# hmetaxa/MVTopicModel

Hardware: AMD Instinct MI355X
Metric: gibbs_tokens_per_sec (higher is better)
Workload: dtype f64

## Files before the change

include/mvhdp.h:

```cpp
#ifndef MVHDP_H
#define MVHDP_H

#include <stddef.h>
#include <stdint.h>

#ifdef __cplusplus
extern "C" {
#endif

#define MVHDP_MAX_MODALITIES 8
#define MVHDP_MAX_TOPICS     2048
#define MVHDP_UNASSIGNED_TOPIC (-1)

typedef enum {
    MVHDP_OK = 0,
    MVHDP_ERR_INVALID_ARG   = -1,
    MVHDP_ERR_STATE         = -2,
    MVHDP_ERR_HIP           = -3,
    MVHDP_ERR_NO_DEVICE     = -4,
    MVHDP_ERR_NEGATIVE_COUNT= -5,
    MVHDP_ERR_UNSUPPORTED   = -6
} mvhdp_status;

typedef struct mvhdp_ctx* mvhdp_handle;

typedef struct {
    int32_t num_topics;
    int32_t num_modalities;
    int32_t num_types[MVHDP_MAX_MODALITIES];
    int32_t device;
    int64_t doc_id_base;
    uint32_t flags;
} mvhdp_config;

typedef struct {
    const double* alpha;
    double alpha_sum[MVHDP_MAX_MODALITIES];
    double beta[MVHDP_MAX_MODALITIES];
    double beta_sum[MVHDP_MAX_MODALITIES];
    double gamma[MVHDP_MAX_MODALITIES];
    double p_a[MVHDP_MAX_MODALITIES][MVHDP_MAX_MODALITIES];
    double p_b[MVHDP_MAX_MODALITIES][MVHDP_MAX_MODALITIES];
    const uint8_t* inactive;
} mvhdp_hyper;

typedef struct {
    int64_t tokens;
    int64_t changed;
    int64_t new_mass_cnt;
    int64_t topic_doc_mass_cnt;
    int64_t word_ftree_mass_cnt;
    int64_t oov_skipped;
    int64_t aborted_docs;
    int64_t exact_fallbacks;
    int32_t activated_topic;
    int32_t activated_modality;
    int64_t activation_key;
    double  sweep_kernel_ms;
    double  total_ms;
    int32_t activations;
    int32_t reserved;
} mvhdp_sweep_stats;

#define MVHDP_ACT_DOC_SHIFT   34
#define MVHDP_ACT_VIEW_SHIFT  31
#define MVHDP_ACT_POS_SHIFT   11
#define MVHDP_ACT_TOPIC_MASK  0x7ffLL
#define MVHDP_ACT_VIEW_MASK   0x7LL
#define MVHDP_ACT_KEY(doc, view, pos, topic) \
    (((int64_t)(doc) << MVHDP_ACT_DOC_SHIFT) | ((int64_t)(view) << MVHDP_ACT_VIEW_SHIFT) | ((int64_t)(pos) << MVHDP_ACT_POS_SHIFT) | (int64_t)(topic))
#define MVHDP_ACT_KEY_TOPIC(key) ((int32_t)((key) & MVHDP_ACT_TOPIC_MASK))
#define MVHDP_ACT_KEY_VIEW(key)  ((int32_t)(((key) >> MVHDP_ACT_VIEW_SHIFT) & MVHDP_ACT_VIEW_MASK))
#define MVHDP_ACT_KEY_NONE INT64_MAX

typedef struct {
    double* tok_dbg[MVHDP_MAX_MODALITIES];
    int32_t n_trace;
    const int64_t* trace_doc;
    const int32_t* trace_view;
    const int32_t* trace_pos;
    double* trace_out;
} mvhdp_debug;

#define MVHDP_SWEEP_REUSE_TREES 0x1u
#define MVHDP_SWEEP_NO_APPLY    0x2u
#define MVHDP_SWEEP_EXACT_CHAIN 0x4u
#define MVHDP_SWEEP_GENERIC_KERNEL 0x8u
#define MVHDP_SWEEP_FROZEN      0x10u

#define MVHDP_SWEEP_LIVE        0x20u
#define MVHDP_SWEEP_LIVE_SEGMENTS(n) (((uint32_t)(n) & 0xffu) << 16)

#define MVHDP_SWEEP_SEGMENT_APPLY 0x40u

#define MVHDP_SWEEP_SEGMENT_OVERLAP 0x80u

#define MVHDP_SWEEP_ONLY_SEGMENT(s) ((((uint32_t)(s) + 1u) & 0xffu) << 24)

#define MVHDP_SWEEP_SHARD_BIRTHS 0x200u

typedef enum {
    MVHDP_BUF_COUNTS = 0,
    MVHDP_BUF_DELTA  = 1,
    MVHDP_BUF_BIRTH_KEYS = 2,
    MVHDP_BUF_COUNTS12 = 3,
    MVHDP_BUF_ROW_CLASS = 4
} mvhdp_buffer;

int mvhdp_create(const mvhdp_config* cfg, mvhdp_handle* out);
int mvhdp_destroy(mvhdp_handle h);
const char* mvhdp_last_error(mvhdp_handle h);
const char* mvhdp_version(void);

int mvhdp_set_corpus(mvhdp_handle h, int32_t m, int64_t num_docs,
                     const int64_t* doc_off , const int32_t* tokens );
int mvhdp_set_assignments(mvhdp_handle h, int32_t m, const int32_t* z );
int mvhdp_set_view_presence(mvhdp_handle h, int32_t m, const uint8_t* present );
int mvhdp_get_assignments(mvhdp_handle h, int32_t m, int32_t* z );

int mvhdp_set_hyper(mvhdp_handle h, const mvhdp_hyper* hy);
int mvhdp_get_alpha(mvhdp_handle h, double* alpha , uint8_t* inactive );
int mvhdp_build_counts(mvhdp_handle h);
int mvhdp_build_trees(mvhdp_handle h);
int mvhdp_build_inference_trees(mvhdp_handle h);
int mvhdp_init_assignments_from_trees(mvhdp_handle h, uint64_t seed);
int mvhdp_get_counts(mvhdp_handle h, int32_t m, int32_t* n_wk , int32_t* n_k );
int mvhdp_set_counts(mvhdp_handle h, int32_t m, const int32_t* n_wk, const int32_t* n_k);
int mvhdp_get_tree(mvhdp_handle h, int32_t m, int32_t type, double* tree );
int mvhdp_get_doc_topic_hist(mvhdp_handle h, int32_t m, int32_t* hist , int32_t hist_len,
                             int32_t* doc_len_counts , int32_t len_len);

int mvhdp_get_count_histogram(mvhdp_handle h, int32_t m, int32_t* hist, int32_t len);
int mvhdp_view_overlap_sums(mvhdp_handle h, double* sums );
int mvhdp_model_log_likelihood(mvhdp_handle h, double* log_likelihood );
int mvhdp_gamma_doc_statistics(mvhdp_handle h, int32_t m, double gamma_m, uint64_t seed, uint32_t round, double* qs, double* qw);
int mvhdp_dp_table_statistics(mvhdp_handle h, int32_t m, const int32_t* hist , int32_t hist_len, const double* conc ,
                              uint64_t seed, uint32_t round, double* mk , uint8_t* active );
int mvhdp_antoniak_draws(mvhdp_handle h, int32_t n, const int32_t* items , const double* conc , uint64_t seed, uint32_t round, int32_t* tables );
int mvhdp_doc_topic_proportions(mvhdp_handle h, const double* view_weights , int64_t d0, int64_t d1, double* out );


int mvhdp_doc_topics_top(mvhdp_handle h, const double* view_weights , int64_t d0, int64_t d1, double threshold, int32_t max,
                         int64_t cap, int64_t* row_off , int32_t* topics, double* weights, int64_t* count);
int mvhdp_entity_topic_distributions(mvhdp_handle h, const double* view_weights, double threshold, int32_t max, int32_t round_digits ,
                                     int64_t n_groups, const int64_t* member_off , const int64_t* members ,
                                     double* out );

typedef enum { MVHDP_SIM_COS_FOLDED = 0,
               MVHDP_SIM_COS        = 1,
               MVHDP_SIM_JSD        = 2    } mvhdp_sim_metric;
typedef struct { int32_t metric; int32_t n, dim; const double* x ; double min_weight; double threshold;
                 int32_t stripe_rows ; int64_t candidate_capacity ; } mvhdp_sim_args;
typedef struct { int64_t pairs_screened ,
                 candidates, emitted; int32_t stripes, regrown; double margin; } mvhdp_sim_stats;
int mvhdp_similar_pairs(mvhdp_handle h, const mvhdp_sim_args* a, int64_t cap, int32_t* i, int32_t* j, double* sim,
                        int64_t* count, mvhdp_sim_stats* stats );
int mvhdp_sim_probe(int32_t n, int32_t dim, int32_t stripe_rows, mvhdp_sim_stats* out);

#define MVHDP_DIAG_MAX_TOP_WORDS 64
#define MVHDP_DIAG_PROPORTIONS   7
#define MVHDP_DIAG_TOKENS             0
#define MVHDP_DIAG_DOCUMENT_ENTROPY   1
#define MVHDP_DIAG_WORD_LENGTH        2
#define MVHDP_DIAG_COHERENCE          3
#define MVHDP_DIAG_NORM_DISCR_WEIGHT  4
#define MVHDP_DIAG_DISCR_WEIGHT       5
#define MVHDP_DIAG_UNIFORM_DIST       6
#define MVHDP_DIAG_CORPUS_DIST        7
#define MVHDP_DIAG_EFF_NUM_WORDS      8
#define MVHDP_DIAG_TOKEN_DOC_DIFF     9
#define MVHDP_DIAG_RANK_1_DOCS       10
#define MVHDP_DIAG_ALLOCATION_RATIO  11
#define MVHDP_DIAG_ALLOCATION_COUNT  12
#define MVHDP_DIAG_ROWS              13
typedef struct {
    int32_t num_top_words;
    const int32_t* word_length;
} mvhdp_diag_args;
typedef struct {
    double*  scores;
    double*  word_scores;
    int32_t* codoc;
    int32_t* top_types;
    int32_t* top_counts;
    int32_t* nonzero;
    int32_t* num_rank1_docs;
    int32_t* num_nonzero_docs;
    int32_t* num_docs_at_proportions;
    double*  sum_count_log_count;
    int32_t* word_type_counts;
    int64_t* num_tokens;
    double*  discr_weight_per_view;
} mvhdp_diag_out;
int mvhdp_top_words(mvhdp_handle h, int32_t m, int32_t n, int32_t* types , int32_t* counts , int32_t* nonzero );
int mvhdp_discr_weights(mvhdp_handle h, double* per_view , int32_t m, double* type_weight );
int mvhdp_diagnostics(mvhdp_handle h, const mvhdp_diag_args* args, mvhdp_diag_out* out);

typedef struct {
    int32_t num_columns;
    int32_t num_context_columns;
    int32_t with_topics;
    int32_t window;
    int32_t num_samples;
    int32_t min_doc_length;
    int64_t sampling_table_size;
    double  sampling_factor;
    double  min_exp, max_exp;
    int32_t sigmoid_cache_size;
    int32_t reserved;
} mvhdp_emb_config;
typedef struct {
    int64_t words_so_far;
    int64_t words_sampled;
    int64_t words_considered;
    int64_t docs_skipped;
    int64_t calls;
    int64_t negatives_skipped;
    double  residual;
    double  last_epoch_residual;
    int64_t last_epoch_calls;
    double  kernel_ms;
} mvhdp_emb_stats;
#define MVHDP_EMB_SERIAL 0x1u
int mvhdp_emb_init(mvhdp_handle h, const mvhdp_emb_config* cfg, const double* weights , uint64_t seed);
int mvhdp_emb_count_words(mvhdp_handle h);
int mvhdp_emb_train(mvhdp_handle h, int32_t epochs, uint64_t seed, uint32_t round, uint32_t flags, mvhdp_emb_stats* stats );
int mvhdp_emb_get_vectors(mvhdp_handle h, double* weights , double* negative_weights );
int mvhdp_emb_set_vectors(mvhdp_handle h, const double* weights , const double* negative_weights );
int mvhdp_emb_word_stats(mvhdp_handle h, int64_t* counts , double* retention , int64_t* total_words );
int mvhdp_emb_sampling_table(mvhdp_handle h, int64_t first, int64_t n, int32_t* types );
int mvhdp_emb_softmax(mvhdp_handle h, int32_t reset_sums, double* exp_dot , double* sum_exp );
int mvhdp_emb_nearest(mvhdp_handle h, const double* query , int32_t n, int32_t* words, double* word_sims, int32_t* topics, double* topic_sims);
int mvhdp_emb_release(mvhdp_handle h);

int mvhdp_set_vectors_mix(mvhdp_handle h, double lambda, const double* exp_dot , const double* sum_exp );
int mvhdp_get_vectors_mix(mvhdp_handle h, double* lambda, double* mix );

int mvhdp_sweep(mvhdp_handle h, uint32_t sweep_idx, uint64_t seed, uint32_t flags,
                const double* p_override, const mvhdp_debug* dbg, mvhdp_sweep_stats* stats);
int mvhdp_sweep_many(mvhdp_handle h, uint32_t first_idx, int32_t n, uint64_t seed, uint32_t flags, mvhdp_sweep_stats* stats );
int mvhdp_apply_delta(mvhdp_handle h, int32_t activated_topic, int32_t activated_modality);
int mvhdp_apply_delta_begin(mvhdp_handle h);
int mvhdp_apply_delta_rows(mvhdp_handle h, int64_t row_begin, int64_t row_end);
int mvhdp_apply_delta_end(mvhdp_handle h, int32_t activated_topic, int32_t activated_modality);
int mvhdp_get_birth_keys(mvhdp_handle h, int64_t* keys );
int mvhdp_activate_births(mvhdp_handle h, const int64_t* keys );
int mvhdp_trees_current(mvhdp_handle h);
int mvhdp_get_view_weights(mvhdp_handle h, double* p );

typedef struct {
    int32_t force_primary;
    int32_t narrow;
    int32_t walk_fixed;
    int32_t single_stream;
    int32_t live16;
    int32_t single_wave;
    double  walk_theta[MVHDP_MAX_MODALITIES];
    double  primary_min_share;
    int32_t learnt_walk_step[4];
// ... 80 lines not shown
```

mvtopicmodel_amd/csrc/mvhdp_api.hip:

```cpp
#include "mvhdp_ctx.h"

static thread_local std::string g_create_error;

static std::mutex g_reg_mutex;
static std::set<mvhdp_ctx*>* g_live = nullptr;
static bool g_exiting = false, g_atexit_registered = false;
static void release_device_resources(mvhdp_ctx* h);

static void mvhdp_at_exit()
{
    std::lock_guard<std::mutex> lk(g_reg_mutex);
    g_exiting = true;
    if (g_live) for (mvhdp_ctx* h : *g_live) release_device_resources(h);
}

static void register_handle(mvhdp_ctx* h)
{
    std::lock_guard<std::mutex> lk(g_reg_mutex);
    if (!g_live) g_live = new std::set<mvhdp_ctx*>();
    g_live->insert(h);
    if (!g_atexit_registered) { atexit(mvhdp_at_exit); g_atexit_registered = true; }
}

bool mvhdp_is_live(mvhdp_ctx* h)
{
    std::lock_guard<std::mutex> lk(g_reg_mutex);
    return g_live && g_live->count(h) != 0;
}

static void read_environment(mvhdp_ctx* h)
{
    if (const char* f = getenv("MVHDP_FORCE_RMAX")) { const int v = atoi(f); if (v == 1 || v == 2 || v == 4 || v == 8 || v == 16 || v == 32) h->tu.force_primary = v; }
    if (const char* f = getenv("MVHDP_NARROW")) h->tu.narrow = atoi(f) != 0 ? -1 : 0;
    if (const char* f = getenv("MVHDP_SINGLE_STREAM")) h->tu.single_stream = atoi(f) != 0;
    if (const char* f = getenv("MVHDP_SIDE_PRIORITY")) h->side_priority = atoi(f);
    if (const char* f = getenv("MVHDP_LIVE16")) h->tu.live16 = atoi(f);
    if (const char* f = getenv("MVHDP_LIVE_OVERLAP")) h->tu.live_overlap = atoi(f);
    if (const char* f = getenv("MVHDP_LIVE_ROWS")) h->tu.live_rows = atoi(f);
    if (const char* f = getenv("MVHDP_LIVE_ROWS_THETA")) h->tu.live_rows_theta = atof(f);
    if (const char* f = getenv("MVHDP_COEF_LDS_KB")) h->tu.coef_lds_max_bytes = std::max(0, std::min(64, atoi(f))) * 1024;
    if (const char* f = getenv("MVHDP_LIVE_ROWS_SEGMENTS")) h->tu.live_rows_segments = std::max(1, std::min(255, atoi(f)));
    if (const char* f = getenv("MVHDP_WIDEST_ON_MAIN")) h->tu.widest_on_main = atoi(f) != 0;
    if (const char* f = getenv("MVHDP_NARROW_WIDE")) h->tu.narrow_wide = atoi(f) != 0;
    if (const char* f = getenv("MVHDP_SLIM")) h->tu.slim = std::max(0, std::min(2, atoi(f)));
    if (const char* f = getenv("MVHDP_LIVE_TREE_EVERY")) h->live_tree_every = std::max(1, atoi(f));
    if (const char* f = getenv("MVHDP_GATE_PCT")) { const int v = atoi(f); if (v >= 5 && v <= 95) h->gate_pct = v; }
    if (const char* f = getenv("MVHDP_FOUR_ROUND_ON_C")) h->tu.four_round_on_c = atoi(f);
    if (const char* f = getenv("MVHDP_DELTA16")) h->tu.delta16 = atoi(f) != 0;
    if (const char* f = getenv("MVHDP_FORK_DELAY_US")) h->tu.fork_delay_us = std::max(0, std::min(1000, atoi(f)));
    if (const char* f = getenv("MVHDP_FORCE_MODE")) { if (!strcmp(f, "serial")) h->tu.single_stream = 1; }
    if (const char* f = getenv("MVHDP_PRIMARY_MIN_SHARE")) { const double v = atof(f); if (v > 0.0 && v <= 1.0) h->tu.primary_min_share = v; }
    if (const char* t = getenv("MVHDP_WALK_THETA")) {
        int m = 0;
        for (const char* q = t; *q && m < MVHDP_MAXM; m++) {
            h->tu.walk_theta[m] = atof(q);
            while (*q && *q != ',') q++;
            if (*q == ',') q++;
        }
        for (; m < MVHDP_MAXM; m++) h->tu.walk_theta[m] = 0.0;
        h->tu.walk_fixed = 1;
    }
    h->dbg_env = getenv("MVHDP_DEBUG") != nullptr;
    h->diag.overlap_serial = getenv("MVHDP_OVERLAP_SERIAL") != nullptr;
    h->diag.no_row_sample = getenv("MVHDP_NO_ROW_SAMPLE") != nullptr;
    h->diag.no_heavy_refresh = getenv("MVHDP_NO_HEAVY_REFRESH") != nullptr;
}

hipError_t make_stream(hipStream_t* out, bool high_priority)
{
    int least = 0, greatest = 0;
    if (high_priority && hipDeviceGetStreamPriorityRange(&least, &greatest) == hipSuccess && greatest < least &&
        hipStreamCreateWithPriority(out, hipStreamNonBlocking, greatest) == hipSuccess) return hipSuccess;
    if (high_priority) { (void)hipGetLastError(); *out = nullptr; }
    return hipStreamCreateWithFlags(out, hipStreamNonBlocking);
}

extern "C" const char* mvhdp_version(void) { return "mvhdp 0.1 (gfx950)"; }

extern "C" const char* mvhdp_last_error(mvhdp_handle h) { return (h && mvhdp_is_live(h)) ? h->err.c_str() : g_create_error.c_str(); }

extern "C" int mvhdp_create(const mvhdp_config* cfg, mvhdp_handle* out)
{
    if (!cfg || !out) { g_create_error = "null argument"; return MVHDP_ERR_INVALID_ARG; }
    *out = nullptr;
    const int K = cfg->num_topics, M = cfg->num_modalities;
    if (K < 1 || K > MVHDP_MAX_TOPICS || M < 1 || M > MVHDP_MAX_MODALITIES) {
        g_create_error = "num_topics must be in [1,2048] and num_modalities in [1,8]";
        return MVHDP_ERR_INVALID_ARG;
    }
    for (int m = 0; m < M; m++) if (cfg->num_types[m] < 1) { g_create_error = "num_types[m] must be >= 1"; return MVHDP_ERR_INVALID_ARG; }
    for (int m = 0; m < M; m++) if (cfg->num_types[m] >= (1 << 29)) { g_create_error = "num_types[m] must be below 2^29"; return MVHDP_ERR_INVALID_ARG; }
    if (cfg->doc_id_base < 0 || cfg->doc_id_base >= (1LL << 29)) { g_create_error = "doc_id_base out of range"; return MVHDP_ERR_INVALID_ARG; }
    int ndev = 0;
    if (hipGetDeviceCount(&ndev) != hipSuccess || ndev <= 0 || cfg->device < 0 || cfg->device >= ndev) {
        g_create_error = "no usable HIP device (the sweep has no CPU fallback)";
        return MVHDP_ERR_NO_DEVICE;
    }
    hipDeviceProp_t prop;
    if (hipGetDeviceProperties(&prop, cfg->device) != hipSuccess) { g_create_error = "hipGetDeviceProperties failed"; return MVHDP_ERR_HIP; }
    if (strncmp(prop.gcnArchName, "gfx950", 6) != 0) {
        g_create_error = std::string("device is ") + prop.gcnArchName + ", this library is built for gfx950 only";
        return MVHDP_ERR_NO_DEVICE;
    }
    mvhdp_ctx* h = new mvhdp_ctx();
    register_handle(h);
    h->cfg = *cfg;
    h->device = cfg->device;
    h->num_cus = prop.multiProcessorCount;
    h->max_lds = 160 * 1024;
    MvModel& mm = h->mm;
    mm.K = K; mm.M = M;
    mm.rowbase[0] = 0;
    for (int m = 0; m < M; m++) { mm.V[m] = cfg->num_types[m]; mm.rowbase[m + 1] = mm.rowbase[m] + cfg->num_types[m]; }
    mm.doc_id_base = cfg->doc_id_base;
    mm.first_inactive = -1;
    mm.D = -1;
#define CREATE_HIP(call) do { hipError_t e_ = (call); if (e_ != hipSuccess) { \
    g_create_error = std::string(#call) + ": " + hipGetErrorString(e_); mvhdp_destroy(h); return MVHDP_ERR_HIP; } } while (0)
    CREATE_HIP(hipSetDevice(h->device));
    CREATE_HIP(hipStreamCreateWithFlags(&h->stream, hipStreamNonBlocking));
    h->own_stream = true;
    for (auto& e : h->ev) CREATE_HIP(hipEventCreate(&e));
    const int64_t nrows = mm.rowbase[M];
    const size_t cbytes = (size_t)(nrows * K + (int64_t)M * K + MVHDP_TAIL_WORDS) * sizeof(int32_t);
    CREATE_HIP(hipMalloc(&mm.counts, cbytes));
    CREATE_HIP(hipMalloc(&mm.delta, cbytes));
    CREATE_HIP(hipMemset(mm.counts, 0, cbytes));
    CREATE_HIP(hipMalloc(&mm.counts16, (size_t)nrows * K * sizeof(uint16_t) + 64));
    CREATE_HIP(hipMemset(mm.counts16, 0, (size_t)nrows * K * sizeof(uint16_t)));
    CREATE_HIP(hipMalloc(&mm.delta16, (size_t)(nrows * K + 2) * sizeof(uint16_t)));
    CREATE_HIP(hipMemsetD16(mm.delta16, (unsigned short)0x8000, (size_t)(nrows * K + 2)));
    CREATE_HIP(hipMalloc(&mm.heavy, (size_t)nrows));
    CREATE_HIP(hipMemset(mm.heavy, 1, (size_t)nrows));
    CREATE_HIP(hipMemset(mm.delta, 0, cbytes));
    CREATE_HIP(hipMalloc(&mm.trees, (size_t)nrows * 2 * K * sizeof(double)));
    CREATE_HIP(hipMalloc(&mm.root, (size_t)nrows * sizeof(double)));
    CREATE_HIP(hipMalloc(&mm.mass0, (size_t)nrows * sizeof(float)));
    CREATE_HIP(hipMemset(mm.mass0, 0, (size_t)nrows * sizeof(float)));
    CREATE_HIP(hipMalloc(&mm.coef, (size_t)M * (((K + 7) & ~7) + K + 8) * sizeof(float)));
    {
        const int nlev = (K > 1) ? (32 - __builtin_clz((unsigned)(K - 1))) : 0;
        mm.dt_f = nlev ? ((nlev - 1) % 3) + 1 : 0;
        mm.dt_nbd = 1; mm.dt_base[0] = 0; mm.dt_depth[0] = 0;
        int nblk = 1;
        for (int dep = mm.dt_f; nlev && dep < nlev; dep += 3) {
            mm.dt_base[mm.dt_nbd] = nblk; mm.dt_depth[mm.dt_nbd] = dep; mm.dt_nbd++;
            nblk += 1 << dep;
        }
        mm.dt_nblk = nblk;
        CREATE_HIP(hipMalloc(&mm.dtab, (size_t)nrows * nblk * 8 * sizeof(double)));
    }
    CREATE_HIP(hipMalloc(&h->d_alpha, (size_t)M * (K + 1) * sizeof(double)));
    CREATE_HIP(hipMalloc(&h->d_inactive, (size_t)K));
    CREATE_HIP(hipMemset(h->d_inactive, 0, (size_t)K));
    CREATE_HIP(hipMalloc(&h->d_births, (size_t)(2 + 2 * K) * sizeof(int32_t)));
    CREATE_HIP(hipMemset(h->d_births, 0, (size_t)(2 + 2 * K) * sizeof(int32_t)));
    CREATE_HIP(hipMalloc(&h->d_birth_keys, (size_t)K * sizeof(long long)));
    CREATE_HIP(hipMalloc(&h->d_birth_table, (size_t)K * sizeof(long long)));
    {
        const std::vector<long long> none((size_t)K, LLONG_MAX);
        CREATE_HIP(hipMemcpy(h->d_birth_table, none.data(), (size_t)K * sizeof(long long), hipMemcpyHostToDevice));
    }
    CREATE_HIP(hipMalloc(&h->d_ctl, CTL_WORDS * sizeof(unsigned long long)));
    CREATE_HIP(hipMemset(h->d_ctl, 0, CTL_WORDS * sizeof(unsigned long long)));
    h->d_stats = h->d_ctl;
    h->d_act_key = (long long*)(h->d_ctl + ST_COUNT);
    h->d_ovf_meta = (unsigned int*)(h->d_ctl + ST_COUNT + 1);
    h->d_doc_counter = h->d_ctl + ST_COUNT + 1 + META_WORDS64;
    CREATE_HIP(hipHostMalloc((void**)&h->h_ctl, CTL_WORDS * sizeof(unsigned long long), hipHostMallocDefault));
    for (int c = 0; c < MVHDP_N_CLASSES; c++)
        for (int f = 0; f < MVHDP_N_FLAVOURS; f++) { h->regs.regs[c][f] = mvhdp_sweep_kernel_regs(c, f); h->regs.regs_mix[c][f] = mvhdp_sweep_kernel_regs(c, f == MVHDP_FLAVOUR_PLAIN ? MVHDP_FLAVOUR_WALK : f, true); }
    read_environment(h);
    {
        int vmax = 0;
        for (int m = 0; m < M; m++) vmax = std::max(vmax, (int)cfg->num_types[m]);
        if (plan_slim_table(K, vmax, h->tu.slim)) {
            CREATE_HIP(hipMalloc(&mm.counts12, (size_t)nrows * mvhdp_slim_row_bytes(K)));
            CREATE_HIP(hipMemset(mm.counts12, 0, (size_t)nrows * mvhdp_slim_row_bytes(K)));
        }
    }
    mm.alpha = h->d_alpha;
    mm.inactive = h->d_inactive;
    h->h_alpha.assign((size_t)M * (K + 1), 0.0);
    h->h_inactive.assign((size_t)K, 0);
    h->wt.init_defaults(K);
    h->wt_mix.init_defaults(K);
    *out = h;
    return MVHDP_OK;
}

static void release_device_resources(mvhdp_ctx* h)
{
    if (h->device_released) return;
    h->device_released = true;
    hipSetDevice(h->device);
    if (h->stream) hipStreamSynchronize(h->stream);
    auto fr = [](auto*& p) { if (p) { hipFree((void*)p); p = nullptr; } };
    for (int m = 0; m < MVHDP_MAXM; m++) { fr(h->d_doc_off[m]); fr(h->d_tok[m]); fr(h->d_z[m]); fr(h->d_carry[m]); fr(h->d_present[m]); }
    fr(h->mm.counts); fr(h->mm.delta16); fr(h->mm.counts16); fr(h->mm.counts12); fr(h->mm.heavy); fr(h->mm.delta); fr(h->mm.trees); fr(h->mm.root); fr(h->mm.coef); fr(h->mm.mass0); fr(h->d_births); fr(h->d_birth_keys); fr(h->d_birth_table); fr(h->mm.dtab); fr(h->mm.p);
    fr(h->d_alpha); fr(h->d_inactive); fr(h->d_ctl);
    fr(h->d_mix); fr(h->d_mix32); h->mm.mix = nullptr; h->mm.mix32 = nullptr; h->mix_lambda = 0.0;
    mvhdp_emb_free(h);
    if (h->h_ctl) { hipHostFree(h->h_ctl); h->h_ctl = nullptr; }
    h->d_stats = nullptr; h->d_act_key = nullptr; h->d_doc_counter = nullptr; h->d_ovf_meta = nullptr;
    fr(h->d_doc_order); fr(h->d_lists); fr(h->d_nslots); fr(h->d_stats_many); fr(h->d_heavy_list); fr(h->d_heavy_ctl);
    if (h->ev_rf_go) { hipEventDestroy(h->ev_rf_go); h->ev_rf_go = nullptr; }
    if (h->ev_rf_done) { hipEventDestroy(h->ev_rf_done); h->ev_rf_done = nullptr; }
    if (h->rf_stream) { hipStreamDestroy(h->rf_stream); h->rf_stream = nullptr; }
    fr(h->ov.counts2); fr(h->ov.counts16_2); fr(h->ov.dtab2); fr(h->ov.root2); fr(h->ov.trees2); fr(h->ov.delta2); fr(h->ov.delta3); fr(h->ov.ctl2); fr(h->ov.lists2);
    for (auto& e : h->ov.ev_seg) if (e) { hipEventDestroy(e); e = nullptr; }
    if (h->ov.ev_start) { hipEventDestroy(h->ov.ev_start); h->ov.ev_start = nullptr; }
    if (h->ov.x1) { hipStreamDestroy(h->ov.x1); h->ov.x1 = nullptr; }
    if (h->ov.xa) { hipStreamDestroy(h->ov.xa); h->ov.xa = nullptr; }
    for (auto& e : h->ev_many) if (e) { hipEventDestroy(e); e = nullptr; }
    for (auto& e : h->ev) if (e) { hipEventDestroy(e); e = nullptr; }
    if (h->ev_fork) { hipEventDestroy(h->ev_fork); h->ev_fork = nullptr; }
    for (auto& e : h->ev_join) if (e) { hipEventDestroy(e); e = nullptr; }
    for (auto& st : h->side) if (st) { hipStreamDestroy(st); st = nullptr; }
    if (h->own_stream && h->stream) hipStreamDestroy(h->stream);
    h->stream = nullptr;
}

extern "C" int mvhdp_destroy(mvhdp_handle h)
{
    if (!h) return MVHDP_OK;
    bool exiting;
    {
        std::lock_guard<std::mutex> lk(g_reg_mutex);
        if (!g_live || g_live->erase(h) == 0) return MVHDP_ERR_INVALID_ARG;
        exiting = g_exiting;
    }
    if (!exiting) release_device_resources(h);
    delete h;
    return MVHDP_OK;
}

extern "C" int mvhdp_set_stream(mvhdp_handle h, void* hip_stream)
{
    CHECK_H(h);
    HIPC(h, hipSetDevice(h->device));
    HIPC(h, hipStreamSynchronize(h->stream));
    if (h->own_stream) { hipStreamDestroy(h->stream); h->own_stream = false; }
    if (hip_stream) h->stream = (hipStream_t)hip_stream;
    else { HIPC(h, hipStreamCreateWithFlags(&h->stream, hipStreamNonBlocking)); h->own_stream = true; }
    return MVHDP_OK;
}

extern "C" int mvhdp_synchronize(mvhdp_handle h)
{
    CHECK_H(h);
    HIPC(h, hipSetDevice(h->device));
    HIPC(h, hipStreamSynchronize(h->stream));
    return MVHDP_OK;
}

extern "C" int mvhdp_set_corpus(mvhdp_handle h, int32_t m, int64_t D, const int64_t* doc_off, const int32_t* tokens)
{
    CHECK_H(h);
    MvModel& mm = h->mm;
    if (m < 0 || m >= mm.M || D < 0 || !doc_off) FAIL(h, MVHDP_ERR_INVALID_ARG, "set_corpus: bad view, num_docs or doc_off");
    if (mm.D >= 0 && D != mm.D) {
        bool any_other = false;
        for (int j = 0; j < mm.M; j++) if (j != m && h->have_corpus[j]) any_other = true;
        if (any_other) FAIL(h, MVHDP_ERR_INVALID_ARG, "set_corpus: every view must list the same entities (empty span = view absent)");
    }
    if (mm.doc_id_base + D >= (1LL << 29)) FAIL(h, MVHDP_ERR_INVALID_ARG, "set_corpus: too many entities");
    if (doc_off[0] != 0) FAIL(h, MVHDP_ERR_INVALID_ARG, "set_corpus: doc_off[0] must be 0");
    for (int64_t d = 0; d < D; d++) {
        int64_t len = doc_off[d + 1] - doc_off[d];
        if (len < 0) FAIL(h, MVHDP_ERR_INVALID_ARG, "set_corpus: doc_off must be non-decreasing");
        if (len >= (1 << 20)) FAIL(h, MVHDP_ERR_INVALID_ARG, "set_corpus: a view of one entity is limited to 2^20-1 tokens");
    }
    const int64_t N = doc_off[D];
    if (N > 0 && !tokens) FAIL(h, MVHDP_ERR_INVALID_ARG, "set_corpus: tokens is null");
    HIPC(h, hipSetDevice(h->device));
    HIPC(h, hipStreamSynchronize(h->stream));
    if (h->d_doc_off[m]) { hipFree(h->d_doc_off[m]); h->d_doc_off[m] = nullptr; }
    if (h->d_tok[m]) { hipFree(h->d_tok[m]); h->d_tok[m] = nullptr; }
    if (h->d_z[m]) { hipFree(h->d_z[m]); h->d_z[m] = nullptr; }
    if (h->d_present[m]) { hipFree(h->d_present[m]); h->d_present[m] = nullptr; }
    h->h_present[m].clear(); mm.present[m] = nullptr;
    HIPC(h, hipMalloc(&h->d_doc_off[m], (size_t)(D + 1) * sizeof(int64_t)));
    HIPC(h, hipMemcpy(h->d_doc_off[m], doc_off, (size_t)(D + 1) * sizeof(int64_t), hipMemcpyHostToDevice));
    const size_t nb = (size_t)std::max<int64_t>(N, 1) * sizeof(int32_t);
    HIPC(h, hipMalloc(&h->d_tok[m], nb));
    HIPC(h, hipMalloc(&h->d_z[m], nb));
    if (N > 0) HIPC(h, hipMemcpy(h->d_tok[m], tokens, (size_t)N * sizeof(int32_t), hipMemcpyHostToDevice));
    HIPC(h, hipMemset(h->d_z[m], 0xff, nb));
    h->unassigned[m] = N > 0;
    h->h_doc_off[m].assign(doc_off, doc_off + D + 1);
    h->N[m] = N;
    h->have_corpus[m] = true;
    h->max_doc_tokens = -1;
    if (h->d_doc_order) { hipFree(h->d_doc_order); h->d_doc_order = nullptr; }
    if (h->d_lists) { hipFree(h->d_lists); h->d_lists = nullptr; }
    if (h->ov.lists2) { hipFree(h->ov.lists2); h->ov.lists2 = nullptr; }
    if (h->d_nslots) { hipFree(h->d_nslots); h->d_nslots = nullptr; }
    mm.nslots = nullptr;
    for (auto& c : h->d_carry) if (c) { hipFree(c); c = nullptr; }
    h->nslots_valid = false;
    mm.D = D;
    mm.doc_off[m] = (const int64_t*)h->d_doc_off[m];
    mm.tok[m] = (const int32_t*)h->d_tok[m];
    mm.z[m] = (int32_t*)h->d_z[m];
    if (mm.p) { hipFree(mm.p); mm.p = nullptr; }
    h->have_counts = false; h->have_trees = false;
    return MVHDP_OK;
}

int require_corpus(mvhdp_ctx* h)
{
    for (int m = 0; m < h->mm.M; m++)
        if (!h->have_corpus[m]) FAIL(h, MVHDP_ERR_STATE, "set_corpus has not been called for every view");
    return MVHDP_OK;
}

extern "C" int mvhdp_set_assignments(mvhdp_handle h, int32_t m, const int32_t* z)
{
    CHECK_H(h);
    if (m < 0 || m >= h->mm.M) FAIL(h, MVHDP_ERR_INVALID_ARG, "set_assignments: bad view");
    if (!h->have_corpus[m]) FAIL(h, MVHDP_ERR_STATE, "set_assignments before set_corpus");
    if (h->N[m] > 0 && !z) FAIL(h, MVHDP_ERR_INVALID_ARG, "set_assignments: null z");
    bool any_unassigned = false;
    for (int64_t i = 0; i < h->N[m]; i++) {
        if (z[i] < -1 || z[i] >= h->mm.K) FAIL(h, MVHDP_ERR_INVALID_ARG, "set_assignments: topic out of range");
        any_unassigned = any_unassigned || z[i] < 0;
    }
    HIPC(h, hipSetDevice(h->device));
    HIPC(h, hipStreamSynchronize(h->stream));
    if (h->N[m] > 0) HIPC(h, hipMemcpy(h->d_z[m], z, (size_t)h->N[m] * sizeof(int32_t), hipMemcpyHostToDevice));
    h->unassigned[m] = any_unassigned;
    h->nslots_valid = false;
    if (h->have_counts) h->counts_stale = true;
    return MVHDP_OK;
}

extern "C" int mvhdp_set_view_presence(mvhdp_handle h, int32_t m, const uint8_t* present)
{
    CHECK_H(h);
    MvModel& mm = h->mm;
    if (m < 0 || m >= mm.M) FAIL(h, MVHDP_ERR_INVALID_ARG, "set_view_presence: bad view");
    if (!h->have_corpus[m]) FAIL(h, MVHDP_ERR_STATE, "set_view_presence before set_corpus");
    HIPC(h, hipSetDevice(h->device));
    HIPC(h, hipStreamSynchronize(h->stream));
    if (h->d_present[m]) { hipFree(h->d_present[m]); h->d_present[m] = nullptr; }
    h->h_present[m].clear(); mm.present[m] = nullptr;
    if (h->d_carry[m]) { hipFree(h->d_carry[m]); h->d_carry[m] = nullptr; }
    if (!present || mm.D == 0) return MVHDP_OK;
    for (int64_t d = 0; d < mm.D; d++)
        if (!present[d] && h->h_doc_off[m][d + 1] > h->h_doc_off[m][d]) FAIL(h, MVHDP_ERR_INVALID_ARG, "set_view_presence: an entity with tokens in the view is marked absent");
    h->h_present[m].assign(present, present + mm.D);
    HIPC(h, hipMalloc(&h->d_present[m], (size_t)mm.D));
    HIPC(h, hipMemcpy(h->d_present[m], present, (size_t)mm.D, hipMemcpyHostToDevice));
    mm.present[m] = h->d_present[m];
    return MVHDP_OK;
}

extern "C" int mvhdp_get_assignments(mvhdp_handle h, int32_t m, int32_t* z)
{
    CHECK_H(h);
    if (m < 0 || m >= h->mm.M) FAIL(h, MVHDP_ERR_INVALID_ARG, "get_assignments: bad view");
    if (!h->have_corpus[m]) FAIL(h, MVHDP_ERR_STATE, "get_assignments before set_corpus");
    HIPC(h, hipSetDevice(h->device));
    HIPC(h, hipStreamSynchronize(h->stream));
    if (h->N[m] > 0) HIPC(h, hipMemcpy(z, h->d_z[m], (size_t)h->N[m] * sizeof(int32_t), hipMemcpyDeviceToHost));
    return MVHDP_OK;
}

extern "C" int mvhdp_set_hyper(mvhdp_handle h, const mvhdp_hyper* hy)
{
    CHECK_H(h);
    if (!hy || !hy->alpha) FAIL(h, MVHDP_ERR_INVALID_ARG, "set_hyper: null");
    MvModel& mm = h->mm;
    const int K = mm.K, M = mm.M;
    for (int m = 0; m < M; m++) {
        if (!(hy->beta_sum[m] >= 1e-30 && hy->beta_sum[m] <= 1e30) || !(hy->beta[m] >= 1e-30 && hy->beta[m] <= 1e30))
            FAIL(h, MVHDP_ERR_INVALID_ARG, "set_hyper: beta and beta_sum must be in [1e-30, 1e30]");
        mm.alpha_sum[m] = hy->alpha_sum[m]; mm.beta[m] = hy->beta[m];
        mm.beta_sum[m] = hy->beta_sum[m];   mm.gamma[m] = hy->gamma[m];
        for (int j = 0; j < M; j++) { mm.p_a[m][j] = hy->p_a[m][j]; mm.p_b[m][j] = hy->p_b[m][j]; }
    }
    h->h_alpha.assign(hy->alpha, hy->alpha + (size_t)M * (K + 1));
    if (hy->inactive) h->h_inactive.assign(hy->inactive, hy->inactive + K);
    else h->h_inactive.assign((size_t)K, 0);
    mm.first_inactive = -1;
    for (int k = 0; k < K; k++) if (h->h_inactive[k]) { mm.first_inactive = k; break; }
    HIPC(h, hipSetDevice(h->device));
    HIPC(h, hipStreamSynchronize(h->stream));
    HIPC(h, hipMemcpy(h->d_alpha, h->h_alpha.data(), (size_t)M * (K + 1) * sizeof(double), hipMemcpyHostToDevice));
    HIPC(h, hipMemcpy(h->d_inactive, h->h_inactive.data(), (size_t)K, hipMemcpyHostToDevice));
    h->have_hyper = true;
    h->have_trees = false;
    return MVHDP_OK;
}

extern "C" int mvhdp_get_alpha(mvhdp_handle h, double* alpha, uint8_t* inactive)
{
    CHECK_H(h);
    if (!h->have_hyper) FAIL(h, MVHDP_ERR_STATE, "get_alpha before set_hyper");
    if (alpha) memcpy(alpha, h->h_alpha.data(), h->h_alpha.size() * sizeof(double));
    if (inactive) memcpy(inactive, h->h_inactive.data(), h->h_inactive.size());
    return MVHDP_OK;
}

extern "C" int mvhdp_build_counts(mvhdp_handle h)
{
    CHECK_H(h);
    int rc = require_corpus(h); if (rc) return rc;
    HIPC(h, hipSetDevice(h->device));
    HIPC(h, mvhdp_launch_build_counts(h->mm, h->N, h->stream));
    if (h->delta_pending) {
        HIPC(h, hipMemsetAsync(h->mm.delta, 0, (size_t)counts_len(h) * sizeof(int32_t), h->stream));
        h->delta_pending = false; h->delta_clean = true;
    }
    if (h->delta16_used) {
        HIPC(h, hipMemsetD16Async(h->mm.delta16, (unsigned short)0x8000, (size_t)(h->mm.rowbase[h->mm.M] * h->mm.K), h->stream));
        h->delta16_used = false;
    }
    HIPC(h, hipStreamSynchronize(h->stream));
    h->have_counts = true; h->have_trees = false; h->counts_stale = false;
    return MVHDP_OK;
}

static int ensure_full_trees(mvhdp_ctx* h)
{
    if (!h->have_trees || h->full_trees) return MVHDP_OK;
    HIPC(h, mvhdp_launch_build_trees(h->mm, h->trees_inference, true, h->stream));
    HIPC(h, hipStreamSynchronize(h->stream));
    h->full_trees = true;
    return MVHDP_OK;
}

extern "C" int mvhdp_build_trees(mvhdp_handle h)
{
    CHECK_H(h);
    if (!h->have_hyper) FAIL(h, MVHDP_ERR_STATE, "build_trees before set_hyper");
    if (!h->have_counts) FAIL(h, MVHDP_ERR_STATE, "build_trees before build_counts/set_counts");
    HIPC(h, hipSetDevice(h->device));
    HIPC(h, mvhdp_launch_build_trees(h->mm, false, true, h->stream));
    HIPC(h, hipStreamSynchronize(h->stream));
    h->have_trees = true; h->full_trees = true; h->trees_inference = false;
    return MVHDP_OK;
}

extern "C" int mvhdp_build_inference_trees(mvhdp_handle h)
{
    CHECK_H(h);
    if (!h->have_hyper) FAIL(h, MVHDP_ERR_STATE, "build_inference_trees before set_hyper");
    if (!h->have_counts) FAIL(h, MVHDP_ERR_STATE, "build_inference_trees before build_counts/set_counts");
    HIPC(h, hipSetDevice(h->device));
    HIPC(h, mvhdp_launch_build_trees(h->mm, true, true, h->stream));
    HIPC(h, hipStreamSynchronize(h->stream));
    h->have_trees = true; h->full_trees = true; h->trees_inference = true;
    return MVHDP_OK;
}

extern "C" int mvhdp_init_assignments_from_trees(mvhdp_handle h, uint64_t seed)
{
    CHECK_H(h);
    int rc = require_corpus(h); if (rc) return rc;
    if (!h->have_trees) FAIL(h, MVHDP_ERR_STATE, "init_assignments_from_trees before build_trees/build_inference_trees");
    HIPC(h, hipSetDevice(h->device));
    HIPC(h, mvhdp_launch_init_from_trees(h->mm, (uint32_t)seed, (uint32_t)(seed >> 32), h->stream));
    HIPC(h, hipStreamSynchronize(h->stream));
    for (int m = 0; m < h->mm.M; m++) h->unassigned[m] = false;
    h->nslots_valid = false;
    if (h->have_counts) h->counts_stale = true;
    return MVHDP_OK;
}

extern "C" int mvhdp_get_counts(mvhdp_handle h, int32_t m, int32_t* n_wk, int32_t* n_k)
{
    CHECK_H(h);
    MvModel& mm = h->mm;
    if (m < 0 || m >= mm.M) FAIL(h, MVHDP_ERR_INVALID_ARG, "get_counts: bad view");
    HIPC(h, hipSetDevice(h->device));
    HIPC(h, hipStreamSynchronize(h->stream));
    const int K = mm.K;
    if (n_wk) HIPC(h, hipMemcpy(n_wk, mm.counts + mm.rowbase[m] * K, (size_t)mm.V[m] * K * sizeof(int32_t), hipMemcpyDeviceToHost));
    if (n_k) HIPC(h, hipMemcpy(n_k, mm.counts + mm.rowbase[mm.M] * K + (int64_t)m * K, (size_t)K * sizeof(int32_t), hipMemcpyDeviceToHost));
    return MVHDP_OK;
}

extern "C" int mvhdp_set_counts(mvhdp_handle h, int32_t m, const int32_t* n_wk, const int32_t* n_k)
{
    CHECK_H(h);
    MvModel& mm = h->mm;
    if (m < 0 || m >= mm.M) FAIL(h, MVHDP_ERR_INVALID_ARG, "set_counts: bad view");
    HIPC(h, hipSetDevice(h->device));
    HIPC(h, hipStreamSynchronize(h->stream));
    const int K = mm.K;
    if (n_wk) HIPC(h, hipMemcpy(mm.counts + mm.rowbase[m] * K, n_wk, (size_t)mm.V[m] * K * sizeof(int32_t), hipMemcpyHostToDevice));
    if (n_k) HIPC(h, hipMemcpy(mm.counts + mm.rowbase[mm.M] * K + (int64_t)m * K, n_k, (size_t)K * sizeof(int32_t), hipMemcpyHostToDevice));
    h->have_counts = true; h->have_trees = false; h->counts_stale = false;
    return MVHDP_OK;
}

extern "C" int mvhdp_get_tree(mvhdp_handle h, int32_t m, int32_t type, double* tree)
{
    CHECK_H(h);
    MvModel& mm = h->mm;
    if (m < 0 || m >= mm.M || type < 0 || type >= mm.V[m] || !tree) FAIL(h, MVHDP_ERR_INVALID_ARG, "get_tree: bad argument");
    if (!h->have_trees) FAIL(h, MVHDP_ERR_STATE, "get_tree before build_trees");
    HIPC(h, hipSetDevice(h->device));
    { int rc2 = ensure_full_trees(h); if (rc2) return rc2; }
    HIPC(h, hipStreamSynchronize(h->stream));
    HIPC(h, hipMemcpy(tree, mm.trees + (mm.rowbase[m] + type) * 2 * mm.K, (size_t)2 * mm.K * sizeof(double), hipMemcpyDeviceToHost));
    return MVHDP_OK;
}

extern "C" int mvhdp_get_doc_topic_hist(mvhdp_handle h, int32_t m, int32_t* hist, int32_t hist_len,
                                        int32_t* doc_len_counts, int32_t len_len)
{
    CHECK_H(h);
    MvModel& mm = h->mm;
    if (m < 0 || m >= mm.M || (hist && hist_len < 1) || (doc_len_counts && len_len < 1))
        FAIL(h, MVHDP_ERR_INVALID_ARG, "get_doc_topic_hist: bad argument");
    int rc = require_corpus(h); if (rc) return rc;
    HIPC(h, hipSetDevice(h->device));
    int32_t *d_hist = nullptr, *d_len = nullptr;
    hipError_t e = hipSuccess;
    if (hist) e = hipMalloc(&d_hist, (size_t)mm.K * hist_len * sizeof(int32_t));
    if (e == hipSuccess && doc_len_counts) e = hipMalloc(&d_len, (size_t)len_len * sizeof(int32_t));
    if (e == hipSuccess) e = mvhdp_launch_doc_topic_hist(mm, m, d_hist, hist_len, d_len, len_len, h->stream);
    if (e == hipSuccess && hist) e = hipMemcpy(hist, d_hist, (size_t)mm.K * hist_len * sizeof(int32_t), hipMemcpyDeviceToHost);
    if (e == hipSuccess && doc_len_counts) e = hipMemcpy(doc_len_counts, d_len, (size_t)len_len * sizeof(int32_t), hipMemcpyDeviceToHost);
    if (d_hist) hipFree(d_hist);
    if (d_len) hipFree(d_len);
    HIPC(h, e);
    return MVHDP_OK;
}

int64_t compute_max_doc_tokens(mvhdp_ctx* h)
{
    if (h->max_doc_tokens >= 0) return h->max_doc_tokens;
    int64_t mx = 0, mn = INT64_MAX;
    const MvModel& mm = h->mm;
    std::vector<int64_t> tot((size_t)mm.D);
    for (int64_t d = 0; d < mm.D; d++) {
        int64_t t = 0;
        for (int m = 0; m < mm.M; m++) t += h->h_doc_off[m][d + 1] - h->h_doc_off[m][d];
        tot[d] = t;
        mx = std::max(mx, t); mn = std::min(mn, t);
    }
    if (h->d_doc_order) { hipFree(h->d_doc_order); h->d_doc_order = nullptr; }
// ... 125 lines not shown
    if (row_begin < 0 || row_end > nrows || row_begin > row_end) FAIL(h, MVHDP_ERR_INVALID_ARG, "apply_delta_rows: bad row range");
    HIPC(h, hipSetDevice(h->device));
    HIPC(h, mvhdp_launch_build_trees_rows(h->mm, false, h->last_need_full, row_begin, row_end, true, h->d_stats + ST_NEGATIVE, h->stream));
    h->rows_applied += row_end - row_begin;
    return MVHDP_OK;
}

extern "C" int mvhdp_apply_delta_end(mvhdp_handle h, int32_t activated_topic, int32_t activated_modality)
{
    CHECK_H(h);
    const int64_t nrows = h->mm.rowbase[h->mm.M];
    if (h->rows_applied != nrows) { h->rows_applied = -1; FAIL(h, MVHDP_ERR_STATE, "apply_delta_end: the row ranges applied do not cover every row exactly once"); }
    h->rows_applied = -1;
    HIPC(h, hipSetDevice(h->device));
    unsigned long long neg = 0;
    HIPC(h, hipMemcpyAsync(&neg, h->d_stats + ST_NEGATIVE, sizeof neg, hipMemcpyDeviceToHost, h->stream));
    HIPC(h, hipStreamSynchronize(h->stream));
    h->delta_clean = true; h->delta_pending = false;
    h->have_trees = true; h->full_trees = h->last_need_full; h->trees_inference = false;
    if (activated_topic >= 0) {
        h->have_trees = false;
        int rc = apply_activation(h, activated_topic, activated_modality);
        if (rc) return rc;
    }
    if (neg) FAIL(h, MVHDP_ERR_NEGATIVE_COUNT, "a topic count went below zero (UPD:202-215)");
    return MVHDP_OK;
}

extern "C" int mvhdp_trees_current(mvhdp_handle h)
{
    CHECK_H(h);
    return h->have_trees ? 1 : 0;
}

extern "C" int mvhdp_get_tuning(mvhdp_handle h, mvhdp_tuning* t)
{
    CHECK_H(h);
    if (!t) FAIL(h, MVHDP_ERR_INVALID_ARG, "get_tuning: null");
    memset(t, 0, sizeof *t);
    t->force_primary = h->tu.force_primary; t->narrow = h->tu.narrow; t->walk_fixed = h->tu.walk_fixed;
    t->single_stream = h->tu.single_stream; t->primary_min_share = h->tu.primary_min_share; t->live16 = h->tu.live16;
    t->single_wave = h->tu.single_wave; t->live_overlap = h->tu.live_overlap; t->live_rows = h->tu.live_rows;
    for (int m = 0; m < MVHDP_MAX_MODALITIES; m++) { t->walk_theta[m] = h->tu.walk_theta[m]; t->tree_branch_share[m] = h->wt.walk_f[m]; }
    for (int g = 0; g < WALK_GROUPS; g++) t->learnt_walk_step[g] = g == h->wt.walk_cls ? h->wt.walk_i : h->wt.walk_i_by[g];
    t->learnt_walk_step[3] = -1;
    return MVHDP_OK;
}

extern "C" int mvhdp_set_tuning(mvhdp_handle h, const mvhdp_tuning* t)
{
    CHECK_H(h);
    if (!t) FAIL(h, MVHDP_ERR_INVALID_ARG, "set_tuning: null");
    const int fp = t->force_primary;
    if (!(fp == 0 || fp == 1 || fp == 2 || fp == 4 || fp == 8 || fp == 16 || fp == 32)) FAIL(h, MVHDP_ERR_INVALID_ARG, "set_tuning: force_primary must be 0, 1, 2, 4, 8, 16 or 32");
    if (t->primary_min_share < 0.0 || t->primary_min_share > 1.0) FAIL(h, MVHDP_ERR_INVALID_ARG, "set_tuning: primary_min_share outside [0, 1]");
    for (int g = 0; g < WALK_GROUPS; g++) if (t->learnt_walk_step[g] < -1 || t->learnt_walk_step[g] > MVHDP_WALK_BINS) FAIL(h, MVHDP_ERR_INVALID_ARG, "set_tuning: learnt_walk_step outside [-1, 20]");
    h->tu.force_primary = fp; h->tu.narrow = t->narrow; h->tu.walk_fixed = t->walk_fixed ? 1 : 0;
    h->tu.single_stream = t->single_stream ? 1 : 0;
    h->tu.live16 = t->live16 < 0 ? -1 : (t->live16 ? 1 : 0);
    h->tu.single_wave = t->single_wave ? 1 : 0;
    h->tu.live_overlap = t->live_overlap < 0 ? -1 : (t->live_overlap ? 1 : 0);
    h->tu.live_rows = t->live_rows < 0 ? -1 : (t->live_rows ? 1 : 0);
    h->tu.primary_min_share = t->primary_min_share > 0.0 ? t->primary_min_share : 0.10;
    for (int m = 0; m < MVHDP_MAX_MODALITIES; m++) h->tu.walk_theta[m] = t->walk_theta[m];
    if (t->learnt_walk_step[0] >= 0 || t->learnt_walk_step[1] >= 0 || t->learnt_walk_step[2] >= 0) h->wt.restore(t->learnt_walk_step, t->tree_branch_share, h->mm.M);
    return MVHDP_OK;
}

extern "C" int mvhdp_plan_probe(const mvhdp_plan_input* pi, const mvhdp_tuning* t, mvhdp_plan_output* po)
{
    if (!pi || !po) return MVHDP_ERR_INVALID_ARG;
    PlanIn in;
    in.K = pi->num_topics; in.M = pi->num_modalities; in.D = pi->num_entities; in.mdt = pi->max_entity_tokens;
    if (in.K < 1 || in.K > MVHDP_MAX_TOPICS || in.M < 1 || in.M > MVHDP_MAX_MODALITIES || in.D < 0) return MVHDP_ERR_INVALID_ARG;
    in.have_order = true;
    for (int c = 0; c < 5; c++) in.n_longer[c] = pi->entities_longer_than[c];
    for (int b = 0; b < MVHDP_HIST_BINS; b++) in.tok_hist[b] = pi->tokens_by_list_rounds[b];
    for (int b = 0; b < MVHDP_ENT_BINS; b++) in.ent_hist[b] = pi->entities_by_class[b];
    in.flags = pi->flags; in.debug = pi->debug != 0; in.batch = pi->batch != 0; in.trees_current = pi->trees_current != 0;
    in.first_inactive = pi->inactive_topics ? 0 : -1;
    in.num_cus = pi->num_cus > 0 ? pi->num_cus : 256;
    for (int c = 0; c < MVHDP_N_CLASSES; c++) for (int f = 0; f < 3; f++) in.regs.regs[c][f] = pi->kernel_registers[c][f];
    for (int c = 0; c < MVHDP_N_CLASSES; c++) for (int f = 0; f < 3; f++) in.regs.regs_mix[c][f] = pi->kernel_registers_mix[c][f] > 0 ? pi->kernel_registers_mix[c][f] : pi->kernel_registers[c][f];
    in.vectors_mix = pi->vectors_mix != 0 && !(pi->flags & MVHDP_SWEEP_FROZEN);
    in.slim_table = t && t->narrow == 2;
    PlanTuning tu;
    WalkTuner wt;
    wt.init_defaults(in.K);
    if (t) {
        tu.force_primary = t->force_primary; tu.narrow = t->narrow; tu.walk_fixed = t->walk_fixed; tu.single_stream = t->single_stream;
        tu.live16 = t->live16; tu.single_wave = t->single_wave ? 1 : 0; tu.live_overlap = t->live_overlap; tu.live_rows = t->live_rows;
        if (t->primary_min_share > 0) tu.primary_min_share = t->primary_min_share;
        for (int m = 0; m < MVHDP_MAX_MODALITIES; m++) tu.walk_theta[m] = t->walk_theta[m];
        if (t->learnt_walk_step[0] >= 0 || t->learnt_walk_step[1] >= 0 || t->learnt_walk_step[2] >= 0) wt.restore(t->learnt_walk_step, t->tree_branch_share, in.M);
    }
    SweepPlan p;
    plan_sweep(in, tu, wt, p);
    memset(po, 0, sizeof *po);
    po->status = p.err;
    if (p.err) return MVHDP_OK;
    po->segments = p.nseg; po->primary_class = p.pc; po->routed_prefix = p.H; po->register_resident = p.fast ? 1 : 0;
    po->need_full_trees = p.need_full ? 1 : 0; po->dominant_class = p.dominant;
    for (int c = 0; c < MVHDP_N_CLASSES; c++) {
        po->class_used[c] = p.cls[c].used ? 1 : 0; po->class_map[c] = p.class_map[c];
        po->class_stream[c] = p.cls[c].stream; po->class_grid[c] = p.cls[c].grid; po->class_lds_bytes[c] = (int64_t)p.cls[c].lds;
        po->class_walk[c] = p.cls[c].walk; po->class_narrow[c] = p.cls[c].narrow; po->class_register_resident[c] = p.cls[c].fast ? 1 : 0;
        po->class_theta0[c] = p.cls[c].theta[0];
    }
    po->delta16 = p.delta16 ? 1 : 0;
    po->live_rows = p.live_rows ? 1 : 0;
    return MVHDP_OK;
}

extern "C" int mvhdp_tuner_probe(int32_t num_modalities, const double* tree_branch_share, const double* u1_hist, const double* ns_by_step ,
                                 int32_t n_sweeps, int32_t group, int32_t* steps_out )
{
    if (!tree_branch_share || !ns_by_step || !steps_out || num_modalities < 1 || num_modalities > MVHDP_MAX_MODALITIES || n_sweeps < 0) return MVHDP_ERR_INVALID_ARG;
    WalkTuner wt;
    if (group < 0 || group >= WALK_GROUPS) return MVHDP_ERR_INVALID_ARG;
    for (int m = 0; m < num_modalities; m++) wt.walk_f[m] = tree_branch_share[m];
    for (int b = 0; b < MVHDP_WALK_BINS; b++) wt.walk_hist[b] = u1_hist ? u1_hist[b] : 0.0;
    for (int i = 0; i < n_sweeps; i++) {
        double theta[WALK_GROUPS][MVHDP_MAXM]; bool measure;
        wt.propose(group, num_modalities, theta, &measure);
        steps_out[i] = wt.walk_probe_i;
        wt.observe(true, 1, num_modalities, ns_by_step[std::max(0, std::min(MVHDP_WALK_BINS, wt.walk_probe_i))]);
    }
    return MVHDP_OK;
}

extern "C" int mvhdp_get_view_weights(mvhdp_handle h, double* p)
{
    CHECK_H(h);
    MvModel& mm = h->mm;
    if (!p) FAIL(h, MVHDP_ERR_INVALID_ARG, "get_view_weights: null");
    if (mm.M == 1) { for (int64_t d = 0; d < mm.D; d++) p[d] = 1.0; return MVHDP_OK; }
    if (!mm.p) FAIL(h, MVHDP_ERR_STATE, "get_view_weights before the first sweep");
    HIPC(h, hipSetDevice(h->device));
    HIPC(h, hipStreamSynchronize(h->stream));
    HIPC(h, hipMemcpy(p, mm.p, (size_t)mm.D * mm.M * mm.M * sizeof(double), hipMemcpyDeviceToHost));
    return MVHDP_OK;
}

extern "C" int mvhdp_device_buffer(mvhdp_handle h, mvhdp_buffer which, void** dev_ptr, size_t* bytes)
{
    CHECK_H(h);
    if (!dev_ptr || !bytes) FAIL(h, MVHDP_ERR_INVALID_ARG, "device_buffer: null");
    size_t b = (size_t)counts_len(h) * sizeof(int32_t);
    if (which == MVHDP_BUF_COUNTS) { *dev_ptr = h->mm.counts; *bytes = b; return MVHDP_OK; }
    if (which == MVHDP_BUF_DELTA) { *dev_ptr = h->mm.delta; *bytes = b; return MVHDP_OK; }
    if (which == MVHDP_BUF_BIRTH_KEYS) { *dev_ptr = h->d_birth_table; *bytes = (size_t)h->mm.K * sizeof(long long); return MVHDP_OK; }
    if (which == MVHDP_BUF_COUNTS12 && h->mm.counts12) { *dev_ptr = h->mm.counts12; *bytes = (size_t)h->mm.rowbase[h->mm.M] * mvhdp_slim_row_bytes(h->mm.K); return MVHDP_OK; }
    if (which == MVHDP_BUF_ROW_CLASS) { *dev_ptr = h->mm.heavy; *bytes = (size_t)h->mm.rowbase[h->mm.M]; return MVHDP_OK; }
    FAIL(h, MVHDP_ERR_INVALID_ARG, "device_buffer: unknown buffer (or a handle without that table)");
}

extern "C" int mvhdp_counts_written(mvhdp_handle h)
{
    CHECK_H(h);
    h->have_counts = true; h->have_trees = false; h->counts_stale = false;
    return MVHDP_OK;
}

static double log_gamma_stirling_host(double z)
{
    const double HALF_LOG_TWO_PI = std::log(6.283185307179586) / 2.0;
    int shift = 0;
    while (z < 2.0) { z = z + 1; shift++; }
    double result = HALF_LOG_TWO_PI + (z - 0.5) * std::log(z) - z + 1 / (12.0 * z) - 1 / (360.0 * z * z * z)
                    + 1 / (1260.0 * z * z * z * z * z);
    while (shift > 0) { shift--; z = z - 1; result = result - std::log(z); }
    return result;
}

extern "C" int mvhdp_get_count_histogram(mvhdp_handle h, int32_t m, int32_t* hist, int32_t len)
{
    CHECK_H(h);
    MvModel& mm = h->mm;
    if (m < 0 || m >= mm.M || !hist || len < 1) FAIL(h, MVHDP_ERR_INVALID_ARG, "get_count_histogram: bad argument");
    if (!h->have_counts) FAIL(h, MVHDP_ERR_STATE, "get_count_histogram before build_counts/set_counts");
    HIPC(h, hipSetDevice(h->device));
    int32_t* d = nullptr;
    HIPC(h, hipMalloc(&d, (size_t)len * sizeof(int32_t)));
    hipError_t e = mvhdp_launch_count_hist(mm, m, d, len, h->stream);
    if (e == hipSuccess) e = hipMemcpyAsync(hist, d, (size_t)len * sizeof(int32_t), hipMemcpyDeviceToHost, h->stream);
    if (e == hipSuccess) e = hipStreamSynchronize(h->stream);
    hipFree(d);
    HIPC(h, e);
    return MVHDP_OK;
}

int mvhdp_view_overlap_accumulate(mvhdp_ctx* h, double* acc)
{
    MvModel& mm = h->mm;
    int rc = require_corpus(h); if (rc) return rc;
    const int M = mm.M;
    if (mm.D == 0) return MVHDP_OK;
    HIPC(h, hipSetDevice(h->device));
    double* d = nullptr;
    const size_t n = (size_t)M * M * mm.D;
    HIPC(h, hipMalloc(&d, n * sizeof(double)));
    std::vector<double> host(n);
    hipError_t e = mvhdp_launch_view_overlap(mm, d, h->stream);
    if (e == hipSuccess) e = hipMemcpyAsync(host.data(), d, n * sizeof(double), hipMemcpyDeviceToHost, h->stream);
    if (e == hipSuccess) e = hipStreamSynchronize(h->stream);
    hipFree(d);
    HIPC(h, e);
    for (int i = 0; i < M * M; i++) {
        double a = acc[i];
        const double* col = host.data() + (size_t)i * mm.D;
        for (int64_t doc = 0; doc < mm.D; doc++) a += col[doc];
        acc[i] = a;
    }
    return MVHDP_OK;
}

extern "C" int mvhdp_view_overlap_sums(mvhdp_handle h, double* sums)
{
    CHECK_H(h);
    if (!sums) FAIL(h, MVHDP_ERR_INVALID_ARG, "view_overlap_sums: null");
    for (int i = 0; i < h->mm.M * h->mm.M; i++) sums[i] = 0.0;
    return mvhdp_view_overlap_accumulate(h, sums);
}

int mvhdp_doc_topic_prepare(mvhdp_ctx* h, DocTopicCarry& carry)
{
    MvModel& mm = h->mm;
    int rc = require_corpus(h); if (rc) return rc;
    if (!h->have_hyper) FAIL(h, MVHDP_ERR_STATE, "doc_topic_proportions before set_hyper");
    HIPC(h, hipSetDevice(h->device));
    for (int m = 0; m < mm.M; m++) {
        if (!h->d_carry[m] && mm.D > 0) {
            std::vector<int64_t> src((size_t)mm.D);
            int64_t last = -1;
            for (int64_t d = 0; d < mm.D; d++) {
                const bool has = h->h_present[m].empty() ? h->h_doc_off[m][d + 1] > h->h_doc_off[m][d] : h->h_present[m][(size_t)d] != 0;
                if (has) last = d;
                src[(size_t)d] = last;
            }
            HIPC(h, hipMalloc(&h->d_carry[m], (size_t)mm.D * sizeof(int64_t)));
            HIPC(h, hipMemcpy(h->d_carry[m], src.data(), (size_t)mm.D * sizeof(int64_t), hipMemcpyHostToDevice));
        }
        carry.src[m] = h->d_carry[m];
    }
    return MVHDP_OK;
}

extern "C" int mvhdp_doc_topic_proportions(mvhdp_handle h, const double* view_weights, int64_t d0, int64_t d1, double* out)
{
    CHECK_H(h);
    MvModel& mm = h->mm;
    int rc = require_corpus(h); if (rc) return rc;
    if (!h->have_hyper) FAIL(h, MVHDP_ERR_STATE, "doc_topic_proportions before set_hyper");
    if (!view_weights || !out || d0 < 0 || d1 > mm.D || d0 > d1) FAIL(h, MVHDP_ERR_INVALID_ARG, "doc_topic_proportions: bad range or null buffer");
    if (d1 == d0) return MVHDP_OK;
    DocTopicCarry carry{};
    rc = mvhdp_doc_topic_prepare(h, carry); if (rc) return rc;
    double *d_w = nullptr, *d_out = nullptr;
    const size_t n = (size_t)(d1 - d0) * mm.K;
    hipError_t e = hipMalloc(&d_w, (size_t)mm.M * sizeof(double));
    if (e == hipSuccess) e = hipMalloc(&d_out, n * sizeof(double));
    if (e == hipSuccess) e = hipMemcpyAsync(d_w, view_weights, (size_t)mm.M * sizeof(double), hipMemcpyHostToDevice, h->stream);
    if (e == hipSuccess) e = mvhdp_launch_doc_topic_prop(mm, carry, d_w, d0, d1, d_out, h->stream);
    if (e == hipSuccess) e = hipMemcpyAsync(out, d_out, n * sizeof(double), hipMemcpyDeviceToHost, h->stream);
    if (e == hipSuccess) e = hipStreamSynchronize(h->stream);
    if (d_w) hipFree(d_w);
    if (d_out) hipFree(d_out);
    HIPC(h, e);
    return MVHDP_OK;
}

extern "C" int mvhdp_gamma_doc_statistics(mvhdp_handle h, int32_t m, double gamma_m, uint64_t seed, uint32_t round, double* qs, double* qw)
{
    CHECK_H(h);
    MvModel& mm = h->mm;
    if (m < 0 || m >= mm.M || !qs || !qw || !(gamma_m > 0.0)) FAIL(h, MVHDP_ERR_INVALID_ARG, "gamma_doc_statistics: bad argument");
    int rc = require_corpus(h); if (rc) return rc;
    *qs = 0; *qw = 0;
    if (mm.D == 0) return MVHDP_OK;
    HIPC(h, hipSetDevice(h->device));
    const int NB = 1024;
    double* d_part = nullptr;
    std::vector<double> part(2 * NB);
    hipError_t e = hipMalloc(&d_part, 2 * NB * sizeof(double));
    if (e == hipSuccess) e = mvhdp_launch_gamma_doc_stats(mm, m, gamma_m, (uint32_t)seed, (uint32_t)(seed >> 32), round, d_part, NB, h->stream);
    if (e == hipSuccess) e = hipMemcpyAsync(part.data(), d_part, 2 * NB * sizeof(double), hipMemcpyDeviceToHost, h->stream);
    if (e == hipSuccess) e = hipStreamSynchronize(h->stream);
    if (d_part) hipFree(d_part);
    HIPC(h, e);
    double a = 0, b = 0;
    for (int i = 0; i < NB; i++) { a += part[2 * i]; b += part[2 * i + 1]; }
    *qs = a; *qw = b;
    return MVHDP_OK;
}

extern "C" int mvhdp_dp_table_statistics(mvhdp_handle h, int32_t m, const int32_t* hist, int32_t hist_len, const double* conc, uint64_t seed, uint32_t round,
                                         double* mk, uint8_t* active)
{
    CHECK_H(h);
    MvModel& mm = h->mm;
    const int K = mm.K;
    if (m < 0 || m >= mm.M || !hist || hist_len < 1 || !conc || !mk || !active) FAIL(h, MVHDP_ERR_INVALID_ARG, "dp_table_statistics: bad argument");
    HIPC(h, hipSetDevice(h->device));
    const size_t hb = (size_t)K * hist_len * sizeof(int32_t);
    void* d = nullptr;
    hipError_t e = hipMalloc(&d, hb + (size_t)K * (2 * sizeof(double) + 8));
// ... 116 lines not shown
```

mvtopicmodel_amd/csrc/mvhdp_ctx.h:

```cpp
#pragma once
#include "mvhdp_device.h"
#include "../../include/mvhdp.h"
#include "mvhdp_plan.h"

#include <algorithm>
#include <functional>
#include <limits>
#include <climits>
#include <mutex>
#include <set>
#include <cmath>
#include <cstdio>
#include <cstdlib>
#include <cstring>
#include <string>
#include <vector>


struct EmbState;

struct mvhdp_ctx {
    mvhdp_config cfg{};
    MvModel mm{};
    int device = 0;
    int num_cus = 256;
    size_t max_lds = 65536;
    hipStream_t stream = nullptr;
    bool own_stream = false;
    hipEvent_t ev[4]{};
    std::string err;

    int64_t N[MVHDP_MAXM]{};
    bool have_corpus[MVHDP_MAXM]{};
    std::vector<int64_t> h_doc_off[MVHDP_MAXM];
    void* d_doc_off[MVHDP_MAXM]{};
    void* d_tok[MVHDP_MAXM]{};
    void* d_z[MVHDP_MAXM]{};
    uint8_t* d_present[MVHDP_MAXM]{};
    std::vector<uint8_t> h_present[MVHDP_MAXM];
    int64_t max_doc_tokens = -1;

    double* d_alpha = nullptr;
    uint8_t* d_inactive = nullptr;
    std::vector<double> h_alpha;
    std::vector<uint8_t> h_inactive;
    bool have_hyper = false, have_counts = false, have_trees = false;
    bool full_trees = false;
    bool trees_inference = false;
    bool delta_clean = false;
    bool delta_pending = false;
    bool last_need_full = true;
    int64_t rows_applied = -1;
    bool device_released = false;

    unsigned long long* d_ctl = nullptr;
    unsigned long long* h_ctl = nullptr;
    unsigned long long* d_stats = nullptr;
    long long* d_act_key = nullptr;
    int32_t* d_births = nullptr;
    long long* d_birth_keys = nullptr;
    long long* d_birth_table = nullptr;
    std::vector<int32_t> h_births;
    std::vector<long long> h_birth_keys;
    unsigned long long* d_doc_counter = nullptr;
    int32_t* d_doc_order = nullptr;
    unsigned int* d_ovf_meta = nullptr;
    int32_t* d_lists = nullptr;
    uint16_t* d_nslots = nullptr;
    int32_t* d_heavy_list = nullptr; unsigned int* d_heavy_ctl = nullptr;
    hipStream_t rf_stream = nullptr; hipEvent_t ev_rf_go = nullptr, ev_rf_done = nullptr;
    int live_tree_every = 1;
    int gate_pct = 60;
    struct Diag {
        bool overlap_serial = false;
        bool no_row_sample = false;
        bool no_heavy_refresh = false;
    } diag;
    bool delta16_used = false;
    int side_priority = 2;
    hipStream_t side[PLAN_N_STREAMS]{};
    hipEvent_t ev_fork = nullptr, ev_join[PLAN_N_STREAMS]{};
    std::vector<hipEvent_t> ev_many;
    unsigned long long* d_stats_many = nullptr;
    int stats_many_cap = 0;
    std::vector<int64_t> tokens_desc;
    int64_t* d_carry[MVHDP_MAXM]{};
    unsigned long long last_hist[MVHDP_HIST_BINS]{};
    unsigned long long last_ent[MVHDP_ENT_BINS]{};
    bool nslots_valid = false;
    bool unassigned[MVHDP_MAXM]{};
    bool counts_stale = false;
    struct Overlap {
        int32_t* counts2 = nullptr; uint16_t* counts16_2 = nullptr; double* dtab2 = nullptr; double* root2 = nullptr; double* trees2 = nullptr;
        int32_t* delta2 = nullptr; int32_t* delta3 = nullptr;
        unsigned long long* ctl2 = nullptr;
        int32_t* lists2 = nullptr;
        hipStream_t x1 = nullptr, xa = nullptr;
        hipEvent_t ev_start = nullptr;
        bool deltas_dirty = false;
        std::vector<hipEvent_t> ev_seg;
    } ov;
    PlanRegs regs{};
    PlanTuning tu;
    WalkTuner wt;
    bool dbg_env = false;
    size_t lds_attr_set = 0;
    EmbState* emb = nullptr;
    double* d_mix = nullptr;
    float* d_mix32 = nullptr;
    double mix_lambda = 0.0;
    WalkTuner wt_mix;
};


bool mvhdp_is_live(mvhdp_ctx* h);
#define CHECK_H(h) do { if (!(h) || !mvhdp_is_live(h)) return MVHDP_ERR_INVALID_ARG; \
                        if ((h)->device_released) return MVHDP_ERR_STATE;  } while (0)
#define HIPC(h, call) do { hipError_t e_ = (call); if (e_ != hipSuccess) { \
    (h)->err = std::string(#call) + ": " + hipGetErrorString(e_); return MVHDP_ERR_HIP; } } while (0)
#define FAIL(h, code, msg) do { (h)->err = (msg); return (code); } while (0)

enum { MVHDP_HEAVY_CAP = 8192 };
enum { MVHDP_REFRESH_BLOCKS = 16 };
enum { MVHDP_TAIL_WORDS = 4 };
static int64_t counts_len(const mvhdp_ctx* h) { return h->mm.rowbase[h->mm.M] * h->mm.K + (int64_t)h->mm.M * h->mm.K; }

enum { META_HIST = 0, META_MISROUTED = 40, META_WORDS64 = 48, META_BYTES = META_WORDS64 * 8, META_CLASS_COUNTS = 64  };
static_assert(MVHDP_HIST_BINS + MVHDP_ENT_BINS <= 32, "histograms overlap the class counts");
enum { CTL_WORDS = ST_COUNT + 1 + META_WORDS64 + 8 };


struct DebugBufs {
    std::vector<void*> to_free;
    double* tok_dbg[MVHDP_MAXM] = {};
    int n_trace = 0;
    const int64_t* trace_doc = nullptr; const int32_t* trace_view = nullptr; const int32_t* trace_pos = nullptr;
    double* trace_out = nullptr;
    void release() { for (void* p : to_free) hipFree(p); to_free.clear(); }
};

struct SweepOutcome {
    int n_activations = 0;
    long long first_act = LLONG_MAX;
};

struct PendingSweep {
    SweepPlan p;
    SweepOutcome oc;
    uint32_t flags = 0;
    bool debug = false;
    const mvhdp_debug* dbg = nullptr;
    DebugBufs db;
    bool open = false;
    bool births = false;
};
int mvhdp_sweep_begin(mvhdp_ctx* h, uint32_t sweep_idx, uint64_t seed, uint32_t flags, const double* p_override, const mvhdp_debug* dbg, PendingSweep& ps);
int mvhdp_sweep_finish(mvhdp_ctx* h, PendingSweep& ps, mvhdp_sweep_stats* stats);
int require_corpus(mvhdp_ctx* h);
int64_t compute_max_doc_tokens(mvhdp_ctx* h);
int apply_activation(mvhdp_ctx* h, int32_t activated_topic, int32_t activated_modality);
int activate_born(mvhdp_ctx* h, const std::vector<std::pair<int32_t, long long>>& born, SweepOutcome& oc);
hipError_t make_stream(hipStream_t* out, bool high_priority);
int mvhdp_activate_births_ex(mvhdp_ctx* h, const int64_t* keys, int* n_born, long long* first_key);
int mvhdp_view_overlap_accumulate(mvhdp_ctx* h, double* acc );
int mvhdp_ll_doc_accumulate(mvhdp_ctx* h, int m, double* ll, int64_t* cnt);
int mvhdp_ll_model_finish(mvhdp_ctx* h, int m, double ll_doc, int64_t modalityCnt, double* out);

struct DiagModel {
    int N = 0;
    std::vector<int32_t> types, counts, nonzero, nk;
    std::vector<int64_t> word_type_counts;
    std::vector<double> type_weight, per_view;
};
struct DiagAcc {
    std::vector<int32_t> codoc, rank1_docs, nonzero_docs, at_proportions;
    std::vector<double> sum_count_log_count;
    int64_t num_tokens = 0;
    void reset(int K, int N)
    {
        codoc.assign((size_t)K * N * N, 0); rank1_docs.assign((size_t)K, 0); nonzero_docs.assign((size_t)K, 0);
        at_proportions.assign((size_t)K * MVHDP_DIAG_PROPORTIONS, 0); sum_count_log_count.assign((size_t)K, 0.0); num_tokens = 0;
    }
};
int mvhdp_diag_check_args(mvhdp_ctx* h, const mvhdp_diag_args* args, const mvhdp_diag_out* out);
int mvhdp_diag_model(mvhdp_ctx* h, int N, DiagModel& dm);
int mvhdp_diag_docs(mvhdp_ctx* h, const DiagModel& dm, DiagAcc& acc);
int mvhdp_diag_finish(mvhdp_ctx* h, const DiagModel& dm, const DiagAcc& acc, const mvhdp_diag_args* args, const mvhdp_diag_out* out);

int mvhdp_doc_topic_prepare(mvhdp_ctx* h, DocTopicCarry& carry);

void mvhdp_emb_free(mvhdp_ctx* h);
static inline WalkTuner& walk_tuner_of(mvhdp_ctx* h, uint32_t flags) { return (h->mm.mix && !(flags & MVHDP_SWEEP_FROZEN)) ? h->wt_mix : h->wt; }
```

mvtopicmodel_amd/csrc/mvhdp_device.h:

```cpp
#pragma once
#include <hip/hip_runtime.h>
#include <stdint.h>
#include "mvhdp_flavour.h"

#define MVHDP_MAXM 8
#define MVHDP_WALK_BINS 20
#define MVHDP_VIEW_STATS (2 + MVHDP_WALK_BINS)

struct MvModel {
    int32_t K, M;
    int32_t V[MVHDP_MAXM];
    int64_t rowbase[MVHDP_MAXM + 1];
    int64_t D;
    int64_t doc_id_base;
    const int64_t* doc_off[MVHDP_MAXM];
    const int32_t* tok[MVHDP_MAXM];
    int32_t* z[MVHDP_MAXM];
    const uint8_t* present[MVHDP_MAXM];
    uint16_t* nslots;
    int32_t* counts;
    uint16_t* delta16;
    uint16_t* counts16;
    uint8_t* heavy;
    int32_t* delta;
    double* trees;
    double* root;
    float* coef;
    float* mass0;
    double* dtab;
    int32_t dt_nblk, dt_nbd, dt_f;
    int32_t dt_base[6], dt_depth[6];
    const double* alpha;
    const uint8_t* inactive;
    double alpha_sum[MVHDP_MAXM], beta[MVHDP_MAXM], beta_sum[MVHDP_MAXM], gamma[MVHDP_MAXM];
    double p_a[MVHDP_MAXM][MVHDP_MAXM], p_b[MVHDP_MAXM][MVHDP_MAXM];
    double* p;
    int32_t first_inactive;
    const double* mix;
    const float* mix32;
    double oml;
    uint8_t* counts12;
};

#define MVHDP_SL_STRICT_LIVE 0x8000u
#define MVHDP_SL_NO_ROW_SAMPLE 0x2000u
#define MVHDP_ROW_HEAVY 1
#define MVHDP_ROW_BIG 2
#define MVHDP_ROW_SLIM 4
#define MVHDP_ROW_CLASS(h) ((h) & 3)

struct SweepLaunch {
    uint32_t sweep_idx;
    uint32_t seed_lo, seed_hi;
    uint32_t flags;
    int32_t  S_cap;
    int32_t  waves_per_block;
    uint32_t block_shared_bytes;
    int32_t  nk_global;
    uint32_t wave_bytes;
    unsigned long long* stats;
    long long* act_key;
    int32_t* births;
    long long* birth_keys;
    unsigned long long* doc_counter;
    const int32_t* q_list;
    const unsigned int* q_list_count;
    const int32_t* q_order;
    int64_t q_order_start, q_order_count, q_order_stride;
    double walk_theta[MVHDP_MAXM];
    int32_t walk;
    int32_t narrow;
    int32_t delta16;
    int32_t live16;
    int32_t live_rows;
    int32_t coef_lds;
    unsigned long long* slot_hist;
    double* tok_dbg[MVHDP_MAXM];
    int32_t n_trace;
    const int64_t* trace_doc; const int32_t* trace_view; const int32_t* trace_pos;
    double* trace_out;
};

enum {
    ST_TOKENS = 0, ST_CHANGED, ST_NEW, ST_DOC, ST_TREE, ST_OOV, ST_ABORT, ST_FALLBACK, ST_NEGATIVE, ST_MISCLASS, ST_ONDEMAND,
    ST_VIEW_BASE, ST_VIEW_LAST = ST_VIEW_BASE + MVHDP_VIEW_STATS * MVHDP_MAXM - 1,
    ST_T_QUEUE, ST_T_PROLOGUE, ST_T_VIEW, ST_T_CHUNK_HEAD, ST_T_TOKENS, ST_T_CHUNK_END, ST_T_TOTAL,
    ST_T_ENT0, ST_T_ENT1, ST_T_ENT2, ST_N_ENT0, ST_N_ENT1, ST_N_ENT2, ST_T_INIT, ST_T_FLUSH, ST_N_WAVES, ST_T_ROWS, ST_T_ROWS_WAIT,
    ST_COUNT
};

size_t mvhdp_sweep_wave_bytes(int M, int S_cap);

hipError_t mvhdp_launch_build_counts(const MvModel& mm, const int64_t* n_tokens_per_view, hipStream_t s);
hipError_t mvhdp_launch_build_trees(const MvModel& mm, bool inference_leaves, bool write_full, hipStream_t s, bool beside_samplers = false);
hipError_t mvhdp_launch_build_trees_rows(const MvModel& mm, bool inference_leaves, bool write_full, int64_t row_begin, int64_t row_end,
                                         bool apply_first, unsigned long long* negatives, hipStream_t s);
hipError_t mvhdp_launch_build_trees_from_mirror(const MvModel& mm, bool write_full, hipStream_t s, bool beside_samplers = false);
hipError_t mvhdp_launch_widen_mirror(const MvModel& mm, hipStream_t s);
hipError_t mvhdp_launch_live_rows_prepare(const MvModel& mm, bool from_mirror, bool with_heavy_trees, int32_t* heavy_list, unsigned int* heavy_ctl, int heavy_cap, int batch_cells, hipStream_t s);
hipError_t mvhdp_launch_heavy_refresh(const MvModel& mm, const int32_t* heavy_list, const unsigned int* ctl, int heavy_cap, int blocks, hipStream_t s);
hipError_t mvhdp_launch_set_u32(unsigned int* p, unsigned int v, hipStream_t s);
hipError_t mvhdp_launch_apply_nk(const MvModel& mm, unsigned long long* negatives, hipStream_t s);
hipError_t mvhdp_launch_apply2_counts(const MvModel& dst, const int32_t* dA, int32_t* dB, bool use_mirror, unsigned long long* negatives, hipStream_t s);
hipError_t mvhdp_launch_apply_sparse(const MvModel& dst, int32_t* d, bool use_mirror, hipStream_t s);
hipError_t mvhdp_launch_gate(const unsigned long long* qhead, unsigned long long threshold, hipStream_t s);
hipError_t mvhdp_launch_init_from_trees(const MvModel& mm, uint32_t seed_lo, uint32_t seed_hi, hipStream_t s);
hipError_t mvhdp_launch_draw_p(const MvModel& mm, uint32_t sweep_idx, uint32_t seed_lo, uint32_t seed_hi, hipStream_t s);
hipError_t mvhdp_launch_sweep(const MvModel& mm, const SweepLaunch& sl, int grid_blocks, bool debug, hipStream_t s);
hipError_t mvhdp_launch_apply_delta(const MvModel& mm, unsigned long long* stats, hipStream_t s, bool with_delta16 = false);
hipError_t mvhdp_launch_delay(int microseconds, hipStream_t s);
hipError_t mvhdp_launch_ctl_reset(unsigned long long* stats, int n_stats, long long* act_key, unsigned long long* meta, int n_meta,
                                  unsigned int* class_counts, unsigned long long* qheads, hipStream_t s);
hipError_t mvhdp_launch_birth_table(const int32_t* births, const long long* birth_keys, const long long* act_key, int K, long long* keys, hipStream_t s);
hipError_t mvhdp_launch_live_helper(const MvModel& mm, int which, unsigned long long* stats, hipStream_t s);
hipError_t mvhdp_launch_doc_topic_hist(const MvModel& mm, int m, int32_t* hist, int32_t hist_len,
                                       int32_t* doc_len_counts, int32_t len_len, hipStream_t s);
hipError_t mvhdp_sweep_set_max_lds(size_t bytes);
hipError_t mvhdp_launch_count_hist(const MvModel& mm, int m, int32_t* hist, int32_t len, hipStream_t s);
hipError_t mvhdp_launch_view_overlap(const MvModel& mm, double* out, hipStream_t s);
hipError_t mvhdp_launch_loglik_doc(const MvModel& mm, int m, double* doc_out, hipStream_t s);
hipError_t mvhdp_launch_loglik_topic(const MvModel& mm, int m, double* partial, int n_partial, unsigned long long* nonzero, hipStream_t s);
hipError_t mvhdp_launch_gamma_doc_stats(const MvModel& mm, int m, double gamma_m, uint32_t seed_lo, uint32_t seed_hi, uint32_t round,
                                        double* partial, int n_blocks, hipStream_t s);
hipError_t mvhdp_launch_dp_tables(const int32_t* hist, int hist_len, int K, int m, const double* conc, uint32_t seed_lo, uint32_t seed_hi, uint32_t round,
                                  double* mk, uint8_t* active, hipStream_t s);
hipError_t mvhdp_launch_antoniak_draws(int n, const int32_t* items, const double* conc, uint32_t seed_lo, uint32_t seed_hi, uint32_t round, int32_t* tables, hipStream_t s);
hipError_t mvhdp_launch_slot_hist(const MvModel& mm, unsigned long long* hist, hipStream_t s);
struct DocTopicCarry { const int64_t* src[MVHDP_MAXM]; };
hipError_t mvhdp_launch_doc_topic_prop(const MvModel& mm, const DocTopicCarry& carry, const double* w_dev, int64_t d0, int64_t d1, double* out_dev, hipStream_t s);
#define MVHDP_N_CLASSES 6
struct ClassifyArgs {
    const int32_t* order;
    int64_t n, start, stride;
    int32_t class_map[MVHDP_N_CLASSES];
    int32_t check_views;
    int32_t* lists[MVHDP_N_CLASSES];
    unsigned int* counts;
    unsigned long long* misrouted;
};
hipError_t mvhdp_launch_classify(const MvModel& mm, const ClassifyArgs& ca, hipStream_t s);
size_t mvhdp_sweep_fast_wave_bytes(int M, int S_cap, int rmax);
hipError_t mvhdp_launch_sweep_fast(const MvModel& mm, const SweepLaunch& sl, int rmax, int grid_blocks, bool debug, hipStream_t s);
int mvhdp_sweep_kernel_regs(int cls, int flavour, bool mix = false);
int mvhdp_sweep_generic_regs(bool debug, bool mix = false);

#define MVHDP_DOC_BATCH 2
#define MVHDP_HIST_BINS 17
#define MVHDP_ENT_BINS 8
#define MVHDP_NSLOTS_UNKNOWN 0xFFFFu

__host__ __device__ __forceinline__ int mvhdp_class_of(int n, bool view_beyond_16_bits)
{
    int c = (n <= 64) ? 0 : (n <= 128) ? 1 : (n <= 256) ? 2 : (n <= 512) ? 3 : (n <= 1024) ? 4 : 5;
    if (c >= 3 && view_beyond_16_bits) c = 5;
    return c;
}

__device__ __forceinline__ int dtab_sample(const MvModel& mm, int64_t row, double u01)
{
    const int K = mm.K;
    const double* __restrict__ dt = mm.dtab + row * (int64_t)mm.dt_nblk * 8;
    double u = 0.0;
    int i = 1;
    for (int bd = 0; bd < mm.dt_nbd; bd++) {
        if (bd == 0 || i < K) {
            const double2* __restrict__ blk = (const double2*)(dt + (int64_t)(mm.dt_base[bd] + (i - (1 << mm.dt_depth[bd]))) * 8);
            const double2 q0 = blk[0], q1 = blk[1], q2 = blk[2], q3 = blk[3];
            const int levels = (bd == 0) ? mm.dt_f : 3;
            if (bd == 0) u = u01 * q3.y;
            int path = 0;
            if (i < K && levels > 0) {
                const double l = q0.x;
                if (u < l) { i = 2 * i; } else { u = u - l; i = 2 * i + 1; path = 1; }
            }
            if (i < K && levels > 1) {
                const double l = path ? q1.x : q0.y;
                if (u < l) { i = 2 * i; path = 2 * path; } else { u = u - l; i = 2 * i + 1; path = 2 * path + 1; }
                if (i < K && levels > 2) {
                    const double l3 = (path == 0) ? q1.y : (path == 1) ? q2.x : (path == 2) ? q2.y : q3.x;
                    if (u < l3) { i = 2 * i; } else { u = u - l3; i = 2 * i + 1; }
                }
            }
        }
    }
    return i - K;
}

__device__ __forceinline__ int dtab_sample_uniform(const MvModel& mm, int64_t row, double u01)
{
    typedef const __attribute__((address_space(4))) double* cdptr;
    const int K = mm.K;
    const cdptr dt = (cdptr)(mm.dtab + row * (int64_t)mm.dt_nblk * 8);
    double u = 0.0;
    int i = 1;
    for (int bd = 0; bd < mm.dt_nbd; bd++) {
        if (bd == 0 || i < K) {
            const cdptr blk = dt + (int64_t)(mm.dt_base[bd] + (i - (1 << mm.dt_depth[bd]))) * 8;
            const double q0x = blk[0], q0y = blk[1], q1x = blk[2], q1y = blk[3], q2x = blk[4], q2y = blk[5], q3x = blk[6], q3y = blk[7];
            const int levels = (bd == 0) ? mm.dt_f : 3;
            if (bd == 0) u = u01 * q3y;
            int path = 0;
            if (i < K && levels > 0) {
                const double l = q0x;
                if (u < l) { i = 2 * i; } else { u = u - l; i = 2 * i + 1; path = 1; }
            }
            if (i < K && levels > 1) {
                const double l = path ? q1x : q0y;
                if (u < l) { i = 2 * i; path = 2 * path; } else { u = u - l; i = 2 * i + 1; path = 2 * path + 1; }
                if (i < K && levels > 2) {
                    const double l3 = (path == 0) ? q1y : (path == 1) ? q2x : (path == 2) ? q2y : q3x;
                    if (u < l3) { i = 2 * i; } else { u = u - l3; i = 2 * i + 1; }
                }
            }
            i = __builtin_amdgcn_readfirstlane(i);
        }
    }
    return i - K;
}
```

mvtopicmodel_amd/csrc/mvhdp_enqueue.hip:

```cpp
#include "mvhdp_ctx.h"

static hipError_t births_begin(mvhdp_ctx* h, hipStream_t s)
{
    const int K = h->mm.K;
    h->h_births.assign((size_t)2 + 2 * K, -1);
    int n = 0;
    for (int k = 0; k < K; k++) if (h->h_inactive[k]) { h->h_births[(size_t)2 + K + k] = n; h->h_births[(size_t)2 + n++] = k; }
    h->h_births[0] = 0; h->h_births[1] = n;
    h->h_birth_keys.assign((size_t)K, LLONG_MAX);
    hipError_t e = hipMemcpyAsync(h->d_births, h->h_births.data(), h->h_births.size() * sizeof(int32_t), hipMemcpyHostToDevice, s);
    if (e == hipSuccess) e = hipMemcpyAsync(h->d_birth_keys, h->h_birth_keys.data(), (size_t)K * sizeof(long long), hipMemcpyHostToDevice, s);
    return e;
}
int activate_born(mvhdp_ctx* h, const std::vector<std::pair<int32_t, long long>>& born, SweepOutcome& oc)
{
    if (born.empty()) return MVHDP_OK;
    MvModel& mm = h->mm;
    const int K = mm.K;
    for (const auto& b : born) {
        const int t = b.first, mv = MVHDP_ACT_KEY_VIEW(b.second);
        h->h_inactive[t] = 0;
        h->h_alpha[(size_t)mv * (K + 1) + t] = h->h_alpha[(size_t)mv * (K + 1) + K];
        if (oc.n_activations++ == 0) oc.first_act = b.second;
    }
// ... 79 lines not shown
static int alloc_debug(mvhdp_ctx* h, const mvhdp_debug* dbg, DebugBufs& db)
{
    const int K = h->mm.K, M = h->mm.M;
    hipStream_t s = h->stream;
    for (int m = 0; m < M; m++) {
        if (dbg->tok_dbg[m] && h->N[m] > 0) {
            void* p = nullptr;
            hipError_t e = hipMalloc(&p, (size_t)h->N[m] * 4 * sizeof(double));
            if (e != hipSuccess) { db.release(); HIPC(h, e); }
            db.to_free.push_back(p);
            hipMemsetAsync(p, 0, (size_t)h->N[m] * 4 * sizeof(double), s);
            db.tok_dbg[m] = (double*)p;
        }
    }
    if (dbg->n_trace > 0) {
        void *a = nullptr, *b = nullptr, *c = nullptr, *o = nullptr;
        const size_t n = (size_t)dbg->n_trace;
        if (hipMalloc(&a, n * 8) != hipSuccess || hipMalloc(&b, n * 4) != hipSuccess ||
            hipMalloc(&c, n * 4) != hipSuccess || hipMalloc(&o, n * (K + 1) * 8) != hipSuccess) {
            for (void* q : {a, b, c, o}) if (q) hipFree(q);
            db.release(); FAIL(h, MVHDP_ERR_HIP, "debug trace allocation failed");
        }
        db.to_free.push_back(a); db.to_free.push_back(b); db.to_free.push_back(c); db.to_free.push_back(o);
        hipMemcpyAsync(a, dbg->trace_doc, n * 8, hipMemcpyHostToDevice, s);
        hipMemcpyAsync(b, dbg->trace_view, n * 4, hipMemcpyHostToDevice, s);
        hipMemcpyAsync(c, dbg->trace_pos, n * 4, hipMemcpyHostToDevice, s);
        hipMemsetAsync(o, 0, n * (K + 1) * 8, s);
        db.n_trace = dbg->n_trace;
        db.trace_doc = (const int64_t*)a; db.trace_view = (const int32_t*)b; db.trace_pos = (const int32_t*)c;
        db.trace_out = (double*)o;
    }
    return MVHDP_OK;
}

static int64_t segment_share(int64_t P, int seg, int nseg) { return P > seg ? (P - seg + nseg - 1) / nseg : 0; }

struct SegCtl {
    unsigned int* class_counts;
    unsigned long long* qheads;
    int32_t* lists;
};

static hipError_t launch_segment_kernels(mvhdp_ctx* h, const SweepPlan& p, const MvModel& mk_in, const SweepLaunch& sl, int seg, hipStream_t s,
                                         const SegCtl& ctl, unsigned long long* d_stats)
{
    const MvModel& mm = h->mm;
    MvModel mk = mk_in;
    if (p.frozen) { mk.mix = nullptr; mk.mix32 = nullptr; }
    const int nseg = p.nseg;
    hipError_t e = hipSuccess;
    auto step = [&](hipError_t r) { if (e == hipSuccess) e = r; };
    auto share = [&](int64_t P) { return segment_share(P, seg, nseg); };
    const int64_t n_seg = share(mm.D);
    unsigned int* class_counts = ctl.class_counts;
    double tok_tot = 0;
    for (int b = 0; b < MVHDP_HIST_BINS; b++) tok_tot += (double)h->last_hist[b];
    const bool sizes_known = h->last_ent[MVHDP_N_CLASSES] == 0 && tok_tot > 0;
    auto blocks_for = [&](int64_t n, const ClassLaunch& g) {
        const int64_t need = (n + (int64_t)g.wpb * MVHDP_DOC_BATCH - 1) / ((int64_t)g.wpb * MVHDP_DOC_BATCH);
        return (int)std::max<int64_t>(1, std::min<int64_t>(need, g.grid));
    };
    {
        const int64_t H_seg = p.route ? share(p.H) : 0;
        ClassifyArgs ca{};
        int32_t* lists = ctl.lists ? ctl.lists : h->d_lists;
        bool used_stream[PLAN_N_STREAMS] = {};
        if (p.route && H_seg > 0) {
            if (!ctl.lists && !h->d_lists) step(hipMalloc(&h->d_lists, (size_t)MVHDP_N_CLASSES * mm.D * sizeof(int32_t)));
            lists = ctl.lists ? ctl.lists : h->d_lists;
            if (!h->ev_fork) step(hipEventCreateWithFlags(&h->ev_fork, hipEventDisableTiming));
            if (e != hipSuccess) return e;
            ca.order = h->d_doc_order; ca.n = H_seg; ca.start = seg; ca.stride = nseg;
            for (int c = 0; c < MVHDP_N_CLASSES; c++) { ca.class_map[c] = p.class_map[c]; ca.lists[c] = lists + (size_t)c * mm.D; }
            ca.check_views = compute_max_doc_tokens(h) > 65535 ? 1 : 0;
            ca.counts = class_counts;
            ca.misrouted = d_stats + ST_MISCLASS;
            step(mvhdp_launch_classify(mm, ca, s));
            step(hipEventRecord(h->ev_fork, s));
        }
        for (int c = MVHDP_N_CLASSES - 1; c >= p.pc && e == hipSuccess; c--) {
            const ClassLaunch& g = p.cls[c];
            if (!g.used) continue;
            if (c != p.pc && !(p.route && H_seg > 0)) continue;
            hipStream_t st = s;
            if (g.stream != PLAN_STREAM_MAIN && p.route && H_seg > 0) {
                const int si = g.stream;
                if (!h->side[si]) step(make_stream(&h->side[si], si != PLAN_STREAM_C && h->side_priority && !(h->side_priority == 2 && si == PLAN_STREAM_D)));
                if (!h->ev_join[si]) step(hipEventCreateWithFlags(&h->ev_join[si], hipEventDisableTiming));
                if (e != hipSuccess) return e;
                if (!used_stream[si]) step(hipStreamWaitEvent(h->side[si], h->ev_fork, 0));
                used_stream[si] = true;
                st = h->side[si];
            }
            if (c == p.pc && st == s) {
                bool side = false;
                for (int si = 1; si < PLAN_N_STREAMS; si++) side = side || used_stream[si];
                if (side) step(mvhdp_launch_delay(h->tu.fork_delay_us, s));
            }
            SweepLaunch sc = sl;
            sc.doc_counter = ctl.qheads + c;
            sc.wave_bytes = g.wave_bytes; sc.waves_per_block = g.wpb; sc.S_cap = g.S_cap;
            sc.walk = g.walk; sc.narrow = g.narrow;
            for (int m = 0; m < MVHDP_MAXM; m++) sc.walk_theta[m] = g.theta[m];
            int64_t n_c;
            if (c == p.pc) {
                if (p.route && H_seg > 0) { sc.q_list = ca.lists[c]; sc.q_list_count = class_counts + c; }
                sc.q_order = h->d_doc_order; sc.q_order_start = seg + H_seg * nseg; sc.q_order_stride = nseg; sc.q_order_count = n_seg - H_seg;
                n_c = n_seg;
            } else {
                sc.q_list = ca.lists[c]; sc.q_list_count = class_counts + c;
                sc.q_order = nullptr; sc.q_order_start = 0; sc.q_order_count = 0;
                n_c = H_seg;
                if (sizes_known) {
                    unsigned long long cnt = 0;
                    for (int q = 0; q < MVHDP_N_CLASSES; q++) if (p.class_map[q] == c) cnt += h->last_ent[q];
                    n_c = std::min<int64_t>(H_seg, (int64_t)(2 * cnt / (unsigned)nseg) + 64);
                }
            }
            if (g.fast) step(mvhdp_launch_sweep_fast(mk, sc, g.r, blocks_for(n_c, g), p.debug, st));
            else step(mvhdp_launch_sweep(mk, sc, blocks_for(n_c, g), p.debug, st));
        }
        for (int si = 1; si < PLAN_N_STREAMS; si++) if (used_stream[si]) step(hipEventRecord(h->ev_join[si], h->side[si]));
        for (int si = 1; si < PLAN_N_STREAMS; si++) if (used_stream[si]) step(hipStreamWaitEvent(s, h->ev_join[si], 0));
    }
    return e;
}


static SweepLaunch fill_launch(mvhdp_ctx* h, const SweepPlan& p, uint32_t sweep_idx, uint64_t seed, const DebugBufs* db, unsigned long long* d_stats)
{
    SweepLaunch sl{};
    sl.sweep_idx = sweep_idx; sl.seed_lo = (uint32_t)seed; sl.seed_hi = (uint32_t)(seed >> 32);
    sl.flags = p.flags & 0x7fffu; sl.S_cap = p.S_cap;
    if (h->tu.single_wave && p.live) sl.flags |= MVHDP_SL_STRICT_LIVE;
    if (p.live_rows && h->diag.no_row_sample) sl.flags |= MVHDP_SL_NO_ROW_SAMPLE;
#ifdef MVHDP_PROBE
    if (!p.overlap)
        if (const char* f = getenv("MVHDP_ATOMIC_PROBE")) sl.flags |= ((unsigned)atoi(f) & 7u) << 16;
#endif
    sl.q_order_stride = 1;
    sl.nk_global = p.nk_global; sl.block_shared_bytes = p.block_shared_bytes;
    sl.live16 = p.live16 ? 1 : 0; sl.delta16 = p.delta16 ? 1 : 0;
    sl.live_rows = p.live_rows ? 1 : 0; sl.coef_lds = p.coef_lds ? 1 : 0;
    sl.stats = d_stats; sl.act_key = h->d_act_key;
    if (sweep_births(p, p.flags, h->mm)) { sl.births = h->d_births; sl.birth_keys = h->d_birth_keys; }
    sl.slot_hist = (unsigned long long*)h->d_ovf_meta + META_HIST;
    if (db) {
        for (int m = 0; m < h->mm.M; m++) sl.tok_dbg[m] = db->tok_dbg[m];
        sl.n_trace = db->n_trace; sl.trace_doc = db->trace_doc; sl.trace_view = db->trace_view; sl.trace_pos = db->trace_pos; sl.trace_out = db->trace_out;
    }
    return sl;
}

static hipError_t view_weights(mvhdp_ctx* h, uint32_t sweep_idx, uint64_t seed, const double* p_override, hipStream_t s)
{
    MvModel& mm = h->mm;
    if (mm.M <= 1) return hipSuccess;
    const size_t bytes = (size_t)mm.D * mm.M * mm.M * sizeof(double);
    if (!mm.p && mm.D > 0) { hipError_t e = hipMalloc(&mm.p, bytes); if (e != hipSuccess) return e; }
    if (p_override) return hipMemcpyAsync(mm.p, p_override, bytes, hipMemcpyHostToDevice, s);
    return mvhdp_launch_draw_p(mm, sweep_idx, (uint32_t)seed, (uint32_t)(seed >> 32), s);
}

static bool uses_refresher(const mvhdp_ctx* h, const SweepPlan& p) { return p.live_rows && p.live16 && !h->tu.single_wave && !h->diag.no_heavy_refresh; }

static hipError_t ensure_heavy_list(mvhdp_ctx* h)
{
    if (h->d_heavy_list) return hipSuccess;
    const hipError_t e = hipMalloc(&h->d_heavy_list, (size_t)MVHDP_HEAVY_CAP * sizeof(int32_t));
    return e != hipSuccess ? e : hipMalloc(&h->d_heavy_ctl, 2 * sizeof(unsigned int));
}
static hipError_t ensure_refresher(mvhdp_ctx* h)
{
    if (h->rf_stream) return hipSuccess;
    hipError_t e = make_stream(&h->rf_stream, true);
    if (e == hipSuccess) e = hipEventCreateWithFlags(&h->ev_rf_go, hipEventDisableTiming);
    return e != hipSuccess ? e : hipEventCreateWithFlags(&h->ev_rf_done, hipEventDisableTiming);
}

static hipError_t live_rows_prepare(mvhdp_ctx* h, const SweepPlan& p, bool from_mirror, hipStream_t s)
{
    hipError_t e = p.live16 ? ensure_heavy_list(h) : hipSuccess;
    if (e == hipSuccess && uses_refresher(h, p)) e = ensure_refresher(h);
    if (e != hipSuccess) return e;
    return mvhdp_launch_live_rows_prepare(h->mm, from_mirror, p.live16, p.live16 ? h->d_heavy_list : nullptr, p.live16 ? h->d_heavy_ctl : nullptr, MVHDP_HEAVY_CAP,
                                          p.live16 ? 512 : 256 , s);
}

static hipError_t rebuild_trees(mvhdp_ctx* h, const SweepPlan& p, hipStream_t s)
{
    const hipError_t e = mvhdp_launch_build_trees(h->mm, false, p.need_full, s);
    h->have_trees = true; h->full_trees = p.need_full; h->trees_inference = false;
    return e;
}

static hipError_t trees_at_sweep_start(mvhdp_ctx* h, const SweepPlan& p, hipStream_t s)
{
    hipError_t e = hipSuccess, e2 = hipSuccess;
    h->last_need_full = p.need_full;
    if (p.live_rows) { e = live_rows_prepare(h, p, false, s); h->have_trees = false; h->full_trees = false; }
    else if (!(p.flags & MVHDP_SWEEP_REUSE_TREES)) e = rebuild_trees(h, p, s);
    if (p.need_full && !h->full_trees) { e2 = mvhdp_launch_build_trees(h->mm, h->trees_inference, true, s); h->full_trees = true; }
    return e != hipSuccess ? e : e2;
}

static hipError_t live_epilogue(mvhdp_ctx* h, const SweepPlan& p, unsigned long long* d_stats, hipStream_t s)
{
    MvModel& mm = h->mm;
    const bool no_apply = (p.flags & MVHDP_SWEEP_NO_APPLY) != 0;
    hipError_t e = hipSuccess;
    if (p.live16 && mm.D > 0) { e = mvhdp_launch_widen_mirror(mm, s); h->have_trees = false; }
    const hipError_t e2 = mvhdp_launch_live_helper(mm, no_apply ? 1 : 2, d_stats, s);
    if (p.nseg > 1 && !(p.flags & MVHDP_SWEEP_REUSE_TREES) && (no_apply || p.overlap)) h->have_trees = false;
    return e != hipSuccess ? e : e2;
}

static int ensure_overlap_buffers(mvhdp_ctx* h, const SweepPlan& p)
{
    MvModel& mm = h->mm;
    const int64_t nrows = mm.rowbase[mm.M];
    const size_t cbytes = (size_t)(counts_len(h) + MVHDP_TAIL_WORDS) * sizeof(int32_t);
    auto& ov = h->ov;
    if (!ov.x1) HIPC(h, hipStreamCreateWithFlags(&ov.x1, hipStreamNonBlocking));
    if (!ov.ev_start) HIPC(h, hipEventCreateWithFlags(&ov.ev_start, hipEventDisableTiming));
    while (ov.ev_seg.size() < (size_t)3 * p.nseg) { hipEvent_t ev; HIPC(h, hipEventCreateWithFlags(&ev, hipEventDisableTiming)); ov.ev_seg.push_back(ev); }
    if (p.live) {
        if (!ov.dtab2) HIPC(h, hipMalloc(&ov.dtab2, (size_t)nrows * mm.dt_nblk * 8 * sizeof(double)));
        if (!ov.root2) HIPC(h, hipMalloc(&ov.root2, (size_t)nrows * sizeof(double)));
        if (p.need_full && !ov.trees2) HIPC(h, hipMalloc(&ov.trees2, (size_t)nrows * 2 * mm.K * sizeof(double)));
    }
    if (!ov.ctl2) { HIPC(h, hipMalloc(&ov.ctl2, 16 * sizeof(unsigned long long))); HIPC(h, hipMemset(ov.ctl2, 0, 16 * sizeof(unsigned long long))); }
    if (p.route && !ov.lists2 && mm.D > 0) HIPC(h, hipMalloc(&ov.lists2, (size_t)MVHDP_N_CLASSES * mm.D * sizeof(int32_t)));
    if (p.seg_apply) {
        if (!ov.counts2) HIPC(h, hipMalloc(&ov.counts2, cbytes));
        if (!ov.counts16_2) HIPC(h, hipMalloc(&ov.counts16_2, (size_t)nrows * mm.K * sizeof(uint16_t)));
        if (!ov.delta2) { HIPC(h, hipMalloc(&ov.delta2, cbytes)); HIPC(h, hipMemset(ov.delta2, 0, cbytes)); }
        if (!ov.delta3) { HIPC(h, hipMalloc(&ov.delta3, cbytes)); HIPC(h, hipMemset(ov.delta3, 0, cbytes)); }
    }
    return MVHDP_OK;
}

static int enqueue_overlapped(mvhdp_ctx* h, const SweepPlan& p, uint32_t sweep_idx, uint64_t seed, const double* p_override,
                              unsigned long long* d_stats, hipEvent_t ev_k0, hipEvent_t ev_k1)
{
    MvModel& mm = h->mm;
    const int M = mm.M, nseg = p.nseg;
    const uint32_t flags = p.flags;
    if (p.live_rows || p.coef_lds || p.debug || sweep_births(p, flags, mm) || p.only_seg >= 0)
        FAIL(h, MVHDP_ERR_HIP, "internal: overlapped segments planned together with live rows, debug outputs, births or a single segment");
    int rc = ensure_overlap_buffers(h, p); if (rc) return rc;
    auto& ov = h->ov;
    hipStream_t X[2] = {h->stream, h->diag.overlap_serial ? h->stream : ov.x1};
    hipError_t e = hipSuccess;
    auto step = [&](hipError_t r) { if (e == hipSuccess) e = r; };
    const int64_t clen = counts_len(h), nrows = mm.rowbase[M];
    const size_t cbytes = (size_t)clen * sizeof(int32_t);

    const SweepLaunch sl = fill_launch(h, p, sweep_idx, seed, nullptr, d_stats);
    step(view_weights(h, sweep_idx, seed, p_override, X[0]));
    bool use_mirror = false;
    for (int c = 0; c < MVHDP_N_CLASSES; c++) use_mirror = use_mirror || (p.cls[c].used && p.cls[c].narrow);
    step(trees_at_sweep_start(h, p, X[0]));
    MvModel B[2] = {mm, mm};
    if (p.live) { B[1].dtab = ov.dtab2; B[1].root = ov.root2; if (ov.trees2) B[1].trees = ov.trees2; }
    int32_t* D3[3] = {mm.delta, ov.delta2, ov.delta3};
    if (p.seg_apply) {
        B[1].counts = ov.counts2; B[1].counts16 = ov.counts16_2;
        step(hipMemcpyAsync(ov.counts2, mm.counts, cbytes, hipMemcpyDeviceToDevice, X[0]));
        step(hipMemcpyAsync(ov.counts16_2, mm.counts16, (size_t)nrows * mm.K * sizeof(uint16_t), hipMemcpyDeviceToDevice, X[0]));
        if (!h->delta_clean) step(hipMemsetAsync(mm.delta, 0, cbytes, X[0]));
        h->delta_clean = false;
        if (ov.deltas_dirty) { step(hipMemsetAsync(ov.delta2, 0, cbytes, X[0])); step(hipMemsetAsync(ov.delta3, 0, cbytes, X[0])); }
        ov.deltas_dirty = true;
    } else if (flags & MVHDP_SWEEP_NO_APPLY) {
        step(mvhdp_launch_live_helper(mm, 0, d_stats, X[0])); h->delta_clean = false;
    }
    SegCtl ctl[2] = {{h->d_ovf_meta + META_CLASS_COUNTS, h->d_doc_counter, nullptr}, {(unsigned int*)(ov.ctl2 + 8), ov.ctl2, ov.lists2}};
    step(mvhdp_launch_ctl_reset(d_stats, ST_COUNT, h->d_act_key, (unsigned long long*)h->d_ovf_meta, META_WORDS64, nullptr, nullptr, X[0]));
    step(hipEventRecord(ev_k0, X[0]));
    step(hipEventRecord(ov.ev_start, X[0]));
    step(hipStreamWaitEvent(X[1], ov.ev_start, 0));
    auto ev_done = [&](int s) { return ov.ev_seg[(size_t)3 * s]; };
    auto ev_applied = [&](int s) { return ov.ev_seg[(size_t)3 * s + 1]; };
    auto ev_reset = [&](int s) { return ov.ev_seg[(size_t)3 * s + 2]; };

    for (int seg = 0; seg < nseg && e == hipSuccess && mm.D > 0; seg++) {
        hipStream_t xs = X[seg & 1];
        const SegCtl& cs = ctl[seg & 1];
        MvModel mk;
        if (p.seg_apply) {
            mk = B[seg == 0 ? 0 : (seg - 1) & 1];
            mk.delta = D3[seg % 3];
        } else {
            mk = mm;
            mk.delta = mm.counts;
            mk.dtab = B[seg & 1].dtab; mk.root = B[seg & 1].root; mk.trees = B[seg & 1].trees;
            if (seg >= 1 && !(flags & MVHDP_SWEEP_REUSE_TREES)) {
                step(hipStreamWaitEvent(xs, ev_reset(seg - 1), 0));
                const int64_t n_prev = segment_share(mm.D, seg - 1, nseg), H_prev = p.route ? segment_share(p.H, seg - 1, nseg) : 0;
                const unsigned long long thr = (unsigned long long)((n_prev - H_prev) * h->gate_pct / 100);
                step(mvhdp_launch_gate(ctl[(seg - 1) & 1].qheads + p.pc, thr, xs));
                MvModel tm = mm;
                tm.dtab = mk.dtab; tm.root = mk.root; tm.trees = mk.trees;
                if (p.live16) step(mvhdp_launch_build_trees_from_mirror(tm, p.need_full, xs, true));
                else step(mvhdp_launch_build_trees(tm, false, p.need_full, xs, true));
            } else if (seg >= 1) {
                mk.dtab = mm.dtab; mk.root = mm.root; mk.trees = mm.trees;
            }
        }
        step(mvhdp_launch_ctl_reset(nullptr, 0, nullptr, nullptr, 0, cs.class_counts, cs.qheads, xs));
        step(hipEventRecord(ev_reset(seg), xs));
        step(launch_segment_kernels(h, p, mk, sl, seg, xs, cs, d_stats));
        step(hipEventRecord(ev_done(seg), xs));
        if (p.seg_apply) {
            if (seg >= 1) step(hipStreamWaitEvent(xs, ev_applied(seg - 1), 0));
            const MvModel& dst = B[(seg + 1) & 1];
            step(mvhdp_launch_apply2_counts(dst, D3[seg % 3], seg >= 1 ? D3[(seg - 1) % 3] : nullptr, use_mirror, d_stats + ST_NEGATIVE, xs));
            step(hipEventRecord(ev_applied(seg), xs));
        }
    }
    if (mm.D > 0 && e == hipSuccess) {
        step(hipStreamWaitEvent(X[0], p.seg_apply ? ev_applied(nseg - 1) : ev_done(nseg - 1), 0));
        if (nseg >= 2) step(hipStreamWaitEvent(X[0], ev_done(nseg - 2), 0));
        if (p.seg_apply) {
            step(mvhdp_launch_apply_sparse(B[(nseg + 1) & 1], D3[(nseg - 1) % 3], use_mirror, X[0]));
            h->have_trees = false;
        }
    }
    if (p.live) step(live_epilogue(h, p, d_stats, X[0]));
    step(hipEventRecord(ev_k1, X[0]));
    if (e != hipSuccess) HIPC(h, e);
    return MVHDP_OK;
}

static int enqueue_sweep(mvhdp_ctx* h, const SweepPlan& p, uint32_t sweep_idx, uint64_t seed, const double* p_override,
                         const DebugBufs* db, unsigned long long* d_stats, hipEvent_t ev_k0, hipEvent_t ev_k1, SweepOutcome& oc)
{
    if (p.overlap) return enqueue_overlapped(h, p, sweep_idx, seed, p_override, d_stats, ev_k0, ev_k1);
    MvModel& mm = h->mm;
    const int M = mm.M, nseg = p.nseg;
    const uint32_t flags = p.flags;
    hipStream_t s = h->stream;
    hipError_t e = hipSuccess;
    auto step = [&](hipError_t r) { if (e == hipSuccess) e = r; };

    const SweepLaunch sl = fill_launch(h, p, sweep_idx, seed, db, d_stats);
    const bool births = sl.births != nullptr;
    unsigned int* class_counts = h->d_ovf_meta + META_CLASS_COUNTS;
    step(view_weights(h, sweep_idx, seed, p_override, s));
    const bool refresher = uses_refresher(h, p);
    step(trees_at_sweep_start(h, p, s));
    MvModel mk = mm;
    if (p.live) {
        mk.delta = mm.counts;
        if (flags & MVHDP_SWEEP_NO_APPLY) { step(mvhdp_launch_live_helper(mm, 0, d_stats, s)); h->delta_clean = false; }
    } else if (!p.frozen) {
        if (!h->delta_clean) {
            step(hipMemsetAsync(mm.delta, 0, (size_t)counts_len(h) * sizeof(int32_t), s));
            if (h->delta16_used) step(hipMemsetD16Async(mm.delta16, (unsigned short)0x8000, (size_t)(mm.rowbase[M] * mm.K), s));
            h->delta16_used = false;
        }
        h->delta_clean = false;
        if (p.delta16) h->delta16_used = true;
    }
    step(mvhdp_launch_ctl_reset(d_stats, ST_COUNT, h->d_act_key, (unsigned long long*)h->d_ovf_meta, META_WORDS64, nullptr, h->d_doc_counter, s));
    if (births) step(births_begin(h, s));
    step(hipEventRecord(ev_k0, s));

    const int seg_lo = p.only_seg >= 0 ? p.only_seg : 0, seg_hi = p.only_seg >= 0 ? p.only_seg + 1 : nseg;
    for (int seg = seg_lo; seg < seg_hi && e == hipSuccess && mm.D > 0; seg++) {
        if (seg > seg_lo) {
            if (births && !(flags & MVHDP_SWEEP_NO_APPLY) && e == hipSuccess) {
                const int rc = births_end(h, s, oc);
                if (rc != MVHDP_OK) return rc;
                mk.first_inactive = mm.first_inactive;
                step(births_begin(h, s));
                step(mvhdp_launch_ctl_reset(nullptr, 0, h->d_act_key, nullptr, 0, nullptr, nullptr, s));
            } else
            if ((p.live || p.seg_apply) && !(flags & MVHDP_SWEEP_NO_APPLY) && mm.first_inactive >= 0 && e == hipSuccess) {
                long long key = LLONG_MAX;
                step(hipMemcpyAsync(&key, h->d_act_key, sizeof key, hipMemcpyDeviceToHost, s));
                step(hipStreamSynchronize(s));
                if (e == hipSuccess && key != LLONG_MAX) {
                    const int rc = apply_activation(h, MVHDP_ACT_KEY_TOPIC(key), MVHDP_ACT_KEY_VIEW(key));
                    if (rc != MVHDP_OK) return rc;
                    if (oc.n_activations++ == 0) oc.first_act = key;
                    mk.first_inactive = mm.first_inactive;
                    step(mvhdp_launch_ctl_reset(nullptr, 0, h->d_act_key, nullptr, 0, nullptr, nullptr, s));
                }
            }
            if (p.seg_apply) {
                step(mvhdp_launch_apply_nk(mm, d_stats + ST_NEGATIVE, s));
                step(mvhdp_launch_build_trees_rows(mm, false, p.need_full, 0, mm.rowbase[M], true, d_stats + ST_NEGATIVE, s));
                h->have_trees = true; h->full_trees = p.need_full; h->trees_inference = false;
            } else if (p.live_rows) {
                step(live_rows_prepare(h, p, p.live16, s));
            } else if (p.live && !(flags & MVHDP_SWEEP_REUSE_TREES) && (h->live_tree_every <= 1 || seg % h->live_tree_every == 0)) {
                if (p.live16) {
                    step(mvhdp_launch_build_trees_from_mirror(mm, p.need_full, s));
                    h->have_trees = true; h->full_trees = p.need_full; h->trees_inference = false;
                } else step(rebuild_trees(h, p, s));
            }
            step(mvhdp_launch_ctl_reset(nullptr, 0, nullptr, nullptr, 0, class_counts, h->d_doc_counter, s));
        }
        if (e != hipSuccess) break;
        if (refresher) {
            step(hipEventRecord(h->ev_rf_go, s));
            step(hipStreamWaitEvent(h->rf_stream, h->ev_rf_go, 0));
            step(mvhdp_launch_heavy_refresh(mm, h->d_heavy_list, h->d_heavy_ctl, MVHDP_HEAVY_CAP, MVHDP_REFRESH_BLOCKS, h->rf_stream));
            step(hipEventRecord(h->ev_rf_done, h->rf_stream));
        }
        step(launch_segment_kernels(h, p, mk, sl, seg, s, SegCtl{class_counts, h->d_doc_counter, nullptr}, d_stats));
        if (refresher) {
            hipError_t e2 = mvhdp_launch_set_u32(h->d_heavy_ctl + 1, 1u, s);
            if (e2 == hipSuccess) e2 = hipStreamWaitEvent(s, h->ev_rf_done, 0);
            step(e2);
        }
    }
    if (p.seg_apply && mm.D > 0) {
        step(mvhdp_launch_apply_delta(mm, d_stats, s));
        h->have_trees = false;
    }
    if (p.live) step(live_epilogue(h, p, d_stats, s));
    step(hipEventRecord(ev_k1, s));
    if (e != hipSuccess) HIPC(h, e);
    return MVHDP_OK;
}

static void stats_from_counters(const unsigned long long* hs, long long act, mvhdp_sweep_stats& st)
{
    st = mvhdp_sweep_stats{};
    st.tokens = (int64_t)hs[ST_TOKENS]; st.changed = (int64_t)hs[ST_CHANGED];
    st.new_mass_cnt = (int64_t)hs[ST_NEW]; st.topic_doc_mass_cnt = (int64_t)hs[ST_DOC];
    st.word_ftree_mass_cnt = (int64_t)hs[ST_TREE]; st.oov_skipped = (int64_t)hs[ST_OOV];
    st.aborted_docs = (int64_t)hs[ST_ABORT]; st.exact_fallbacks = (int64_t)hs[ST_FALLBACK];
    st.activation_key = act;
    st.activated_topic = -1; st.activated_modality = -1;
    if (act != LLONG_MAX) { st.activated_topic = MVHDP_ACT_KEY_TOPIC(act); st.activated_modality = MVHDP_ACT_KEY_VIEW(act); }
}

static void learn_from_sweep(mvhdp_ctx* h, const SweepPlan& p, const unsigned long long* hs, const unsigned long long* meta_hist, double kernel_ms, bool comparable)
{
    const MvModel& mm = h->mm;
    bool any_walk = false;
    for (int c = 0; c < MVHDP_N_CLASSES; c++) any_walk = any_walk || (p.cls[c].used && p.cls[c].walk);
    WalkTuner& wt = walk_tuner_of(h, p.flags);
    if (any_walk) wt.measured(mm.M, p.nseg, hs + ST_VIEW_BASE);
    if (mm.D > 0 && p.only_seg >= 0) {
        if (meta_hist[MVHDP_HIST_BINS + MVHDP_N_CLASSES] != 0) h->nslots_valid = false;
    } else if (mm.D > 0) {
        std::copy(meta_hist, meta_hist + MVHDP_HIST_BINS, h->last_hist);
        std::copy(meta_hist + MVHDP_HIST_BINS, meta_hist + MVHDP_HIST_BINS + MVHDP_ENT_BINS, h->last_ent);
        h->nslots_valid = h->last_ent[MVHDP_N_CLASSES] == 0;
    }
    if (h->dbg_env) {
        fprintf(stderr, "[mvhdp] walk threshold %.2f (base %.2f, phase %d, dir %+d, group %d); tree branch %.4f of tokens, walked on demand %.4f; per view tree share:",
                (double)wt.walk_probe_i / MVHDP_WALK_BINS, (double)wt.walk_i / MVHDP_WALK_BINS, wt.walk_phase, wt.walk_dir, wt.walk_cls,
                (double)hs[ST_TREE] / std::max<double>(1.0, (double)hs[ST_TOKENS]), (double)hs[ST_ONDEMAND] / std::max<double>(1.0, (double)hs[ST_TOKENS]));
        for (int m = 0; m < mm.M; m++) {
            const double n = std::max<double>(1.0, (double)hs[ST_VIEW_BASE + m * MVHDP_VIEW_STATS]);
            fprintf(stderr, " %.3f", hs[ST_VIEW_BASE + m * MVHDP_VIEW_STATS + 1] / n);
        }
        fprintf(stderr, "\n");
        if (hs[ST_T_TOTAL])
            fprintf(stderr, "[mvhdp] wave cycles: queue %.1f%% prologue %.1f%% view setup %.1f%% chunk head %.1f%% tokens %.1f%% chunk end %.1f%% | %.0f cycles per token per wave\n",
                    100.0 * hs[ST_T_QUEUE] / hs[ST_T_TOTAL], 100.0 * hs[ST_T_PROLOGUE] / hs[ST_T_TOTAL], 100.0 * hs[ST_T_VIEW] / hs[ST_T_TOTAL],
                    100.0 * hs[ST_T_CHUNK_HEAD] / hs[ST_T_TOTAL], 100.0 * hs[ST_T_TOKENS] / hs[ST_T_TOTAL], 100.0 * hs[ST_T_CHUNK_END] / hs[ST_T_TOTAL],
                    (double)hs[ST_T_TOTAL] / std::max<double>(1.0, (double)hs[ST_TOKENS]));
        if (hs[ST_T_ROWS])
            fprintf(stderr, "[mvhdp] live rows: %.0f cycles per tree-branch token, %.0f of them until the row is there (%.1f%% of the waves' time; %llu such tokens)\n",
                    (double)hs[ST_T_ROWS] / std::max<double>(1.0, (double)hs[ST_ONDEMAND]), (double)hs[ST_T_ROWS_WAIT] / std::max<double>(1.0, (double)hs[ST_ONDEMAND]),
                    100.0 * hs[ST_T_ROWS] / hs[ST_T_TOTAL], hs[ST_ONDEMAND]);
        if (hs[ST_N_WAVES])
            fprintf(stderr, "[mvhdp] cycles per token in a wave's first / second / later entities: %.0f / %.0f / %.0f (tokens %llu / %llu / %llu); per wave: block init %.0f cycles, wait + flush at the end %.0f, whole wave %.0f\n",
                    (double)hs[ST_T_ENT0] / std::max<double>(1.0, (double)hs[ST_N_ENT0]), (double)hs[ST_T_ENT1] / std::max<double>(1.0, (double)hs[ST_N_ENT1]),
                    (double)hs[ST_T_ENT2] / std::max<double>(1.0, (double)hs[ST_N_ENT2]), hs[ST_N_ENT0], hs[ST_N_ENT1], hs[ST_N_ENT2],
                    (double)hs[ST_T_INIT] / hs[ST_N_WAVES], (double)hs[ST_T_FLUSH] / hs[ST_N_WAVES], (double)hs[ST_T_TOTAL] / hs[ST_N_WAVES]);
    }
    const double tokens = (double)hs[ST_TOKENS];
    wt.observe(comparable && tokens > 0, p.walk_cfg, mm.M, tokens > 0 ? kernel_ms * 1e6 / tokens : 0.0);
}

static void debug_print_plan(const mvhdp_ctx* h, const SweepPlan& p, uint32_t sweep_idx)
{
    double tot = 0, b1 = 0, b2 = 0;
    for (int b = 0; b < MVHDP_HIST_BINS; b++) { tot += (double)h->last_hist[b]; if (b < 1) b1 += (double)h->last_hist[b]; if (b < 2) b2 += (double)h->last_hist[b]; }
    fprintf(stderr, "[mvhdp] sweep %u: %s primary class %d, routed prefix %lld, S_cap %d, %d segment(s); tokens in lists <=64: %.4f <=128: %.4f; kernels:",
            sweep_idx, p.fast ? "register-resident" : "generic", p.pc, (long long)p.H, p.S_cap, p.nseg, b1 / std::max(1.0, tot), b2 / std::max(1.0, tot));
    for (int c = 0; c < MVHDP_N_CLASSES; c++)
        if (p.cls[c].used)
            fprintf(stderr, " [class %d %s grid %d wpb %d lds %zu stream %d%s%s theta0 %.2f ents %llu]", c, p.cls[c].fast ? "fast" : "generic", p.cls[c].grid, p.cls[c].wpb, p.cls[c].lds,
                    p.cls[c].stream, p.cls[c].walk ? " walk" : "", p.cls[c].narrow == 2 ? " slim" : p.cls[c].narrow ? " narrow" : "", p.cls[c].theta[0], (unsigned long long)h->last_ent[c]);
    fprintf(stderr, "\n");
}

static int sweep_preconditions(mvhdp_ctx* h, uint32_t flags)
{
    if ((flags & MVHDP_SWEEP_SHARD_BIRTHS) && (!(flags & MVHDP_SWEEP_LIVE) || (flags & MVHDP_SWEEP_FROZEN) || (flags >> 24) != 0))
        FAIL(h, MVHDP_ERR_INVALID_ARG, "sweep: SHARD_BIRTHS goes with LIVE, not with FROZEN or ONLY_SEGMENT");
    int rc = require_corpus(h); if (rc) return rc;
    if (!h->have_hyper) FAIL(h, MVHDP_ERR_STATE, "sweep before set_hyper");
    if (!h->have_counts) FAIL(h, MVHDP_ERR_STATE, "sweep before build_counts/set_counts");
    if ((flags & (MVHDP_SWEEP_REUSE_TREES | MVHDP_SWEEP_FROZEN)) && !h->have_trees) FAIL(h, MVHDP_ERR_STATE, "REUSE_TREES / FROZEN without trees");
    if (h->rows_applied >= 0) FAIL(h, MVHDP_ERR_STATE, "sweep: an mvhdp_apply_delta_begin bracket is open (call mvhdp_apply_delta_end)");
    if (h->delta_pending && !(flags & MVHDP_SWEEP_FROZEN))
        FAIL(h, MVHDP_ERR_STATE, "sweep: the previous NO_APPLY sweep's deltas have not been applied (mvhdp_apply_delta)");
    if (h->counts_stale && !(flags & MVHDP_SWEEP_FROZEN))
        FAIL(h, MVHDP_ERR_STATE, "sweep: the assignments were replaced after the counts were built (call mvhdp_build_counts, mvhdp_set_counts or mvhdp_counts_written first)");
    return MVHDP_OK;
}

static int set_generic_lds(mvhdp_ctx* h, const SweepPlan& p)
{
    size_t lds = 0;
    for (int c = 0; c < MVHDP_N_CLASSES; c++) if (p.cls[c].used && !p.cls[c].fast) lds = std::max(lds, p.cls[c].lds);
    if (lds > 65536 && lds > h->lds_attr_set) { HIPC(h, mvhdp_sweep_set_max_lds(lds)); h->lds_attr_set = lds; }
    return MVHDP_OK;
}

static int plan_checked(mvhdp_ctx* h, uint32_t sweep_idx, uint32_t flags, bool debug, bool batch, SweepPlan& p)
{
    int rc = sweep_preconditions(h, flags); if (rc) return rc;
    HIPC(h, hipSetDevice(h->device));
    rc = ensure_slot_counts(h); if (rc) return rc;
    PlanIn in; fill_plan_in(h, flags, debug, batch, in);
    plan_sweep(in, h->tu, walk_tuner_of(h, flags), p);
    if (p.err) FAIL(h, p.err, p.msg);
    rc = set_generic_lds(h, p); if (rc) return rc;
    if (h->dbg_env) debug_print_plan(h, p, sweep_idx);
    return MVHDP_OK;
}

int mvhdp_sweep_begin(mvhdp_ctx* h, uint32_t sweep_idx, uint64_t seed, uint32_t flags, const double* p_override, const mvhdp_debug* dbg, PendingSweep& ps)
{
    ps.flags = flags; ps.dbg = dbg; ps.debug = dbg != nullptr; ps.oc = SweepOutcome();
    int rc = plan_checked(h, sweep_idx, flags, ps.debug, false, ps.p); if (rc) return rc;
    hipStream_t s = h->stream;
    if (ps.debug) { rc = alloc_debug(h, dbg, ps.db); if (rc) return rc; }
    HIPC(h, hipEventRecord(h->ev[0], s));
    ps.births = sweep_births(ps.p, flags, h->mm);
    rc = enqueue_sweep(h, ps.p, sweep_idx, seed, p_override, ps.debug ? &ps.db : nullptr, h->d_stats, h->ev[1], h->ev[2], ps.oc);
    if (rc) { ps.db.release(); return rc; }
    hipError_t e = hipSuccess;
    if ((flags & MVHDP_SWEEP_NO_APPLY) && !ps.p.frozen)
        e = mvhdp_launch_birth_table(ps.births ? h->d_births : nullptr, h->d_birth_keys, h->d_act_key, h->mm.K, h->d_birth_table, s);
    if (e == hipSuccess) e = hipMemcpyAsync(h->h_ctl, h->d_ctl, (ST_COUNT + 1 + META_WORDS64) * sizeof(unsigned long long), hipMemcpyDeviceToHost, s);
    if (e != hipSuccess) { ps.db.release(); HIPC(h, e); }
    ps.open = true;
    return MVHDP_OK;
}

int mvhdp_sweep_finish(mvhdp_ctx* h, PendingSweep& ps, mvhdp_sweep_stats* stats)
{
    if (!ps.open) FAIL(h, MVHDP_ERR_STATE, "sweep_finish without sweep_begin");
    ps.open = false;
    MvModel& mm = h->mm;
    const SweepPlan& p = ps.p;
    const uint32_t flags = ps.flags;
    HIPC(h, hipSetDevice(h->device));
    hipStream_t s = h->stream;
    hipError_t e = hipStreamSynchronize(s);
    if (e != hipSuccess) { ps.db.release(); HIPC(h, e); }
    const unsigned long long* hs = h->h_ctl;
    const long long act = (long long)h->h_ctl[ST_COUNT];
    const unsigned long long* meta = h->h_ctl + ST_COUNT + 1;
    if (hs[ST_MISCLASS] || meta[META_MISROUTED]) {
        ps.db.release();
        h->nslots_valid = false;
        FAIL(h, MVHDP_ERR_HIP, "internal: an entity reached a sweep kernel variant that cannot hold its topic list");
    }
    if (ps.debug) {
        const mvhdp_debug* dbg = ps.dbg;
        for (int m = 0; m < mm.M; m++)
            if (ps.db.tok_dbg[m] && e == hipSuccess) e = hipMemcpy(dbg->tok_dbg[m], ps.db.tok_dbg[m], (size_t)h->N[m] * 4 * sizeof(double), hipMemcpyDeviceToHost);
        if (ps.db.n_trace > 0 && e == hipSuccess) e = hipMemcpy(dbg->trace_out, ps.db.trace_out, (size_t)ps.db.n_trace * (mm.K + 1) * sizeof(double), hipMemcpyDeviceToHost);
        ps.db.release();
        if (e != hipSuccess) HIPC(h, e);
    }

    mvhdp_sweep_stats st;
    stats_from_counters(hs, act, st);
    if (!p.frozen && p.only_seg < 0 && st.aborted_docs == 0) for (int m = 0; m < mm.M; m++) h->unassigned[m] = false;
    const unsigned long long negatives = hs[ST_NEGATIVE];
    unsigned long long hist_keep[MVHDP_HIST_BINS + MVHDP_ENT_BINS];
    std::copy(meta + META_HIST, meta + META_HIST + MVHDP_HIST_BINS + MVHDP_ENT_BINS, hist_keep);
    unsigned long long hs_keep[ST_COUNT];
    std::copy(hs, hs + ST_COUNT, hs_keep);
    int n_activations = ps.oc.n_activations;
    int ret = MVHDP_OK;
    if (p.frozen) {
    } else if (flags & MVHDP_SWEEP_NO_APPLY) {
        h->delta_pending = true;
    } else if (p.live || p.seg_apply) {
        h->have_trees = false;
        if (p.seg_apply) h->delta_clean = true;
        if (p.seg_apply && p.overlap) h->ov.deltas_dirty = false;
        if (ps.births) {
            ret = births_end(h, s, ps.oc);
            n_activations = ps.oc.n_activations;
        } else {
            ret = apply_activation(h, st.activated_topic, st.activated_modality);
            if (st.activated_topic >= 0) n_activations++;
        }
        if (ps.oc.first_act != LLONG_MAX) {
            st.activation_key = ps.oc.first_act;
            st.activated_topic = MVHDP_ACT_KEY_TOPIC(ps.oc.first_act); st.activated_modality = MVHDP_ACT_KEY_VIEW(ps.oc.first_act);
        }
        if (ret == MVHDP_OK && negatives) { h->err = "a topic count went below zero (UPD:202-215)"; ret = MVHDP_ERR_NEGATIVE_COUNT; }
    } else {
        if (st.activated_topic >= 0) n_activations = 1;
        ret = mvhdp_apply_delta(h, st.activated_topic, st.activated_modality);
    }
    HIPC(h, hipEventRecord(h->ev[3], s));
    HIPC(h, hipEventSynchronize(h->ev[3]));
    float ms_k = 0, ms_t = 0;
    hipEventElapsedTime(&ms_k, h->ev[1], h->ev[2]);
    hipEventElapsedTime(&ms_t, h->ev[0], h->ev[3]);
    st.sweep_kernel_ms = ms_k; st.total_ms = ms_t;
    st.activations = n_activations; st.reserved = 0;
    const bool comparable = p.fast && !ps.debug && !h->tu.walk_fixed && !(flags & (MVHDP_SWEEP_FROZEN | MVHDP_SWEEP_EXACT_CHAIN));
    learn_from_sweep(h, p, hs_keep, hist_keep, ms_k, comparable);
    if (stats) *stats = st;
    return ret;
}

extern "C" int mvhdp_sweep(mvhdp_handle h, uint32_t sweep_idx, uint64_t seed, uint32_t flags,
                           const double* p_override, const mvhdp_debug* dbg, mvhdp_sweep_stats* stats)
{
    CHECK_H(h);
    PendingSweep ps;
    const int rc = mvhdp_sweep_begin(h, sweep_idx, seed, flags, p_override, dbg, ps);
    if (rc) return rc;
    return mvhdp_sweep_finish(h, ps, stats);
}

extern "C" int mvhdp_sweep_many(mvhdp_handle h, uint32_t first_idx, int32_t n, uint64_t seed, uint32_t flags, mvhdp_sweep_stats* stats)
{
    CHECK_H(h);
    if (n < 0) FAIL(h, MVHDP_ERR_INVALID_ARG, "sweep_many: n < 0");
    if (n == 0) return MVHDP_OK;
    MvModel& mm = h->mm;
    const bool frozen = (flags & MVHDP_SWEEP_FROZEN) != 0;
    if (n == 1 || mm.first_inactive >= 0 || ((flags & MVHDP_SWEEP_NO_APPLY) && !frozen) || ((flags & MVHDP_SWEEP_REUSE_TREES) && !frozen) || n > 4096) {
        for (int i = 0; i < n; i++) {
            const int rc = mvhdp_sweep(h, first_idx + (uint32_t)i, seed, flags, nullptr, nullptr, stats ? stats + i : nullptr);
            if (rc) return rc;
        }
        return MVHDP_OK;
    }
    SweepPlan p;
    int rc = plan_checked(h, first_idx, flags, false, true, p); if (rc) return rc;
    hipStream_t s = h->stream;
    if (h->stats_many_cap < n) {
        if (h->d_stats_many) { hipFree(h->d_stats_many); h->d_stats_many = nullptr; h->stats_many_cap = 0; }
        HIPC(h, hipMalloc(&h->d_stats_many, (size_t)n * ST_COUNT * sizeof(unsigned long long)));
        h->stats_many_cap = n;
    }
    while ((int)h->ev_many.size() < 2 * n) { hipEvent_t ev; HIPC(h, hipEventCreate(&ev)); h->ev_many.push_back(ev); }
    HIPC(h, hipEventRecord(h->ev[0], s));
    for (int i = 0; i < n; i++) {
        SweepOutcome oc;
        unsigned long long* d_st = h->d_stats_many + (size_t)i * ST_COUNT;
        rc = enqueue_sweep(h, p, first_idx + (uint32_t)i, seed, nullptr, nullptr, d_st, h->ev_many[2 * i], h->ev_many[2 * i + 1], oc);
        if (rc) return rc;
        if (!p.frozen && !p.live && !p.seg_apply) {
            HIPC(h, mvhdp_launch_apply_delta(mm, d_st, s, h->delta16_used));
            h->delta16_used = false;
            h->have_trees = false; h->delta_clean = true;
        } else if (p.live || p.seg_apply) {
            h->have_trees = false;
            if (p.seg_apply) h->delta_clean = true;
        }
    }
    HIPC(h, hipEventRecord(h->ev[3], s));
    std::vector<unsigned long long> hs((size_t)n * ST_COUNT);
    unsigned long long meta[META_WORDS64] = {0};
    HIPC(h, hipMemcpyAsync(hs.data(), h->d_stats_many, hs.size() * sizeof(unsigned long long), hipMemcpyDeviceToHost, s));
    HIPC(h, hipMemcpyAsync(meta, h->d_ovf_meta, sizeof meta, hipMemcpyDeviceToHost, s));
    HIPC(h, hipStreamSynchronize(s));
    if (p.seg_apply && p.overlap) h->ov.deltas_dirty = false;
    float ms_t = 0;
    hipEventElapsedTime(&ms_t, h->ev[0], h->ev[3]);
    int ret = MVHDP_OK;
    double ms_sum = 0;
    for (int i = 0; i < n; i++) {
        const unsigned long long* hi = hs.data() + (size_t)i * ST_COUNT;
        mvhdp_sweep_stats st;
        stats_from_counters(hi, LLONG_MAX, st);
        float ms_k = 0;
        hipEventElapsedTime(&ms_k, h->ev_many[2 * i], h->ev_many[2 * i + 1]);
        st.sweep_kernel_ms = ms_k; st.total_ms = ms_t / n;
        ms_sum += ms_k;
        if (stats) stats[i] = st;
        if (hi[ST_MISCLASS]) { h->nslots_valid = false; FAIL(h, MVHDP_ERR_HIP, "internal: an entity reached a sweep kernel variant that cannot hold its topic list"); }
        if (hi[ST_NEGATIVE] && ret == MVHDP_OK) { h->err = "a topic count went below zero (UPD:202-215)"; ret = MVHDP_ERR_NEGATIVE_COUNT; }
    }
    if (meta[META_MISROUTED]) { h->nslots_valid = false; FAIL(h, MVHDP_ERR_HIP, "internal: an entity could not be routed to a sweep kernel"); }
    std::vector<unsigned long long> acc(ST_COUNT, 0);
    for (int i = 0; i < n; i++) for (int k = 0; k < ST_COUNT; k++) acc[k] += hs[(size_t)i * ST_COUNT + k];
    const bool comparable = p.fast && !h->tu.walk_fixed && !(flags & (MVHDP_SWEEP_FROZEN | MVHDP_SWEEP_EXACT_CHAIN));
    learn_from_sweep(h, p, acc.data(), meta + META_HIST, ms_sum, comparable);
    if (!p.frozen && acc[ST_ABORT] == 0) for (int m = 0; m < mm.M; m++) h->unassigned[m] = false;
    return ret;
}
```

mvtopicmodel_amd/csrc/mvhdp_kernels.hip:

```cpp
#include "mvhdp_device.h"
#include "mvhdp_slim.h"
#include "../../include/mvhdp.h"

#include "mvhdp_wave.h"
#include <algorithm>

__global__ __launch_bounds__(256) void build_counts_kernel(MvModel mm, int m, int64_t n_tokens)
{
    extern __shared__ int nk_local[];
    const int K = mm.K;
    for (int i = threadIdx.x; i < K; i += blockDim.x) nk_local[i] = 0;
    __syncthreads();
    int32_t* nwk = mm.counts;
    const int64_t stride = (int64_t)gridDim.x * blockDim.x;
    for (int64_t i = (int64_t)blockIdx.x * blockDim.x + threadIdx.x; i < n_tokens; i += stride) {
        int topic = mm.z[m][i];
        if (topic == MVHDP_UNASSIGNED_TOPIC) continue;
        int type = mm.tok[m][i];
        if (type < 0 || type >= mm.V[m] || topic < 0 || topic >= K) continue;
        atomicAdd(&nk_local[topic], 1);
        atomicAdd(&nwk[(mm.rowbase[m] + type) * K + topic], 1);
    }
    __syncthreads();
    int32_t* nk = mm.counts + mm.rowbase[mm.M] * K + (int64_t)m * K;
    for (int i = threadIdx.x; i < K; i += blockDim.x)
        if (nk_local[i]) atomicAdd(&nk[i], nk_local[i]);
}

hipError_t mvhdp_launch_build_counts(const MvModel& mm, const int64_t* n_tokens, hipStream_t s)
{
    const int K = mm.K;
    size_t total = (size_t)(mm.rowbase[mm.M] * K + (int64_t)mm.M * K) * sizeof(int32_t);
    hipError_t e = hipMemsetAsync(mm.counts, 0, total, s);
    if (e != hipSuccess) return e;
    for (int m = 0; m < mm.M; m++) {
        if (n_tokens[m] <= 0) continue;
        int64_t blocks = (n_tokens[m] + 255) / 256;
        int grid = (int)(blocks < 2048 ? blocks : 2048);
        hipLaunchKernelGGL(build_counts_kernel, dim3(grid), dim3(256), (size_t)K * sizeof(int), s, mm, m, n_tokens[m]);
        e = hipGetLastError();
        if (e != hipSuccess) return e;
    }
    return hipSuccess;
}

template <bool COHERENT = false>
__device__ __forceinline__ void tree_from_leaves(const MvModel& mm, int64_t row, double* t, int lane, bool write_full)
{
    const int K = mm.K;
    if (lane == 0) t[0] = 0.0;
    __syncthreads();
    if (K > 1) {
        int dmax = 31 - __clz(K - 1);
        for (int d = dmax; d >= 0; d--) {
            int lo = 1 << d, hi = min(2 << d, K);
            for (int i = lo + lane; i < hi; i += WAVE) t[i] = t[2 * i] + t[2 * i + 1];
            __syncthreads();
        }
    }
    if (write_full) {
        double* out = mm.trees + row * 2 * K;
        for (int i = lane; i < 2 * K; i += WAVE) out[i] = t[i];
    }
    if (lane == 0) { if (COHERENT) __hip_atomic_store(&mm.root[row], t[1], __ATOMIC_RELAXED, __HIP_MEMORY_SCOPE_AGENT); else mm.root[row] = t[1]; }
    double* dt = mm.dtab + row * (int64_t)mm.dt_nblk * 8;
    double2* o = (double2*)dt;
    for (int u = lane; u < mm.dt_nblk * 4; u += WAVE) {
        const int x = u >> 2, j = u & 3;
        int base = 0, dep = 0;
        if (x >= 1) {
            base = 1; dep = mm.dt_f;
            while (x >= base + (1 << dep)) { base += 1 << dep; dep += 3; }
        }
        const int b = (1 << dep) + (x - base);
        double v2[2];
#pragma unroll
        for (int h = 0; h < 2; h++) {
            const int q = 2 * j + h;
            const int node = (q == 0) ? b : (q < 3) ? 2 * b + (q - 1) : 4 * b + (q - 3);
            v2[h] = (q == 7) ? ((x == 0) ? t[1] : 0.0) : ((node < K) ? t[2 * node] : 0.0);
        }
        if (COHERENT) {
            __hip_atomic_store(&dt[2 * u], v2[0], __ATOMIC_RELAXED, __HIP_MEMORY_SCOPE_AGENT);
            __hip_atomic_store(&dt[2 * u + 1], v2[1], __ATOMIC_RELAXED, __HIP_MEMORY_SCOPE_AGENT);
        } else o[u] = make_double2(v2[0], v2[1]);
    }
    __syncthreads();
}

template <int TB, bool MIX = false>
__global__ __launch_bounds__(64) void build_trees_kernel(MvModel mm, bool inference_leaves, bool write_full, int64_t row_begin, int64_t row_end,
                                                         bool apply_first, unsigned long long* negatives, bool from_mirror, bool only_heavy = false)
{
    extern __shared__ double t[];
    const int K = mm.K, lane = threadIdx.x;
    const int64_t nrows = mm.rowbase[mm.M];
    const int32_t* nk_all = mm.counts + nrows * K;
    int neg = 0;
    __builtin_amdgcn_s_setprio(3);
    for (int64_t row = row_begin + blockIdx.x; row < row_end; row += gridDim.x) {
        if (only_heavy && MVHDP_ROW_CLASS(mm.heavy[row]) != MVHDP_ROW_HEAVY) continue;
        int m = 0;
        while (m + 1 < mm.M && row >= mm.rowbase[m + 1]) m++;
        int32_t* cnt = mm.counts + row * K;
        int32_t* dl = mm.delta + row * K;
        const int32_t* nk = nk_all + (int64_t)m * K;
        const double* al = mm.alpha + (int64_t)m * (K + 1);
        const double beta = mm.beta[m], beta_sum = mm.beta_sum[m], gamma = mm.gamma[m];
        uint16_t* c16 = mm.counts16 + row * K;
        const bool light_src = from_mirror && MVHDP_ROW_CLASS(mm.heavy[row]) != MVHDP_ROW_HEAVY;
        const bool mixed = MIX && m == 0 && !inference_leaves;
        const double* mixrow = mixed ? mm.mix + row * K : nullptr;
        bool hv = false, slim = false;
        if (!from_mirror) {
            long long sum = 0;
            int big = 0;
            for (int k0 = 0; k0 < K; k0 += WAVE * TB) {
                int cv[TB], dv[TB];
#pragma unroll
                for (int u = 0; u < TB; u++) {
                    const int k = k0 + u * WAVE + lane;
                    cv[u] = (k < K) ? cnt[k] : 0;
                    dv[u] = (apply_first && k < K) ? dl[k] : 0;
                }
#pragma unroll
                for (int u = 0; u < TB; u++) {
                    const int k = k0 + u * WAVE + lane;
                    if (k < K) {
                        int c = cv[u];
                        if (apply_first) {
                            const int d = dv[u];
                            if (d) { c += d; cnt[k] = c; dl[k] = 0; neg += c < 0; }
                        }
                        sum += c < 0 ? 70000 : c;
                        big = max(big, c < 0 ? 70000 : c);
                    }
                }
            }
#pragma unroll
            for (int sft = 32; sft >= 1; sft >>= 1) { sum += __shfl_xor(sum, sft, WAVE); big = max(big, __shfl_xor(big, sft, WAVE)); }
            hv = sum > 65534;
            slim = mm.counts12 != nullptr && big <= MVHDP_SLIM_MAX;
            if (lane == 0) mm.heavy[row] = (uint8_t)((hv ? MVHDP_ROW_HEAVY : (sum > 32767 ? MVHDP_ROW_BIG : 0)) | (slim ? MVHDP_ROW_SLIM : 0));
        }
        for (int k0 = 0; k0 < K; k0 += WAVE * TB) {
            int cv[TB], nkv[TB];
            double alv[TB], mxv[TB];
            bool inact[TB];
#pragma unroll
            for (int u = 0; u < TB; u++) {
                const int k = k0 + u * WAVE + lane;
                const bool in = k < K;
                mxv[u] = (MIX && mixed && in) ? mixrow[k] : 0.0;
                cv[u] = in ? (light_src ? (int)c16[k] : cnt[k]) : 0;
                nkv[u] = in ? nk[k] : 0;
                alv[u] = (in && !inference_leaves) ? al[k] : 0.0;
                inact[u] = in && !inference_leaves && mm.inactive[k];
            }
#pragma unroll
            for (int u = 0; u < TB; u++) {
                const int k = k0 + u * WAVE + lane;
                if (k < K) {
                    const int c = cv[u];
                    if (light_src) cnt[k] = c;
                    else if (!from_mirror) c16[k] = hv ? (uint16_t)65535 : (uint16_t)c;
                    if (slim) ((int*)t)[k] = c;
                    double leaf;
                    if (inference_leaves) {
                        leaf = ((double)c + beta) / ((double)nkv[u] + beta_sum);
                    } else if (inact[u]) {
                        leaf = 0.0;
                    } else {
                        double p_wt = ((double)c + beta) / ((double)nkv[u] + beta_sum);
                        if (MIX && mixed) p_wt = mxv[u] + mm.oml * p_wt;
                        leaf = gamma * alv[u] * p_wt;
                    }
                    t[K + k] = leaf;
                }
            }
        }
        if (slim) {
            __syncthreads();
            const int* cs = (const int*)t;
            unsigned int* out12 = (unsigned int*)(mm.counts12 + (size_t)row * mvhdp_slim_row_bytes(K));
            const int nwords = (int)(mvhdp_slim_row_bytes(K) >> 2);
            for (int w = lane; w < nwords; w += WAVE) {
                const int j = w >> 5, bit0 = (w & 31) * 32;
                unsigned int v = 0;
#pragma unroll
                for (int q = 0; q < 4; q++) {
                    const int i = bit0 / 12 + q, k = j * MVHDP_SLIM_CELLS + i, sh = 12 * i - bit0;
                    if (i < MVHDP_SLIM_CELLS && k < K && sh < 32) { const unsigned int c = (unsigned int)cs[k]; v |= sh >= 0 ? c << sh : c >> -sh; }
                }
                out12[w] = v;
            }
            __syncthreads();
        }
        tree_from_leaves(mm, row, t, lane, write_full);
    }
    if (apply_first && negatives) {
#pragma unroll
        for (int sft = 32; sft >= 1; sft >>= 1) neg += __shfl_xor(neg, sft, WAVE);
        if (lane == 0 && neg) atomicAdd(negatives, (unsigned long long)neg);
    }
}

static hipError_t launch_trees(int tb, const MvModel& mm, bool inference_leaves, bool write_full, int64_t row_begin, int64_t row_end,
                               bool apply_first, unsigned long long* negatives, bool from_mirror, hipStream_t s, bool only_heavy = false)
{
    const int64_t nrows = row_end - row_begin;
    if (nrows <= 0) return hipSuccess;
    const bool mix = mm.mix != nullptr;
    const void* f = tb == 1 ? (mix ? (const void*)build_trees_kernel<1, true> : (const void*)build_trees_kernel<1, false>)
                  : tb == 4 ? (mix ? (const void*)build_trees_kernel<4, true> : (const void*)build_trees_kernel<4, false>)
                  : tb == 8 ? (mix ? (const void*)build_trees_kernel<8, true> : (const void*)build_trees_kernel<8, false>) : nullptr;
    if (!f) return hipErrorInvalidValue;
    void* args[] = {(void*)&mm, &inference_leaves, &write_full, &row_begin, &row_end, &apply_first, &negatives, &from_mirror, &only_heavy};
    (void)hipLaunchKernel(f, dim3((unsigned)(nrows < 65536 ? nrows : 65536)), dim3(64), args, (size_t)2 * mm.K * sizeof(double), s);
    return hipGetLastError();
}

hipError_t mvhdp_launch_build_trees(const MvModel& mm, bool inference_leaves, bool write_full, hipStream_t s, bool beside_samplers)
{
    if (!beside_samplers) return mvhdp_launch_build_trees_rows(mm, inference_leaves, write_full, 0, mm.rowbase[mm.M], false, nullptr, s);
    return launch_trees(1, mm, inference_leaves, write_full, 0, mm.rowbase[mm.M], false, nullptr, false, s);
}

hipError_t mvhdp_launch_build_trees_rows(const MvModel& mm, bool inference_leaves, bool write_full, int64_t row_begin, int64_t row_end,
                                         bool apply_first, unsigned long long* negatives, hipStream_t s)
{
    return launch_trees(mm.K > 512 ? 8 : 4, mm, inference_leaves, write_full, row_begin, row_end, apply_first, negatives, false, s);
}

hipError_t mvhdp_launch_build_trees_from_mirror(const MvModel& mm, bool write_full, hipStream_t s, bool beside_samplers)
{
    return launch_trees(beside_samplers ? 1 : mm.K > 512 ? 8 : 4, mm, false, write_full, 0, mm.rowbase[mm.M], false, nullptr, true, s);
}

__global__ __launch_bounds__(256) void apply2_nk_kernel(int32_t* nk_dst, const int32_t* __restrict__ dA, int32_t* __restrict__ dB, int n, unsigned long long* negatives)
{
    const int i = blockIdx.x * blockDim.x + threadIdx.x;
    if (i >= n) return;
    int d = dA[i];
    if (dB) { const int d2 = dB[i]; if (d2) { d += d2; dB[i] = 0; } }
    if (d) { const int c = nk_dst[i] + d; nk_dst[i] = c; if (c < 0 && negatives) atomicAdd(negatives, 1ull); }
}

__global__ __launch_bounds__(256) void apply2_counts_kernel(MvModel mm, const int32_t* __restrict__ dA, int32_t* __restrict__ dB, bool use_mirror,
                                                           int64_t n_cells, int64_t n_all, unsigned long long* negatives)
{
    const int64_t stride = (int64_t)gridDim.x * blockDim.x;
    unsigned int* m32 = (unsigned int*)mm.counts16;
    const int K = mm.K;
    int neg = 0;
    __builtin_amdgcn_s_setprio(3);
    for (int64_t i = (int64_t)blockIdx.x * blockDim.x + threadIdx.x; i < n_all; i += stride) {
        int d = dA[i];
        if (dB) { const int d2 = dB[i]; if (d2) { d += d2; dB[i] = 0; } }
        if (!d) continue;
        const int old = __hip_atomic_fetch_add(&mm.counts[i], d, __ATOMIC_RELAXED, __HIP_MEMORY_SCOPE_AGENT);
        neg += old + d < 0;
        if (use_mirror && i < n_cells && MVHDP_ROW_CLASS(mm.heavy[i / K]) != MVHDP_ROW_HEAVY) __hip_atomic_fetch_add(&m32[i >> 1], (unsigned int)d << ((i & 1) * 16), __ATOMIC_RELAXED, __HIP_MEMORY_SCOPE_AGENT);
    }
    if (neg && negatives) atomicAdd(negatives, (unsigned long long)neg);
}

hipError_t mvhdp_launch_apply2_counts(const MvModel& dst, const int32_t* dA, int32_t* dB, bool use_mirror, unsigned long long* negatives, hipStream_t s)
{
    const int64_t cells = dst.rowbase[dst.M] * dst.K, all = cells + (int64_t)dst.M * dst.K;
    int grid = (int)std::min<int64_t>((all + 255) / 256, 4096);
    if (grid < 1) grid = 1;
    hipLaunchKernelGGL(apply2_counts_kernel, dim3(grid), dim3(256), 0, s, dst, dA, dB, use_mirror, cells, all, negatives);
    return hipGetLastError();
}

__global__ __launch_bounds__(256) void apply_sparse_kernel(MvModel mm, int32_t* __restrict__ d, bool use_mirror, int64_t n_cells, int64_t n_all)
{
    const int64_t stride = (int64_t)gridDim.x * blockDim.x;
    unsigned int* m32 = (unsigned int*)mm.counts16;
    const int K = mm.K;
    for (int64_t i = (int64_t)blockIdx.x * blockDim.x + threadIdx.x; i < n_all; i += stride) {
        const int dl = d[i];
        if (!dl) continue;
        mm.counts[i] += dl;
        d[i] = 0;
        if (use_mirror && i < n_cells && MVHDP_ROW_CLASS(mm.heavy[i / K]) != MVHDP_ROW_HEAVY) __hip_atomic_fetch_add(&m32[i >> 1], (unsigned int)dl << ((i & 1) * 16), __ATOMIC_RELAXED, __HIP_MEMORY_SCOPE_AGENT);
    }
}

hipError_t mvhdp_launch_apply_sparse(const MvModel& dst, int32_t* d, bool use_mirror, hipStream_t s)
{
    const int64_t cells = dst.rowbase[dst.M] * dst.K, all = cells + (int64_t)dst.M * dst.K;
    int grid = (int)std::min<int64_t>((all + 255) / 256, 8192);
    if (grid < 1) grid = 1;
    hipLaunchKernelGGL(apply_sparse_kernel, dim3(grid), dim3(256), 0, s, dst, d, use_mirror, cells, all);
    return hipGetLastError();
}

__global__ __launch_bounds__(64) void gate_kernel(const unsigned long long* qhead, unsigned long long threshold)
{
    const unsigned long long t0 = __builtin_amdgcn_s_memrealtime();
    for (int i = 0; i < 4000000; i++) {
        const unsigned long long v = __hip_atomic_load(qhead, __ATOMIC_RELAXED, __HIP_MEMORY_SCOPE_AGENT);
        if (v >= threshold) break;
        if (__builtin_amdgcn_s_memrealtime() - t0 > 200000000ull) break;
        __builtin_amdgcn_s_sleep(32);
    }
}

hipError_t mvhdp_launch_gate(const unsigned long long* qhead, unsigned long long threshold, hipStream_t s)
{
    hipLaunchKernelGGL(gate_kernel, dim3(1), dim3(64), 0, s, qhead, threshold);
    return hipGetLastError();
}

__global__ __launch_bounds__(256) void widen_mirror_kernel(MvModel mm)
{
    const int K = mm.K;
    const int64_t nrows = mm.rowbase[mm.M];
    const int lane = threadIdx.x & 63;
    const int64_t wstride = (int64_t)gridDim.x * (blockDim.x >> 6);
    for (int64_t row = (int64_t)blockIdx.x * (blockDim.x >> 6) + (threadIdx.x >> 6); row < nrows; row += wstride) {
        if (MVHDP_ROW_CLASS(mm.heavy[row]) == MVHDP_ROW_HEAVY) continue;
        const uint16_t* c16 = mm.counts16 + row * K;
        int32_t* cnt = mm.counts + row * K;
        for (int k = lane; k < K; k += WAVE) cnt[k] = (int)c16[k];
    }
}

hipError_t mvhdp_launch_widen_mirror(const MvModel& mm, hipStream_t s)
{
    const int64_t nrows = mm.rowbase[mm.M];
    if (nrows <= 0) return hipSuccess;
    int64_t blocks = (nrows + 3) / 4;
    hipLaunchKernelGGL(widen_mirror_kernel, dim3((unsigned int)(blocks < 16384 ? blocks : 16384)), dim3(256), 0, s, mm);
    return hipGetLastError();
}

__global__ __launch_bounds__(64) void live_coef_kernel(MvModel mm)
{
    const int K = mm.K, Kp = (K + 7) & ~7, m = blockIdx.x;
    const int32_t* nk = mm.counts + mm.rowbase[mm.M] * K + (int64_t)m * K;
    float* cf = mm.coef + (int64_t)m * Kp;
    float* smp = mm.coef + (int64_t)mm.M * Kp + (int64_t)m * K;
    for (int k = threadIdx.x; k < Kp; k += blockDim.x)
        cf[k] = (k >= K || mm.inactive[k]) ? 0.0f : (float)(mm.gamma[m] * mm.alpha[(int64_t)m * (K + 1) + k] / ((double)nk[k] + mm.beta_sum[m]));
    __syncthreads();
    if (threadIdx.x == 0) {
        const float beta32 = (float)mm.beta[m];
        float run = 0.0f;
        for (int k = 0; k < K; k++) { run += cf[k] * beta32; smp[k] = run; }
    }
}

template <int TB>
__global__ __launch_bounds__(64) void live_rows_prepare_kernel(MvModel mm, bool from_mirror, int32_t* heavy_list, unsigned int* heavy_n, int heavy_cap, int batch_cells)
{
    const int K = mm.K, lane = threadIdx.x;
    const int64_t nrows = mm.rowbase[mm.M];
    for (int64_t row = blockIdx.x; row < nrows; row += gridDim.x) {
        int m = 0;
        while (m + 1 < mm.M && row >= mm.rowbase[m + 1]) m++;
        const int32_t* cnt = mm.counts + row * K;
        uint16_t* c16 = mm.counts16 + row * K;
        const int Kp = (K + 7) & ~7;
        const float* cf = mm.coef + (int64_t)m * Kp;
        const float smp_total = mm.coef[(int64_t)mm.M * Kp + (int64_t)m * K + K - 1];
        const bool light_src = from_mirror && MVHDP_ROW_CLASS(mm.heavy[row]) != MVHDP_ROW_HEAVY;
        bool hv = false;
        if (!from_mirror) {
            long long sum = 0;
            for (int k0 = 0; k0 < K; k0 += WAVE * TB) {
                int cv[TB];
#pragma unroll
                for (int u = 0; u < TB; u++) { const int k = k0 + u * WAVE + lane; cv[u] = (k < K) ? cnt[k] : 0; }
#pragma unroll
                for (int u = 0; u < TB; u++) sum += cv[u] < 0 ? 70000 : cv[u];
            }
#pragma unroll
            for (int sft = 32; sft >= 1; sft >>= 1) sum += __shfl_xor(sum, sft, WAVE);
            hv = sum > 65534;
            if (lane == 0) mm.heavy[row] = hv ? MVHDP_ROW_HEAVY : (sum > 32767 ? MVHDP_ROW_BIG : 0);
        }
        double acc = 0.0, acc0 = 0.0;
// ... 923 lines not shown
```

mvtopicmodel_amd/native.py:

```python
import atexit
import ctypes as C
import sys
import weakref
from dataclasses import dataclass, field

import numpy as np

from ._lib import (DIAG_MAX_TOP_WORDS, DIAG_PROPORTIONS, DIAG_ROWS, MAX_M, UNIQUE_ID_BYTES, Config, DebugC, DiagArgsC, DiagOutC,
                   EmbConfigC, EmbStatsC, GroupInfoC, HyperC, MvhdpError, SimArgsC, SimStatsC, SweepStatsC, TuningC, load_library,
                   SIM_COS, SIM_COS_FOLDED, SIM_JSD)

SWEEP_REUSE_TREES = 0x1
SWEEP_NO_APPLY = 0x2
SWEEP_EXACT_CHAIN = 0x4
SWEEP_GENERIC_KERNEL = 0x8
SWEEP_FROZEN = 0x10
SWEEP_LIVE = 0x20
SWEEP_SEGMENT_APPLY = 0x40
SWEEP_SEGMENT_OVERLAP = 0x80
SWEEP_ASYNC_EXCHANGE = 0x100
SWEEP_SHARD_BIRTHS = 0x200


def SWEEP_LIVE_SEGMENTS(n):
    return (int(n) & 0xFF) << 16

def SWEEP_ONLY_SEGMENT(s):
    return ((int(s) + 1) & 0xFF) << 24


EMB_SERIAL = 0x1

BUF_COUNTS = 0
BUF_DELTA = 1
BUF_BIRTH_KEYS = 2
BUF_COUNTS12 = 3
BUF_ROW_CLASS = 4
ACT_KEY_NONE = (1 << 63) - 1


def _ptr(a):
    return None if a is None else a.ctypes.data_as(C.c_void_p)


_live = weakref.WeakSet()


@atexit.register
def _close_all():
    for s in list(_live):
        try:
            s.close()
        except Exception:
            pass


@dataclass
class Hyper:
    alpha: np.ndarray
    alpha_sum: np.ndarray
    beta: np.ndarray
    beta_sum: np.ndarray
    gamma: np.ndarray
    p_a: np.ndarray
    p_b: np.ndarray
    inactive: np.ndarray = None

    @staticmethod
    def defaults(K, V, alpha=0.1, beta=0.01, p_a=0.31, p_b=1.0, inactive=None):
        M = len(V)
        return Hyper(alpha=np.full((M, K + 1), alpha, dtype=np.float64),
                     alpha_sum=np.full(M, K * alpha, dtype=np.float64),
                     beta=np.full(M, beta, dtype=np.float64),
                     beta_sum=np.array([beta * v for v in V], dtype=np.float64),
                     gamma=np.ones(M, dtype=np.float64),
                     p_a=np.full((M, M), p_a, dtype=np.float64),
                     p_b=np.full((M, M), p_b, dtype=np.float64),
                     inactive=None if inactive is None else np.asarray(inactive, dtype=np.uint8))


@dataclass
class SweepStats:
    tokens: int = 0
    changed: int = 0
    new_mass_cnt: int = 0
    topic_doc_mass_cnt: int = 0
    word_ftree_mass_cnt: int = 0
    oov_skipped: int = 0
    aborted_docs: int = 0
    exact_fallbacks: int = 0
    activated_topic: int = -1
    activated_modality: int = -1
    activation_key: int = 0
    sweep_kernel_ms: float = 0.0
    total_ms: float = 0.0
    activations: int = 0
    reserved: int = 0
    dbg: list = field(default=None, repr=False)
    trace: np.ndarray = field(default=None, repr=False)


@dataclass
class SimStats:
    pairs_screened: int = 0
    candidates: int = 0
    emitted: int = 0
    stripes: int = 0
    regrown: int = 0
    margin: float = 0.0


SIM_METRICS = {"cos_folded": SIM_COS_FOLDED, "cos": SIM_COS, "jsd": SIM_JSD}


def _sim_stats(c):
    return SimStats(**{f: getattr(c, f) for f, _ in SimStatsC._fields_})


def sim_probe(n, dim, stripe_rows=0):
    st = SimStatsC()
    rc = load_library().mvhdp_sim_probe(int(n), int(dim), int(stripe_rows), C.byref(st))
    if rc != 0:
        raise MvhdpError(rc, "sim_probe: bad shape" if rc == -1 else "sim_probe: dim > 65536")
    return _sim_stats(st)


def round_similarity(sim):
    return np.floor(np.asarray(sim, dtype=np.float64) * 1000 + 0.5) / 1000


@dataclass
class EmbConfig:
    num_columns: int = 200
    num_context_columns: int = 50
    with_topics: bool = True
    window: int = 5
    num_samples: int = 5
    min_doc_length: int = 10
    sampling_table_size: int = 100_000_000
    sampling_factor: float = 1e-4
    min_exp: float = -6.0
    max_exp: float = 6.0
    sigmoid_cache_size: int = 1000

    @staticmethod
    def defaults(with_topics=True, **kw):
        kw.setdefault("num_context_columns", 50 if with_topics else 0)
        return EmbConfig(with_topics=bool(with_topics), **kw)

    def to_c(self):
        return EmbConfigC(int(self.num_columns), int(self.num_context_columns), int(bool(self.with_topics)), int(self.window),
                          int(self.num_samples), int(self.min_doc_length), int(self.sampling_table_size), float(self.sampling_factor),
                          float(self.min_exp), float(self.max_exp), int(self.sigmoid_cache_size), 0)


@dataclass
class EmbStats:
    words_so_far: int = 0
    words_sampled: int = 0
    words_considered: int = 0
    docs_skipped: int = 0
    calls: int = 0
    negatives_skipped: int = 0
    residual: float = 0.0
    last_epoch_residual: float = 0.0
    last_epoch_calls: int = 0
    kernel_ms: float = 0.0


def java_string_lengths(vocabulary):
    return np.array([len(str(w).encode("utf-16-le")) // 2 for w in vocabulary], dtype=np.int32)


@dataclass
class Diagnostics:
    scores: dict
    word_scores: dict
    codoc: np.ndarray
    top_words: np.ndarray
    top_counts: np.ndarray
    nonzero: np.ndarray
    num_rank1_docs: np.ndarray
    num_nonzero_docs: np.ndarray
    num_docs_at_proportions: np.ndarray
    sum_count_log_count: np.ndarray
    word_type_counts: np.ndarray
    num_tokens: int
    discr_weight_per_view: np.ndarray


# ... 594 lines not shown
```

Measured before the change: 6.966 billion.

## Fuse delta apply with tree rebuild and draw next sweep's view weights ahead

After a plain deferred sweep, the count delta (including the 16-bit delta) is applied inside the tree-building kernel. That kernel writes the next sweep's row-class and slim tables into spare buffers, which are swapped in at the next sweep start instead of rebuilding trees. Next-sweep view weights are also drawn on a side stream while the current sweep runs. The host event synchronize in the finish path is skipped for fused sweeps. This removes a separate apply pass, a tree rebuild and a serialized weight draw, at the cost of extra device buffers and more state-tracking complexity.

Result: no change. 6.936 billion, median of 2 (-0.4%).

```diff
diff --git a/include/mvhdp.h b/include/mvhdp.h
--- a/include/mvhdp.h
+++ b/include/mvhdp.h
@@ -104,7 +104,11 @@
     MVHDP_BUF_DELTA  = 1,
     MVHDP_BUF_BIRTH_KEYS = 2,
     MVHDP_BUF_COUNTS12 = 3,
-    MVHDP_BUF_ROW_CLASS = 4
+    MVHDP_BUF_ROW_CLASS = 4,
+    MVHDP_BUF_COUNTS16 = 5,
+    MVHDP_BUF_DESCENT = 6,
+    MVHDP_BUF_ROOTS = 7,
+    MVHDP_BUF_COUNTS12_AHEAD = 8, MVHDP_BUF_ROW_CLASS_AHEAD = 9
 } mvhdp_buffer;
 
 int mvhdp_create(const mvhdp_config* cfg, mvhdp_handle* out);
diff --git a/mvtopicmodel_amd/csrc/mvhdp_ahead.h b/mvtopicmodel_amd/csrc/mvhdp_ahead.h
--- /dev/null
+++ b/mvtopicmodel_amd/csrc/mvhdp_ahead.h
@@ -0,0 +1,40 @@
+#pragma once
+#include <cstdint>
+
+enum { MVHDP_AHEAD_TREES = 1, MVHDP_AHEAD_WEIGHTS = 2, MVHDP_AHEAD_ALL = 3 };
+
+struct AheadSweep {
+    bool frozen, no_apply, live, seg_apply, reuse_trees, only_segment, debug;
+    bool inactive_topics;
+    bool vectors_mix;
+};
+
+static inline bool mvhdp_plain_deferred(const AheadSweep& s)
+{
+    return !s.frozen && !s.no_apply && !s.live && !s.seg_apply && !s.reuse_trees && !s.only_segment && !s.debug && !s.vectors_mix;
+}
+
+static inline bool mvhdp_fuses_update(int ahead_mode, const AheadSweep& s)
+{
+    return (ahead_mode & MVHDP_AHEAD_TREES) != 0 && mvhdp_plain_deferred(s) && !s.inactive_topics;
+}
+
+static inline bool mvhdp_ahead_trees_usable(bool left_ahead, int ahead_mode, const AheadSweep& s)
+{
+    return left_ahead && mvhdp_fuses_update(ahead_mode, s);
+}
+
+struct AheadWeightsTag {
+    bool valid;
+    uint32_t sweep_idx;
+    uint64_t seed;
+    int64_t D, doc_id_base;
+    uint64_t gen;
+};
+
+static inline bool mvhdp_ahead_weights_usable(const AheadWeightsTag& drawn, const AheadWeightsTag& call, bool p_override, int ahead_mode, const AheadSweep& s)
+{
+    return drawn.valid && call.valid && !p_override && (ahead_mode & MVHDP_AHEAD_WEIGHTS) != 0 && mvhdp_plain_deferred(s) &&
+           drawn.sweep_idx == call.sweep_idx && drawn.seed == call.seed && drawn.D == call.D && drawn.doc_id_base == call.doc_id_base &&
+           drawn.gen == call.gen;
+}
diff --git a/mvtopicmodel_amd/csrc/mvhdp_api.hip b/mvtopicmodel_amd/csrc/mvhdp_api.hip
--- a/mvtopicmodel_amd/csrc/mvhdp_api.hip
+++ b/mvtopicmodel_amd/csrc/mvhdp_api.hip
@@ -60,10 +60,37 @@
         for (; m < MVHDP_MAXM; m++) h->tu.walk_theta[m] = 0.0;
         h->tu.walk_fixed = 1;
     }
+    if (const char* f = getenv("MVHDP_AHEAD")) h->ahead.mode = atoi(f) & MVHDP_AHEAD_ALL;
     h->dbg_env = getenv("MVHDP_DEBUG") != nullptr;
     h->diag.overlap_serial = getenv("MVHDP_OVERLAP_SERIAL") != nullptr;
     h->diag.no_row_sample = getenv("MVHDP_NO_ROW_SAMPLE") != nullptr;
     h->diag.no_heavy_refresh = getenv("MVHDP_NO_HEAVY_REFRESH") != nullptr;
+}
+
+void mvhdp_ahead_drop_weights(mvhdp_ctx* h)
+{
+    auto& a = h->ahead;
+    if (a.stream) hipStreamSynchronize(a.stream);
+    if (a.p_next) { hipFree(a.p_next); a.p_next = nullptr; }
+    a.tag = AheadWeightsTag{};
+    a.gen++;
+}
+
+bool mvhdp_ahead_row_tables(mvhdp_ctx* h)
+{
+    auto& a = h->ahead;
+    const MvModel& mm = h->mm;
+    const size_t nrows = (size_t)mm.rowbase[mm.M], b12 = nrows * mvhdp_slim_row_bytes(mm.K);
+    if (a.heavy_next && (a.counts12_next || !mm.counts12)) return true;
+    bool ok = a.heavy_next || (hipMalloc(&a.heavy_next, nrows) == hipSuccess && hipMemset(a.heavy_next, 1, nrows) == hipSuccess);
+    if (ok && mm.counts12 && !a.counts12_next) ok = hipMalloc(&a.counts12_next, b12) == hipSuccess && hipMemset(a.counts12_next, 0, b12) == hipSuccess;
+    if (!ok) {
+        (void)hipGetLastError();
+        if (a.heavy_next) { hipFree(a.heavy_next); a.heavy_next = nullptr; }
+        if (a.counts12_next) { hipFree(a.counts12_next); a.counts12_next = nullptr; }
+        a.mode &= ~MVHDP_AHEAD_TREES;
+    }
+    return ok;
 }
 
 hipError_t make_stream(hipStream_t* out, bool high_priority)
@@ -195,7 +222,12 @@
     h->device_released = true;
     hipSetDevice(h->device);
     if (h->stream) hipStreamSynchronize(h->stream);
+    mvhdp_ahead_drop_weights(h);
+    if (h->ahead.ev_go) { hipEventDestroy(h->ahead.ev_go); h->ahead.ev_go = nullptr; }
+    if (h->ahead.ev_done) { hipEventDestroy(h->ahead.ev_done); h->ahead.ev_done = nullptr; }
+    if (h->ahead.stream) { hipStreamDestroy(h->ahead.stream); h->ahead.stream = nullptr; }
     auto fr = [](auto*& p) { if (p) { hipFree((void*)p); p = nullptr; } };
+    fr(h->ahead.heavy_next); fr(h->ahead.counts12_next);
     for (int m = 0; m < MVHDP_MAXM; m++) { fr(h->d_doc_off[m]); fr(h->d_tok[m]); fr(h->d_z[m]); fr(h->d_carry[m]); fr(h->d_present[m]); }
     fr(h->mm.counts); fr(h->mm.delta16); fr(h->mm.counts16); fr(h->mm.counts12); fr(h->mm.heavy); fr(h->mm.delta); fr(h->mm.trees); fr(h->mm.root); fr(h->mm.coef); fr(h->mm.mass0); fr(h->d_births); fr(h->d_birth_keys); fr(h->d_birth_table); fr(h->mm.dtab); fr(h->mm.p);
     fr(h->d_alpha); fr(h->d_inactive); fr(h->d_ctl);
@@ -304,6 +336,7 @@
     mm.tok[m] = (const int32_t*)h->d_tok[m];
     mm.z[m] = (int32_t*)h->d_z[m];
     if (mm.p) { hipFree(mm.p); mm.p = nullptr; }
+    mvhdp_ahead_drop_weights(h);
     h->have_counts = false; h->have_trees = false;
     return MVHDP_OK;
 }
@@ -391,6 +424,7 @@
     HIPC(h, hipMemcpy(h->d_inactive, h->h_inactive.data(), (size_t)K, hipMemcpyHostToDevice));
     h->have_hyper = true;
     h->have_trees = false;
+    h->ahead.gen++;
     return MVHDP_OK;
 }
 
@@ -822,6 +856,14 @@
     if (which == MVHDP_BUF_BIRTH_KEYS) { *dev_ptr = h->d_birth_table; *bytes = (size_t)h->mm.K * sizeof(long long); return MVHDP_OK; }
     if (which == MVHDP_BUF_COUNTS12 && h->mm.counts12) { *dev_ptr = h->mm.counts12; *bytes = (size_t)h->mm.rowbase[h->mm.M] * mvhdp_slim_row_bytes(h->mm.K); return MVHDP_OK; }
     if (which == MVHDP_BUF_ROW_CLASS) { *dev_ptr = h->mm.heavy; *bytes = (size_t)h->mm.rowbase[h->mm.M]; return MVHDP_OK; }
+    const size_t nrows = (size_t)h->mm.rowbase[h->mm.M];
+    if (which == MVHDP_BUF_COUNTS16) { *dev_ptr = h->mm.counts16; *bytes = nrows * h->mm.K * sizeof(uint16_t); return MVHDP_OK; }
+    if (which == MVHDP_BUF_DESCENT) { *dev_ptr = h->mm.dtab; *bytes = nrows * h->mm.dt_nblk * 8 * sizeof(double); return MVHDP_OK; }
+    if (which == MVHDP_BUF_ROOTS) { *dev_ptr = h->mm.root; *bytes = nrows * sizeof(double); return MVHDP_OK; }
+    if ((which == MVHDP_BUF_ROW_CLASS_AHEAD || which == MVHDP_BUF_COUNTS12_AHEAD) && !h->have_trees.left_ahead)
+        FAIL(h, MVHDP_ERR_STATE, "device_buffer: nothing is kept ahead");
+    if (which == MVHDP_BUF_ROW_CLASS_AHEAD) { *dev_ptr = h->ahead.heavy_next; *bytes = nrows; return MVHDP_OK; }
+    if (which == MVHDP_BUF_COUNTS12_AHEAD && h->ahead.counts12_next) { *dev_ptr = h->ahead.counts12_next; *bytes = nrows * mvhdp_slim_row_bytes(h->mm.K); return MVHDP_OK; }
     FAIL(h, MVHDP_ERR_INVALID_ARG, "device_buffer: unknown buffer (or a handle without that table)");
 }
 
diff --git a/mvtopicmodel_amd/csrc/mvhdp_ctx.h b/mvtopicmodel_amd/csrc/mvhdp_ctx.h
--- a/mvtopicmodel_amd/csrc/mvhdp_ctx.h
+++ b/mvtopicmodel_amd/csrc/mvhdp_ctx.h
@@ -2,6 +2,7 @@
 #include "mvhdp_device.h"
 #include "../../include/mvhdp.h"
 #include "mvhdp_plan.h"
+#include "mvhdp_ahead.h"
 
 #include <algorithm>
 #include <functional>
@@ -19,6 +20,13 @@
 
 struct EmbState;
 
+struct TreesState {
+    bool current = false;
+    bool left_ahead = false;
+    TreesState& operator=(bool c) { current = c; left_ahead = false; return *this; }
+    operator bool() const { return current; }
+};
+
 struct mvhdp_ctx {
     mvhdp_config cfg{};
     MvModel mm{};
@@ -44,7 +52,8 @@
     uint8_t* d_inactive = nullptr;
     std::vector<double> h_alpha;
     std::vector<uint8_t> h_inactive;
-    bool have_hyper = false, have_counts = false, have_trees = false;
+    bool have_hyper = false, have_counts = false;
+    TreesState have_trees;
     bool full_trees = false;
     bool trees_inference = false;
     bool delta_clean = false;
@@ -77,6 +86,16 @@
         bool no_heavy_refresh = false;
     } diag;
     bool delta16_used = false;
+    struct Ahead {
+        int mode = MVHDP_AHEAD_TREES;
+        uint8_t* heavy_next = nullptr; uint8_t* counts12_next = nullptr;
+        double* p_next = nullptr;
+        AheadWeightsTag tag{};
+        uint64_t gen = 0;
+        hipStream_t stream = nullptr;
+        hipEvent_t ev_go = nullptr, ev_done = nullptr;
+        bool alloc_failed = false;
+    } ahead;
     int side_priority = 2;
     hipStream_t side[PLAN_N_STREAMS]{};
     hipEvent_t ev_fork = nullptr, ev_join[PLAN_N_STREAMS]{};
@@ -146,6 +165,7 @@
 
 struct PendingSweep {
     SweepPlan p;
+    bool fused = false;
     SweepOutcome oc;
     uint32_t flags = 0;
     bool debug = false;
@@ -161,6 +181,8 @@
 int apply_activation(mvhdp_ctx* h, int32_t activated_topic, int32_t activated_modality);
 int activate_born(mvhdp_ctx* h, const std::vector<std::pair<int32_t, long long>>& born, SweepOutcome& oc);
 hipError_t make_stream(hipStream_t* out, bool high_priority);
+void mvhdp_ahead_drop_weights(mvhdp_ctx* h);
+bool mvhdp_ahead_row_tables(mvhdp_ctx* h);
 int mvhdp_activate_births_ex(mvhdp_ctx* h, const int64_t* keys, int* n_born, long long* first_key);
 int mvhdp_view_overlap_accumulate(mvhdp_ctx* h, double* acc );
 int mvhdp_ll_doc_accumulate(mvhdp_ctx* h, int m, double* ll, int64_t* cnt);
diff --git a/mvtopicmodel_amd/csrc/mvhdp_device.h b/mvtopicmodel_amd/csrc/mvhdp_device.h
--- a/mvtopicmodel_amd/csrc/mvhdp_device.h
+++ b/mvtopicmodel_amd/csrc/mvhdp_device.h
@@ -94,7 +94,7 @@
 hipError_t mvhdp_launch_build_counts(const MvModel& mm, const int64_t* n_tokens_per_view, hipStream_t s);
 hipError_t mvhdp_launch_build_trees(const MvModel& mm, bool inference_leaves, bool write_full, hipStream_t s, bool beside_samplers = false);
 hipError_t mvhdp_launch_build_trees_rows(const MvModel& mm, bool inference_leaves, bool write_full, int64_t row_begin, int64_t row_end,
-                                         bool apply_first, unsigned long long* negatives, hipStream_t s);
+                                         bool apply_first, unsigned long long* negatives, hipStream_t s, bool with_delta16 = false);
 hipError_t mvhdp_launch_build_trees_from_mirror(const MvModel& mm, bool write_full, hipStream_t s, bool beside_samplers = false);
 hipError_t mvhdp_launch_widen_mirror(const MvModel& mm, hipStream_t s);
 hipError_t mvhdp_launch_live_rows_prepare(const MvModel& mm, bool from_mirror, bool with_heavy_trees, int32_t* heavy_list, unsigned int* heavy_ctl, int heavy_cap, int batch_cells, hipStream_t s);
diff --git a/mvtopicmodel_amd/csrc/mvhdp_enqueue.hip b/mvtopicmodel_amd/csrc/mvhdp_enqueue.hip
--- a/mvtopicmodel_amd/csrc/mvhdp_enqueue.hip
+++ b/mvtopicmodel_amd/csrc/mvhdp_enqueue.hip
@@ -255,14 +255,59 @@
     return sl;
 }
 
-static hipError_t view_weights(mvhdp_ctx* h, uint32_t sweep_idx, uint64_t seed, const double* p_override, hipStream_t s)
+static AheadSweep ahead_sweep_of(const mvhdp_ctx* h, const SweepPlan& p)
+{
+    AheadSweep a{};
+    a.frozen = p.frozen; a.no_apply = (p.flags & MVHDP_SWEEP_NO_APPLY) != 0; a.live = p.live; a.seg_apply = p.seg_apply;
+    a.reuse_trees = (p.flags & MVHDP_SWEEP_REUSE_TREES) != 0; a.only_segment = p.only_seg >= 0; a.debug = p.debug;
+    a.inactive_topics = h->mm.first_inactive >= 0; a.vectors_mix = h->mm.mix != nullptr;
+    return a;
+}
+static AheadWeightsTag weights_tag(const mvhdp_ctx* h, uint32_t sweep_idx, uint64_t seed)
+{
+    return AheadWeightsTag{true, sweep_idx, seed, h->mm.D, h->mm.doc_id_base, h->ahead.gen};
+}
+
+static hipError_t view_weights(mvhdp_ctx* h, const SweepPlan& p, uint32_t sweep_idx, uint64_t seed, const double* p_override, hipStream_t s)
 {
     MvModel& mm = h->mm;
     if (mm.M <= 1) return hipSuccess;
     const size_t bytes = (size_t)mm.D * mm.M * mm.M * sizeof(double);
     if (!mm.p && mm.D > 0) { hipError_t e = hipMalloc(&mm.p, bytes); if (e != hipSuccess) return e; }
+    auto& a = h->ahead;
+    if (a.p_next && mvhdp_ahead_weights_usable(a.tag, weights_tag(h, sweep_idx, seed), p_override != nullptr, a.mode, ahead_sweep_of(h, p))) {
+        a.tag.valid = false;
+        std::swap(mm.p, a.p_next);
+        return hipStreamWaitEvent(s, a.ev_done, 0);
+    }
     if (p_override) return hipMemcpyAsync(mm.p, p_override, bytes, hipMemcpyHostToDevice, s);
     return mvhdp_launch_draw_p(mm, sweep_idx, (uint32_t)seed, (uint32_t)(seed >> 32), s);
+}
+
+static bool draws_weights_ahead(mvhdp_ctx* h, const SweepPlan& p, const double* p_override)
+{
+    MvModel& mm = h->mm;
+    auto& a = h->ahead;
+    if (!(a.mode & MVHDP_AHEAD_WEIGHTS) || a.alloc_failed || mm.M <= 1 || mm.D <= 0 || p_override || !mvhdp_plain_deferred(ahead_sweep_of(h, p))) return false;
+    bool ok = true;
+    if (!a.stream) ok = make_stream(&a.stream, false) == hipSuccess;
+    if (ok && !a.ev_go) ok = hipEventCreateWithFlags(&a.ev_go, hipEventDisableTiming) == hipSuccess;
+    if (ok && !a.ev_done) ok = hipEventCreateWithFlags(&a.ev_done, hipEventDisableTiming) == hipSuccess;
+    if (ok && !a.p_next) ok = hipMalloc(&a.p_next, (size_t)mm.D * mm.M * mm.M * sizeof(double)) == hipSuccess;
+    if (!ok) { (void)hipGetLastError(); a.alloc_failed = true; a.p_next = nullptr; a.tag.valid = false; }
+    return ok;
+}
+static void draw_weights_ahead(mvhdp_ctx* h, uint32_t sweep_idx, uint64_t seed)
+{
+    MvModel& mm = h->mm;
+    auto& a = h->ahead;
+    a.tag.valid = false;
+    MvModel mn = mm;
+    mn.p = a.p_next;
+    if (hipStreamWaitEvent(a.stream, a.ev_go, 0) != hipSuccess) return;
+    if (mvhdp_launch_draw_p(mn, sweep_idx + 1, (uint32_t)seed, (uint32_t)(seed >> 32), a.stream) != hipSuccess) return;
+    if (hipEventRecord(a.ev_done, a.stream) != hipSuccess) return;
+    a.tag = weights_tag(h, sweep_idx + 1, seed);
 }
 
 static bool uses_refresher(const mvhdp_ctx* h, const SweepPlan& p) { return p.live_rows && p.live16 && !h->tu.single_wave && !h->diag.no_heavy_refresh; }
@@ -302,6 +347,11 @@
     hipError_t e = hipSuccess, e2 = hipSuccess;
     h->last_need_full = p.need_full;
     if (p.live_rows) { e = live_rows_prepare(h, p, false, s); h->have_trees = false; h->full_trees = false; }
+    else if (mvhdp_ahead_trees_usable(h->have_trees.left_ahead, h->ahead.mode, ahead_sweep_of(h, p))) {
+        h->have_trees = false; h->trees_inference = false;
+        std::swap(h->mm.heavy, h->ahead.heavy_next);
+        if (h->mm.counts12) std::swap(h->mm.counts12, h->ahead.counts12_next);
+    }
     else if (!(p.flags & MVHDP_SWEEP_REUSE_TREES)) e = rebuild_trees(h, p, s);
     if (p.need_full && !h->full_trees) { e2 = mvhdp_launch_build_trees(h->mm, h->trees_inference, true, s); h->full_trees = true; }
     return e != hipSuccess ? e : e2;
@@ -360,7 +410,7 @@
     const size_t cbytes = (size_t)clen * sizeof(int32_t);
 
     const SweepLaunch sl = fill_launch(h, p, sweep_idx, seed, nullptr, d_stats);
-    step(view_weights(h, sweep_idx, seed, p_override, X[0]));
+    step(view_weights(h, p, sweep_idx, seed, p_override, X[0]));
     bool use_mirror = false;
     for (int c = 0; c < MVHDP_N_CLASSES; c++) use_mirror = use_mirror || (p.cls[c].used && p.cls[c].narrow);
     step(trees_at_sweep_start(h, p, X[0]));
@@ -450,7 +500,7 @@
     const SweepLaunch sl = fill_launch(h, p, sweep_idx, seed, db, d_stats);
     const bool births = sl.births != nullptr;
     unsigned int* class_counts = h->d_ovf_meta + META_CLASS_COUNTS;
-    step(view_weights(h, sweep_idx, seed, p_override, s));
+    step(view_weights(h, p, sweep_idx, seed, p_override, s));
     const bool refresher = uses_refresher(h, p);
     step(trees_at_sweep_start(h, p, s));
     MvModel mk = mm;
@@ -468,6 +518,8 @@
     }
     step(mvhdp_launch_ctl_reset(d_stats, ST_COUNT, h->d_act_key, (unsigned long long*)h->d_ovf_meta, META_WORDS64, nullptr, h->d_doc_counter, s));
     if (births) step(births_begin(h, s));
+    const bool draw_ahead = draws_weights_ahead(h, p, p_override);
+    if (draw_ahead) step(hipEventRecord(h->ahead.ev_go, s));
     step(hipEventRecord(ev_k0, s));
 
     const int seg_lo = p.only_seg >= 0 ? p.only_seg : 0, seg_hi = p.only_seg >= 0 ? p.only_seg + 1 : nseg;
@@ -520,6 +572,7 @@
             step(e2);
         }
     }
+    if (draw_ahead && e == hipSuccess) draw_weights_ahead(h, sweep_idx, seed);
     if (p.seg_apply && mm.D > 0) {
         step(mvhdp_launch_apply_delta(mm, d_stats, s));
         h->have_trees = false;
@@ -528,6 +581,27 @@
     step(hipEventRecord(ev_k1, s));
     if (e != hipSuccess) HIPC(h, e);
     return MVHDP_OK;
+}
+
+static bool sweep_fuses_update(mvhdp_ctx* h, const SweepPlan& p)
+{
+    return h->mm.D > 0 && mvhdp_fuses_update(h->ahead.mode, ahead_sweep_of(h, p)) && mvhdp_ahead_row_tables(h);
+}
+static hipError_t fused_update(mvhdp_ctx* h, const SweepPlan& p, unsigned long long* negatives, hipStream_t s)
+{
+    MvModel& mm = h->mm;
+    hipError_t e = mvhdp_launch_apply_nk(mm, negatives, s);
+    MvModel mn = mm;
+    mn.heavy = h->ahead.heavy_next;
+    if (mm.counts12) mn.counts12 = h->ahead.counts12_next;
+    const hipError_t e2 = mvhdp_launch_build_trees_rows(mn, false, p.need_full, 0, mm.rowbase[mm.M], true, negatives, s, h->delta16_used);
+    return e != hipSuccess ? e : e2;
+}
+static void fused_update_done(mvhdp_ctx* h, const SweepPlan& p, bool keep_ahead)
+{
+    h->delta16_used = false; h->delta_clean = true; h->delta_pending = false;
+    h->have_trees = false; h->full_trees = p.need_full; h->trees_inference = false;
+    h->have_trees.left_ahead = keep_ahead;
 }
 
 static void stats_from_counters(const unsigned long long* hs, long long act, mvhdp_sweep_stats& st)
@@ -647,7 +721,10 @@
     hipError_t e = hipSuccess;
     if ((flags & MVHDP_SWEEP_NO_APPLY) && !ps.p.frozen)
         e = mvhdp_launch_birth_table(ps.births ? h->d_births : nullptr, h->d_birth_keys, h->d_act_key, h->mm.K, h->d_birth_table, s);
+    ps.fused = sweep_fuses_update(h, ps.p);
+    if (ps.fused && e == hipSuccess) e = fused_update(h, ps.p, h->d_stats + ST_NEGATIVE, s);
     if (e == hipSuccess) e = hipMemcpyAsync(h->h_ctl, h->d_ctl, (ST_COUNT + 1 + META_WORDS64) * sizeof(unsigned long long), hipMemcpyDeviceToHost, s);
+    if (ps.fused && e == hipSuccess) e = hipEventRecord(h->ev[3], s);
     if (e != hipSuccess) { ps.db.release(); HIPC(h, e); }
     ps.open = true;
     return MVHDP_OK;
@@ -667,6 +744,7 @@
     const unsigned long long* hs = h->h_ctl;
     const long long act = (long long)h->h_ctl[ST_COUNT];
     const unsigned long long* meta = h->h_ctl + ST_COUNT + 1;
+    if (ps.fused) fused_update_done(h, p, false);
     if (hs[ST_MISCLASS] || meta[META_MISROUTED]) {
         ps.db.release();
         h->nslots_valid = false;
@@ -710,12 +788,17 @@
             st.activated_topic = MVHDP_ACT_KEY_TOPIC(ps.oc.first_act); st.activated_modality = MVHDP_ACT_KEY_VIEW(ps.oc.first_act);
         }
         if (ret == MVHDP_OK && negatives) { h->err = "a topic count went below zero (UPD:202-215)"; ret = MVHDP_ERR_NEGATIVE_COUNT; }
+    } else if (ps.fused) {
+        if (negatives) { h->err = "a topic count went below zero (UPD:202-215)"; ret = MVHDP_ERR_NEGATIVE_COUNT; }
+        else h->have_trees.left_ahead = true;
     } else {
         if (st.activated_topic >= 0) n_activations = 1;
         ret = mvhdp_apply_delta(h, st.activated_topic, st.activated_modality);
     }
-    HIPC(h, hipEventRecord(h->ev[3], s));
-    HIPC(h, hipEventSynchronize(h->ev[3]));
+    if (!ps.fused) {
+        HIPC(h, hipEventRecord(h->ev[3], s));
+        HIPC(h, hipEventSynchronize(h->ev[3]));
+    }
     float ms_k = 0, ms_t = 0;
     hipEventElapsedTime(&ms_k, h->ev[1], h->ev[2]);
     hipEventElapsedTime(&ms_t, h->ev[0], h->ev[3]);
@@ -766,7 +849,10 @@
         unsigned long long* d_st = h->d_stats_many + (size_t)i * ST_COUNT;
         rc = enqueue_sweep(h, p, first_idx + (uint32_t)i, seed, nullptr, nullptr, d_st, h->ev_many[2 * i], h->ev_many[2 * i + 1], oc);
         if (rc) return rc;
-        if (!p.frozen && !p.live && !p.seg_apply) {
+        if (sweep_fuses_update(h, p)) {
+            HIPC(h, fused_update(h, p, d_st + ST_NEGATIVE, s));
+            fused_update_done(h, p, true);
+        } else if (!p.frozen && !p.live && !p.seg_apply) {
             HIPC(h, mvhdp_launch_apply_delta(mm, d_st, s, h->delta16_used));
             h->delta16_used = false;
             h->have_trees = false; h->delta_clean = true;
@@ -795,10 +881,11 @@
         st.sweep_kernel_ms = ms_k; st.total_ms = ms_t / n;
         ms_sum += ms_k;
         if (stats) stats[i] = st;
+        if (hi[ST_MISCLASS] || hi[ST_NEGATIVE]) h->have_trees = false;
         if (hi[ST_MISCLASS]) { h->nslots_valid = false; FAIL(h, MVHDP_ERR_HIP, "internal: an entity reached a sweep kernel variant that cannot hold its topic list"); }
         if (hi[ST_NEGATIVE] && ret == MVHDP_OK) { h->err = "a topic count went below zero (UPD:202-215)"; ret = MVHDP_ERR_NEGATIVE_COUNT; }
     }
-    if (meta[META_MISROUTED]) { h->nslots_valid = false; FAIL(h, MVHDP_ERR_HIP, "internal: an entity could not be routed to a sweep kernel"); }
+    if (meta[META_MISROUTED]) { h->have_trees = false; h->nslots_valid = false; FAIL(h, MVHDP_ERR_HIP, "internal: an entity could not be routed to a sweep kernel"); }
     std::vector<unsigned long long> acc(ST_COUNT, 0);
     for (int i = 0; i < n; i++) for (int k = 0; k < ST_COUNT; k++) acc[k] += hs[(size_t)i * ST_COUNT + k];
     const bool comparable = p.fast && !h->tu.walk_fixed && !(flags & (MVHDP_SWEEP_FROZEN | MVHDP_SWEEP_EXACT_CHAIN));
diff --git a/mvtopicmodel_amd/csrc/mvhdp_kernels.hip b/mvtopicmodel_amd/csrc/mvhdp_kernels.hip
--- a/mvtopicmodel_amd/csrc/mvhdp_kernels.hip
+++ b/mvtopicmodel_amd/csrc/mvhdp_kernels.hip
@@ -90,7 +90,8 @@
 
 template <int TB, bool MIX = false>
 __global__ __launch_bounds__(64) void build_trees_kernel(MvModel mm, bool inference_leaves, bool write_full, int64_t row_begin, int64_t row_end,
-                                                         bool apply_first, unsigned long long* negatives, bool from_mirror, bool only_heavy = false)
+                                                         bool apply_first, unsigned long long* negatives, bool from_mirror, bool only_heavy = false,
+                                                         uint16_t* d16 = nullptr)
 {
     extern __shared__ double t[];
     const int K = mm.K, lane = threadIdx.x;
@@ -104,6 +105,7 @@
         while (m + 1 < mm.M && row >= mm.rowbase[m + 1]) m++;
         int32_t* cnt = mm.counts + row * K;
         int32_t* dl = mm.delta + row * K;
+        uint16_t* dl16 = d16 ? d16 + row * K : nullptr;
         const int32_t* nk = nk_all + (int64_t)m * K;
         const double* al = mm.alpha + (int64_t)m * (K + 1);
         const double beta = mm.beta[m], beta_sum = mm.beta_sum[m], gamma = mm.gamma[m];
@@ -116,12 +118,13 @@
             long long sum = 0;
             int big = 0;
             for (int k0 = 0; k0 < K; k0 += WAVE * TB) {
-                int cv[TB], dv[TB];
+                int cv[TB], dv[TB], sv[TB];
 #pragma unroll
                 for (int u = 0; u < TB; u++) {
                     const int k = k0 + u * WAVE + lane;
                     cv[u] = (k < K) ? cnt[k] : 0;
                     dv[u] = (apply_first && k < K) ? dl[k] : 0;
+                    sv[u] = (apply_first && dl16 && k < K) ? (int)dl16[k] : 0x8000;
                 }
 #pragma unroll
                 for (int u = 0; u < TB; u++) {
@@ -129,8 +132,9 @@
                     if (k < K) {
                         int c = cv[u];
                         if (apply_first) {
-                            const int d = dv[u];
-                            if (d) { c += d; cnt[k] = c; dl[k] = 0; neg += c < 0; }
+                            int d = dv[u];
+                            if (sv[u] != 0x8000) { d += sv[u] - 0x8000; dl16[k] = (uint16_t)0x8000; if (!d && dv[u]) dl[k] = 0; }
+                            if (d) { c += d; cnt[k] = c; if (dv[u]) dl[k] = 0; neg += c < 0; }
                         }
                         sum += c < 0 ? 70000 : c;
                         big = max(big, c < 0 ? 70000 : c);
@@ -206,7 +210,7 @@
 }
 
 static hipError_t launch_trees(int tb, const MvModel& mm, bool inference_leaves, bool write_full, int64_t row_begin, int64_t row_end,
-                               bool apply_first, unsigned long long* negatives, bool from_mirror, hipStream_t s, bool only_heavy = false)
+                               bool apply_first, unsigned long long* negatives, bool from_mirror, hipStream_t s, bool only_heavy = false, uint16_t* d16 = nullptr)
 {
     const int64_t nrows = row_end - row_begin;
     if (nrows <= 0) return hipSuccess;
@@ -215,7 +219,7 @@
                   : tb == 4 ? (mix ? (const void*)build_trees_kernel<4, true> : (const void*)build_trees_kernel<4, false>)
                   : tb == 8 ? (mix ? (const void*)build_trees_kernel<8, true> : (const void*)build_trees_kernel<8, false>) : nullptr;
     if (!f) return hipErrorInvalidValue;
-    void* args[] = {(void*)&mm, &inference_leaves, &write_full, &row_begin, &row_end, &apply_first, &negatives, &from_mirror, &only_heavy};
+    void* args[] = {(void*)&mm, &inference_leaves, &write_full, &row_begin, &row_end, &apply_first, &negatives, &from_mirror, &only_heavy, &d16};
     (void)hipLaunchKernel(f, dim3((unsigned)(nrows < 65536 ? nrows : 65536)), dim3(64), args, (size_t)2 * mm.K * sizeof(double), s);
     return hipGetLastError();
 }
@@ -227,9 +231,10 @@
 }
 
 hipError_t mvhdp_launch_build_trees_rows(const MvModel& mm, bool inference_leaves, bool write_full, int64_t row_begin, int64_t row_end,
-                                         bool apply_first, unsigned long long* negatives, hipStream_t s)
-{
-    return launch_trees(mm.K > 512 ? 8 : 4, mm, inference_leaves, write_full, row_begin, row_end, apply_first, negatives, false, s);
+                                         bool apply_first, unsigned long long* negatives, hipStream_t s, bool with_delta16)
+{
+    return launch_trees(mm.K > 512 ? 8 : 4, mm, inference_leaves, write_full, row_begin, row_end, apply_first, negatives, false, s, false,
+                        apply_first && with_delta16 ? mm.delta16 : nullptr);
 }
 
 hipError_t mvhdp_launch_build_trees_from_mirror(const MvModel& mm, bool write_full, hipStream_t s, bool beside_samplers)
diff --git a/mvtopicmodel_amd/native.py b/mvtopicmodel_amd/native.py
--- a/mvtopicmodel_amd/native.py
+++ b/mvtopicmodel_amd/native.py
@@ -36,6 +36,11 @@
 BUF_BIRTH_KEYS = 2
 BUF_COUNTS12 = 3
 BUF_ROW_CLASS = 4
+BUF_COUNTS16 = 5
+BUF_DESCENT = 6
+BUF_ROOTS = 7
+BUF_COUNTS12_AHEAD = 8
+BUF_ROW_CLASS_AHEAD = 9
 ACT_KEY_NONE = (1 << 63) - 1
 
 
```
